# tkob-vh/umi-collapse-rs

Hardware: AMD Instinct MI355X
Metric: UMI-pair Hamming comparisons/s, effective (W pairs of the positions / hot-path time; 12-bp UMIs, all-pairs adjacency + directional collapse; the n-gram partition compares walked_fraction of W, the all-pairs kernels' result bit for bit) (higher is better)
Workload: dtype u32; 1 GPU; BASELINE config 2 per GPU: 1000000 reads, 12-bp UMIs, one alignment position (uniform UMIs), --data naive --algo dir -k 1 -p 0.5; standard=True, reads_per_rank=1000000, positions_per_rank=1, unique_umis_rank0=970714, pairs_W_total=471142349541, parallelism=one GPU

## Files before the change

### include/umihip.h

```cpp
#ifndef UMIHIP_H
#define UMIHIP_H

#include <stdint.h>

#ifdef __cplusplus
extern "C" {
#endif

#define UMI_OK 0
#define UMI_ERR_ARG (-1)
#define UMI_ERR_HIP (-2)
#define UMI_ERR_ORDER (-3)
#define UMI_ERR_NOMEM (-4)
#define UMI_ERR_NODEV (-5)
#define UMI_ERR_CHAR (-6)

#define UMI_ALGO_DIRECTIONAL 0
#define UMI_ALGO_ADJACENCY 1
#define UMI_ALGO_CLUSTER 2

#define UMI_MAX_UMI_LEN 21
#define UMI_MAX_WIDE_UMI_LEN 85
#define UMI_MAX_SEQ_LEN 256

typedef struct umi_ctx umi_ctx;
typedef struct umi_data umi_data;

typedef struct umi_stats {
    uint64_t n_umis;
    uint64_t n_buckets;
    uint64_t max_bucket;
    uint64_t n_kept;
    uint64_t n_pairs;
    uint64_t n_pairs_evaluated;
    uint64_t n_candidates;
    uint64_t n_edges;
    uint32_t n_rounds;
    uint32_t n_pair_launches;
    float ms_total;
    float ms_prep;
    float ms_pairs;
    float ms_collapse;
    float ms_finalize;
    float ms_kernel;
    uint32_t kernel_id;
} umi_stats;
#define UMI_KERNEL_NONE 0
#define UMI_KERNEL_FUSED 1
#define UMI_KERNEL_SEG_PAIRS 2
#define UMI_KERNEL_SEQ_PAIRS 3
#define UMI_KERNEL_EDIT_PAIRS 4

int umi_ctx_create(int device_id, umi_ctx **out);
int umi_ctx_create_multi(const int *device_ids, int n_devices, umi_ctx **out);
int umi_ctx_device_count(const umi_ctx *ctx);
void umi_ctx_destroy(umi_ctx *ctx);
int umi_partition_buckets(const uint64_t *bucket_off, uint64_t n_buckets, uint32_t n_ranks,
                          uint32_t *owner);
const char *umi_last_error(void);
int umi_ctx_set_option(umi_ctx *ctx, const char *name, int64_t value);
#define UMI_ABI_VERSION 2
int umi_abi_version(void);

int umi_encode_umis(const uint8_t *ascii, uint64_t n, int umi_len, uint64_t *keys,
                    uint64_t *nmask);

int umi_encode_umis_wide(const uint8_t *ascii, uint64_t n, int umi_len, int n_words, uint64_t *keys,
                         uint64_t *nmask);
int umi_dedup_batch_wide(umi_ctx *ctx, const uint64_t *keys, const uint64_t *nmask, int n_words,
                         const int32_t *freq, const uint64_t *bucket_off, uint64_t n_buckets,
                         int umi_len, int k, float percentage, int algo, int32_t adj_max_freq,
                         uint8_t *kept, uint32_t *root, umi_stats *stats);
int umi_dedup_batch_wide_device(umi_ctx *ctx, const uint64_t *d_keys, const uint64_t *d_nmask,
                                int n_words, const int32_t *d_freq, const uint64_t *bucket_off,
                                uint64_t n_buckets, int umi_len, int k, float percentage, int algo,
                                int32_t adj_max_freq, uint8_t *d_kept, uint32_t *d_root,
                                void *hip_stream, umi_stats *stats);

int umi_encode_seqs(const uint8_t *ascii, const uint64_t *seq_off, uint64_t n, int n_words, uint64_t *keys,
                    uint64_t *nmask);
int umi_dedup_seqs(umi_ctx *ctx, const uint64_t *keys, const uint64_t *nmask, int n_words, const int32_t *freq,
                   const uint64_t *bucket_off, const int32_t *bucket_len, uint64_t n_buckets, int k,
                   float percentage, int algo, int32_t adj_max_freq, uint8_t *kept, uint32_t *root,
                   umi_stats *stats);
int umi_dedup_seqs_device(umi_ctx *ctx, const uint64_t *d_keys, const uint64_t *d_nmask, int n_words,
                          const int32_t *d_freq, const uint64_t *bucket_off, const int32_t *bucket_len,
                          uint64_t n_buckets, int k, float percentage, int algo, int32_t adj_max_freq,
                          uint8_t *d_kept, uint32_t *d_root, void *hip_stream, umi_stats *stats);

int umi_stage_reads_device(umi_ctx *ctx, const uint64_t *d_align_key, int align_key_bits,
                           const uint8_t *d_umi_ascii, const int32_t *d_score, uint64_t n_reads,
                           int umi_len, int merge, uint64_t *d_keys, uint64_t *d_nmask,
                           int32_t *d_freq, uint64_t *d_rep, uint64_t *d_bucket_off,
                           uint64_t *n_entries, uint64_t *n_buckets, void *hip_stream);
int umi_stage_reads(umi_ctx *ctx, const uint64_t *align_key, int align_key_bits,
                    const uint8_t *umi_ascii, const int32_t *score, uint64_t n_reads, int umi_len,
                    int merge, uint64_t *keys, uint64_t *nmask, int32_t *freq, uint64_t *rep,
                    uint64_t *bucket_off, uint64_t *n_entries, uint64_t *n_buckets);
int umi_stage_reads_wide_device(umi_ctx *ctx, const uint64_t *d_align_key, int align_key_bits,
                                const uint8_t *d_umi_ascii, const int32_t *d_score, uint64_t n_reads, int umi_len,
                                int n_words, int merge, uint64_t *d_keys, uint64_t *d_nmask, int32_t *d_freq,
                                uint64_t *d_rep, uint64_t *d_bucket_off, uint64_t *n_entries, uint64_t *n_buckets,
                                void *hip_stream);
int umi_stage_reads_wide(umi_ctx *ctx, const uint64_t *align_key, int align_key_bits, const uint8_t *umi_ascii,
                         const int32_t *score, uint64_t n_reads, int umi_len, int n_words, int merge, uint64_t *keys,
                         uint64_t *nmask, int32_t *freq, uint64_t *rep, uint64_t *bucket_off, uint64_t *n_entries,
                         uint64_t *n_buckets);
int umi_stage_reads_grouped_device(umi_ctx *ctx, const uint64_t *d_align_key, int align_key_bits,
                                   const uint64_t *d_group_key, int group_key_bits, const uint8_t *d_umi_ascii,
                                   const int32_t *d_score, uint64_t n_reads, int umi_len, int merge, uint64_t *d_keys,
                                   uint64_t *d_nmask, int32_t *d_freq, uint64_t *d_rep, uint64_t *d_bucket_off,
                                   uint64_t *n_entries, uint64_t *n_buckets, void *hip_stream);
int umi_stage_reads_grouped(umi_ctx *ctx, const uint64_t *align_key, int align_key_bits, const uint64_t *group_key,
                            int group_key_bits, const uint8_t *umi_ascii, const int32_t *score, uint64_t n_reads, int umi_len,
                            int merge, uint64_t *keys, uint64_t *nmask, int32_t *freq, uint64_t *rep, uint64_t *bucket_off,
                            uint64_t *n_entries, uint64_t *n_buckets);
int umi_stage_reads_grouped_wide_device(umi_ctx *ctx, const uint64_t *d_align_key, int align_key_bits,
                                        const uint64_t *d_group_key, int group_key_bits, const uint8_t *d_umi_ascii,
                                        const int32_t *d_score, uint64_t n_reads, int umi_len, int n_words, int merge,
                                        uint64_t *d_keys, uint64_t *d_nmask, int32_t *d_freq, uint64_t *d_rep,
                                        uint64_t *d_bucket_off, uint64_t *n_entries, uint64_t *n_buckets, void *hip_stream);
int umi_stage_reads_grouped_wide(umi_ctx *ctx, const uint64_t *align_key, int align_key_bits, const uint64_t *group_key,
                                 int group_key_bits, const uint8_t *umi_ascii, const int32_t *score, uint64_t n_reads,
                                 int umi_len, int n_words, int merge, uint64_t *keys, uint64_t *nmask, int32_t *freq,
                                 uint64_t *rep, uint64_t *bucket_off, uint64_t *n_entries, uint64_t *n_buckets);

int umi_stage_seqs_device(umi_ctx *ctx, const uint8_t *d_text, const uint64_t *d_seq_pos,
                          const uint64_t *d_qual_pos, const uint32_t *d_len, uint64_t n_reads, int n_words,
                          int merge, uint64_t *d_keys, uint64_t *d_nmask, int32_t *d_freq, uint64_t *d_rep,
                          uint32_t *d_entry_of_read, uint64_t *bucket_off, int32_t *bucket_len,
                          uint64_t *n_entries, uint64_t *n_buckets, int *any_n, void *hip_stream);
int umi_stage_seqs(umi_ctx *ctx, const uint8_t *text, const uint64_t *seq_pos, const uint64_t *qual_pos,
                   const uint32_t *len, uint64_t n_reads, int n_words, int merge, uint64_t *keys,
                   uint64_t *nmask, int32_t *freq, uint64_t *rep, uint32_t *entry_of_read,
                   uint64_t *bucket_off, int32_t *bucket_len, uint64_t *n_entries, uint64_t *n_buckets,
                   int *any_n);

int umi_consensus_seqs_device(umi_ctx *ctx, const uint8_t *d_text, const uint64_t *d_seq_pos,
                              const uint64_t *d_qual_pos, const uint32_t *d_len, uint64_t n_reads,
                              const uint32_t *d_entry_of_read, const int32_t *d_freq, const uint8_t *d_kept,
                              const uint32_t *d_root, uint64_t n_entries, const uint64_t *bucket_off,
                              const int32_t *bucket_len, uint64_t n_buckets, uint8_t *d_cons_seq,
                              uint8_t *d_cons_qual, uint64_t *d_cons_off, uint32_t *d_cluster_reads,
// ... 243 lines not shown
```

### umi_collapse_rs_amd/_lib.py

```python
import ctypes as C
import os

_HERE = os.path.dirname(os.path.abspath(__file__))
LIB_PATH = os.environ.get("UMIHIP_LIB") or os.path.join(_HERE, "libumihip.so")

UMI_OK = 0
UMI_ERR_ARG, UMI_ERR_HIP, UMI_ERR_ORDER, UMI_ERR_NOMEM, UMI_ERR_NODEV, UMI_ERR_CHAR = (
    -1, -2, -3, -4, -5, -6)
UMI_ALGO_DIRECTIONAL, UMI_ALGO_ADJACENCY, UMI_ALGO_CLUSTER = 0, 1, 2
UMI_CELLS_CR22, UMI_CELLS_TOP, UMI_CELLS_MIN = 0, 1, 2
UMI_GENE_ASSIGNED, UMI_GENE_NONE, UMI_GENE_SEVERAL = 0, 1, 2
UMI_STRAND_FORWARD, UMI_STRAND_REVERSE, UMI_STRAND_UNSTRANDED = 0, 1, 2
UMI_INTRONS_OFF, UMI_INTRONS_EXON_FIRST, UMI_INTRONS_ALL = 0, 1, 2
UMI_GENE_TIER_EXON, UMI_GENE_TIER_INTRON = 0, 1
(UMI_READ_CLASS_NONE, UMI_READ_CLASS_EXONIC, UMI_READ_CLASS_JUNCTION, UMI_READ_CLASS_SPANNING,
 UMI_READ_CLASS_INTRONIC) = 0, 1, 2, 3, 4
UMI_READ_UNSTAGED = 0xFFFFFFFF
SATURATION_COLUMNS = ("reads", "molecules", "pairs", "cells", "molecules_in_cells", "pairs_in_cells", "median_molecules",
                      "median_genes")
UMI_MAX_UMI_LEN = 21
UMI_KERNEL_EDIT_PAIRS = 4
UMI_MAX_CONS_LEN = 1024
UMI_NO_CLUSTER = 0xFFFFFFFF


class UmiHipError(RuntimeError):
    def __init__(self, code, msg):
        super().__init__("umihip error %d: %s" % (code, msg))
        self.code = code


class Stats(C.Structure):
    _fields_ = [("n_umis", C.c_uint64), ("n_buckets", C.c_uint64), ("max_bucket", C.c_uint64),
                ("n_kept", C.c_uint64), ("n_pairs", C.c_uint64),
                ("n_pairs_evaluated", C.c_uint64), ("n_candidates", C.c_uint64),
                ("n_edges", C.c_uint64), ("n_rounds", C.c_uint32),
                ("n_pair_launches", C.c_uint32), ("ms_total", C.c_float),
                ("ms_prep", C.c_float), ("ms_pairs", C.c_float), ("ms_collapse", C.c_float),
                ("ms_finalize", C.c_float), ("ms_kernel", C.c_float), ("kernel_id", C.c_uint32)]

    def as_dict(self):
        return {k: getattr(self, k) for k, _ in self._fields_}


_u8p, _u32p, _u64p, _i32p = (C.POINTER(C.c_uint8), C.POINTER(C.c_uint32),
                             C.POINTER(C.c_uint64), C.POINTER(C.c_int32))

SIGNATURES = {
    "umi_ctx_create": (C.c_int, [C.c_int, C.POINTER(C.c_void_p)]),
    "umi_ctx_create_multi": (C.c_int, [C.POINTER(C.c_int), C.c_int, C.POINTER(C.c_void_p)]),
    "umi_ctx_device_count": (C.c_int, [C.c_void_p]),
    "umi_partition_buckets": (C.c_int, [_u64p, C.c_uint64, C.c_uint32, _u32p]),
    "umi_ctx_destroy": (None, [C.c_void_p]),
    "umi_last_error": (C.c_char_p, []),
    "umi_ctx_set_option": (C.c_int, [C.c_void_p, C.c_char_p, C.c_int64]),
    "umi_abi_version": (C.c_int, []),
    "umi_encode_umis": (C.c_int, [_u8p, C.c_uint64, C.c_int, _u64p, _u64p]),
    "umi_encode_umis_wide": (C.c_int, [_u8p, C.c_uint64, C.c_int, C.c_int, _u64p, _u64p]),
    "umi_dedup_batch_wide": (C.c_int, [C.c_void_p, _u64p, _u64p, C.c_int, _i32p, _u64p, C.c_uint64, C.c_int,
                                       C.c_int, C.c_float, C.c_int, C.c_int32, _u8p, _u32p, C.POINTER(Stats)]),
    "umi_dedup_batch_wide_device": (C.c_int, [C.c_void_p, C.c_void_p, C.c_void_p, C.c_int, C.c_void_p, _u64p,
                                              C.c_uint64, C.c_int, C.c_int, C.c_float, C.c_int, C.c_int32,
                                              C.c_void_p, C.c_void_p, C.c_void_p, C.POINTER(Stats)]),
    "umi_stage_reads_device": (C.c_int, [C.c_void_p, C.c_void_p, C.c_int, C.c_void_p, C.c_void_p, C.c_uint64,
                                         C.c_int, C.c_int, C.c_void_p, C.c_void_p, C.c_void_p, C.c_void_p,
                                         C.c_void_p, _u64p, _u64p, C.c_void_p]),
    "umi_stage_reads": (C.c_int, [C.c_void_p, _u64p, C.c_int, _u8p, _i32p, C.c_uint64, C.c_int, C.c_int,
                                  _u64p, _u64p, _i32p, _u64p, _u64p, _u64p, _u64p]),
    "umi_stage_reads_wide_device": (C.c_int, [C.c_void_p, C.c_void_p, C.c_int, C.c_void_p, C.c_void_p, C.c_uint64,
                                              C.c_int, C.c_int, C.c_int, C.c_void_p, C.c_void_p, C.c_void_p, C.c_void_p,
                                              C.c_void_p, _u64p, _u64p, C.c_void_p]),
    "umi_stage_reads_wide": (C.c_int, [C.c_void_p, _u64p, C.c_int, _u8p, _i32p, C.c_uint64, C.c_int, C.c_int, C.c_int,
                                       _u64p, _u64p, _i32p, _u64p, _u64p, _u64p, _u64p]),
    "umi_stage_reads_grouped_device": (C.c_int, [C.c_void_p, C.c_void_p, C.c_int, C.c_void_p, C.c_int, C.c_void_p,
                                                 C.c_void_p, C.c_uint64, C.c_int, C.c_int, C.c_void_p, C.c_void_p,
                                                 C.c_void_p, C.c_void_p, C.c_void_p, _u64p, _u64p, C.c_void_p]),
    "umi_stage_reads_grouped_wide_device": (C.c_int, [C.c_void_p, C.c_void_p, C.c_int, C.c_void_p, C.c_int,
                                                      C.c_void_p, C.c_void_p, C.c_uint64, C.c_int, C.c_int, C.c_int,
                                                      C.c_void_p, C.c_void_p, C.c_void_p, C.c_void_p, C.c_void_p,
                                                      _u64p, _u64p, C.c_void_p]),
    "umi_stage_reads_grouped": (C.c_int, [C.c_void_p, _u64p, C.c_int, _u64p, C.c_int, _u8p, _i32p, C.c_uint64, C.c_int,
                                          C.c_int, _u64p, _u64p, _i32p, _u64p, _u64p, _u64p, _u64p]),
    "umi_stage_reads_grouped_wide": (C.c_int, [C.c_void_p, _u64p, C.c_int, _u64p, C.c_int, _u8p, _i32p, C.c_uint64,
                                               C.c_int, C.c_int, C.c_int, _u64p, _u64p, _i32p, _u64p, _u64p, _u64p,
                                               _u64p]),
    "umi_stage_seqs_device": (C.c_int, [C.c_void_p, C.c_void_p, C.c_void_p, C.c_void_p, C.c_void_p, C.c_uint64, C.c_int,
                                        C.c_int, C.c_void_p, C.c_void_p, C.c_void_p, C.c_void_p, C.c_void_p, _u64p,
                                        _i32p, _u64p, _u64p, C.POINTER(C.c_int), C.c_void_p]),
    "umi_stage_seqs": (C.c_int, [C.c_void_p, _u8p, _u64p, _u64p, _u32p, C.c_uint64, C.c_int, C.c_int, _u64p, _u64p,
                                 _i32p, _u64p, _u32p, _u64p, _i32p, _u64p, _u64p, C.POINTER(C.c_int)]),
    "umi_encode_seqs": (C.c_int, [_u8p, _u64p, C.c_uint64, C.c_int, _u64p, _u64p]),
    "umi_dedup_seqs": (C.c_int, [C.c_void_p, _u64p, _u64p, C.c_int, _i32p, _u64p, _i32p, C.c_uint64, C.c_int,
                                 C.c_float, C.c_int, C.c_int32, _u8p, _u32p, C.POINTER(Stats)]),
    "umi_dedup_seqs_device": (C.c_int, [C.c_void_p, C.c_void_p, C.c_void_p, C.c_int, C.c_void_p, _u64p, _i32p,
                                        C.c_uint64, C.c_int, C.c_float, C.c_int, C.c_int32, C.c_void_p, C.c_void_p,
                                        C.c_void_p, C.POINTER(Stats)]),
    "umi_consensus_seqs_device": (C.c_int, [C.c_void_p, C.c_void_p, C.c_void_p, C.c_void_p, C.c_void_p, C.c_uint64,
                                            C.c_void_p, C.c_void_p, C.c_void_p, C.c_void_p, C.c_uint64, _u64p, _i32p,
                                            C.c_uint64, C.c_void_p, C.c_void_p, C.c_void_p, C.c_void_p, _u64p,
                                            C.c_void_p]),
    "umi_consensus_seqs": (C.c_int, [C.c_void_p, _u8p, _u64p, _u64p, _u32p, C.c_uint64, _u32p, _i32p, _u8p, _u32p,
                                     C.c_uint64, _u64p, _i32p, C.c_uint64, _u8p, _u8p, _u64p, _u32p, _u64p]),
    "umi_consensus_bam_device": (C.c_int, [C.c_void_p, C.c_void_p, C.c_void_p, C.c_void_p, C.c_void_p, C.c_void_p,
                                           C.c_uint64, C.c_void_p, C.c_uint64, C.c_void_p, C.c_void_p, C.c_void_p,
                                           C.c_void_p, C.c_void_p, C.c_void_p, _u64p, _u64p, C.c_void_p]),
    "umi_consensus_bam": (C.c_int, [C.c_void_p, _u8p, _u64p, _u64p, _u32p, _u32p, C.c_uint64, _u32p, C.c_uint64, _u8p,
                                    _u8p, _u64p, _u64p, _u32p, _u32p, _u64p, _u64p]),
    "umi_correct_umis_device": (C.c_int, [C.c_void_p, C.c_void_p, C.c_uint64, C.c_int, _u8p, C.c_uint32, C.c_int, C.c_int,
                                          C.c_void_p, C.c_void_p, C.c_void_p, C.c_void_p, _u64p, C.c_void_p]),
    "umi_correct_umis": (C.c_int, [C.c_void_p, _u8p, C.c_uint64, C.c_int, _u8p, C.c_uint32, C.c_int, C.c_int, _u8p,
                                   _i32p, _u8p, _u8p, _u64p]),
    "umi_correct_barcodes_device": (C.c_int, [C.c_void_p, C.c_void_p, C.c_uint64, C.c_int, _u8p, C.c_uint32, C.c_int,
                                              C.c_void_p, C.c_void_p, _u64p, C.c_void_p]),
    "umi_correct_barcodes": (C.c_int, [C.c_void_p, _u8p, C.c_uint64, C.c_int, _u8p, C.c_uint32, C.c_int, _i32p, _u8p,
                                       _u64p]),
    "umi_correct_barcodes_multi_device": (C.c_int, [C.c_void_p, C.c_void_p, C.c_void_p, C.c_uint64, C.c_int, _u8p,
                                                    C.c_uint32, C.c_int, C.c_int, C.c_void_p, C.c_void_p, C.c_void_p,
                                                    _u64p, C.c_void_p]),
    "umi_correct_barcodes_multi": (C.c_int, [C.c_void_p, _u8p, _u8p, C.c_uint64, C.c_int, _u8p, C.c_uint32, C.c_int,
                                             C.c_int, _i32p, _u8p, _u32p, _u64p]),
    "umi_assign_genes_device": (C.c_int, [C.c_void_p, _i32p, _i32p, _i32p, _u8p, _i32p, C.c_uint64, C.c_uint32, C.c_int,
                                          C.c_void_p, C.c_void_p, C.c_void_p, C.c_void_p, C.c_void_p, C.c_uint64,
                                          C.c_void_p, C.c_void_p, _u64p, C.c_void_p]),
    "umi_assign_genes": (C.c_int, [C.c_void_p, _i32p, _i32p, _i32p, _u8p, _i32p, C.c_uint64, C.c_uint32, C.c_int, _i32p,
                                   _i32p, _u8p, _u32p, _u64p, C.c_uint64, _i32p, _u8p, _u64p]),
    "umi_assign_genes_introns_device": (C.c_int, [C.c_void_p, _i32p, _i32p, _i32p, _u8p, _i32p, C.c_uint64, C.c_uint32, C.c_int,
                                                  C.c_int, C.c_void_p, C.c_void_p, C.c_void_p, C.c_void_p, C.c_void_p,
                                                  C.c_uint64, C.c_void_p, C.c_void_p, C.c_void_p, _u64p, C.c_void_p]),
    "umi_assign_genes_introns": (C.c_int, [C.c_void_p, _i32p, _i32p, _i32p, _u8p, _i32p, C.c_uint64, C.c_uint32, C.c_int,
                                           C.c_int, _i32p, _i32p, _u8p, _u32p, _u64p, C.c_uint64, _i32p, _u8p, _u8p, _u64p]),
    "umi_assign_genes_classes_device": (C.c_int, [C.c_void_p, _i32p, _i32p, _i32p, _u8p, _i32p, C.c_uint64, C.c_uint32, C.c_int,
                                                  C.c_int, C.c_void_p, C.c_void_p, C.c_void_p, C.c_void_p, C.c_void_p,
                                                  C.c_uint64, C.c_void_p, C.c_void_p, C.c_void_p, C.c_void_p, _u64p, _u64p,
                                                  C.c_void_p]),
    "umi_assign_genes_classes": (C.c_int, [C.c_void_p, _i32p, _i32p, _i32p, _u8p, _i32p, C.c_uint64, C.c_uint32, C.c_int,
                                           C.c_int, _i32p, _i32p, _u8p, _u32p, _u64p, C.c_uint64, _i32p, _u8p, _u8p, _u8p, _u64p,
                                           _u64p]),
    "umi_assign_genes_transcripts_device": (C.c_int, [C.c_void_p, _i32p, _i32p, _i32p, _u8p, _i32p, _i32p, C.c_uint64, C.c_uint32,
# ... 119 lines not shown
```

### umi_collapse_rs_amd/api.py

```python
import ctypes as C

import numpy as np

from . import _lib
from ._lib import (UMI_ALGO_ADJACENCY, UMI_ALGO_CLUSTER, UMI_ALGO_DIRECTIONAL, UMI_CELLS_CR22, Stats, UmiHipError, check, load, ptr)


def to_bitset(umis, umi_len=None):
    if isinstance(umis, np.ndarray):
        raw = np.ascontiguousarray(umis, dtype=np.uint8)
        assert umi_len, "umi_len is required for a raw byte array"
        n = raw.size // umi_len
    else:
        bs = [u.encode() if isinstance(u, str) else bytes(u) for u in umis]
        n = len(bs)
        umi_len = umi_len or (len(bs[0]) if bs else 1)
        if any(len(b) != umi_len for b in bs):
            raise ValueError("all UMIs of a run have the same length (umi_length)")
        raw = np.frombuffer(b"".join(bs), dtype=np.uint8)
    keys = np.zeros(n, dtype=np.uint64)
    nmask = np.zeros(n, dtype=np.uint64)
    check(load().umi_encode_umis(ptr(raw, C.c_uint8), n, umi_len, ptr(keys, C.c_uint64),
                                 ptr(nmask, C.c_uint64)))
    return keys, nmask


def to_bitset_wide(umis, umi_len):
    w = (3 * umi_len + 63) // 64
    buf = np.frombuffer("".join(umis).encode(), dtype=np.uint8)
    keys = np.zeros((len(umis), w), dtype=np.uint64)
    nm = np.zeros((len(umis), w), dtype=np.uint64)
    check(load().umi_encode_umis_wide(ptr(buf, C.c_uint8), len(umis), umi_len, w, ptr(keys, C.c_uint64),
                                      ptr(nm, C.c_uint64)))
    return keys, nm


def to_bitset_seq(seqs, n_words=None):
    bs = [s.encode() if isinstance(s, str) else bytes(s) for s in seqs]
    off = np.zeros(len(bs) + 1, dtype=np.uint64)
    off[1:] = np.cumsum([len(b) for b in bs], dtype=np.uint64)
    if n_words is None:
        n_words = max(1, (3 * max([len(b) for b in bs] or [0]) + 63) // 64)
    buf = np.frombuffer(b"".join(bs) or b"\0", dtype=np.uint8)
    keys = np.zeros((len(bs), n_words), dtype=np.uint64)
    nm = np.zeros((len(bs), n_words), dtype=np.uint64)
    check(load().umi_encode_seqs(ptr(buf, C.c_uint8), ptr(off, C.c_uint64), len(bs), n_words,
                                 ptr(keys, C.c_uint64), ptr(nm, C.c_uint64)))
    return keys, nm


def partition_buckets(bucket_off, n_ranks):
    bucket_off = np.ascontiguousarray(bucket_off, dtype=np.uint64)
    nb = max(0, len(bucket_off) - 1)
    owner = np.zeros(nb, dtype=np.uint32)
    check(load().umi_partition_buckets(ptr(bucket_off, C.c_uint64), nb, n_ranks, ptr(owner, C.c_uint32)))
    return owner


class Context:

    def __init__(self, device_id=0, profile=False):
        self._h = C.c_void_p()
        if isinstance(device_id, (list, tuple)):
            ids = (C.c_int * len(device_id))(*[int(d) for d in device_id])
            check(load().umi_ctx_create_multi(ids, len(device_id), C.byref(self._h)))
        else:
            check(load().umi_ctx_create(device_id, C.byref(self._h)))
        self.device_id = device_id
        if profile:
            self.set_option("profile", 1)

    def set_option(self, name, value):
        check(load().umi_ctx_set_option(self._h, name.encode(), int(value)))

    def close(self):
        if getattr(self, "_h", None):
            load().umi_ctx_destroy(self._h)
            self._h = None

    def __del__(self):
        try:
            self.close()
        except Exception:
            pass

    def dedup_batch(self, keys, nmask, freq, bucket_off, umi_len, k=1, percentage=0.5,
                    algo=UMI_ALGO_DIRECTIONAL, adj_max_freq=0, want_root=True):
        keys = np.ascontiguousarray(keys, dtype=np.uint64)
        freq = np.ascontiguousarray(freq, dtype=np.int32)
        bucket_off = np.ascontiguousarray(bucket_off, dtype=np.uint64)
        nm = None if nmask is None else np.ascontiguousarray(nmask, dtype=np.uint64)
        n = len(keys)
        if len(freq) != n or (nm is not None and len(nm) != n):
            raise ValueError("keys/nmask/freq lengths differ")
        if len(bucket_off) < 1 or (len(bucket_off) > 1 and int(bucket_off[-1]) != n):
            raise ValueError("bucket_off[-1] must equal len(keys)")
        kept = np.zeros(n, dtype=np.uint8)
        root = np.zeros(n, dtype=np.uint32) if want_root else None
        st = Stats()
        check(load().umi_dedup_batch(self._h, ptr(keys, C.c_uint64), ptr(nm, C.c_uint64),
                                     ptr(freq, C.c_int32), ptr(bucket_off, C.c_uint64),
                                     len(bucket_off) - 1, umi_len, k, percentage, algo,
                                     adj_max_freq, ptr(kept, C.c_uint8), ptr(root, C.c_uint32),
                                     C.byref(st)))
        return kept, root, st.as_dict()

    def dedup_batch_edit(self, keys, nmask, freq, bucket_off, umi_len, k=1, percentage=0.5,
                         algo=UMI_ALGO_DIRECTIONAL, adj_max_freq=0, want_root=True):
        keys = np.ascontiguousarray(keys, dtype=np.uint64)
        freq = np.ascontiguousarray(freq, dtype=np.int32)
        bucket_off = np.ascontiguousarray(bucket_off, dtype=np.uint64)
        nm = None if nmask is None else np.ascontiguousarray(nmask, dtype=np.uint64)
        n = len(keys)
        if len(freq) != n or (nm is not None and len(nm) != n):
            raise ValueError("keys/nmask/freq lengths differ")
        if len(bucket_off) < 1 or (len(bucket_off) > 1 and int(bucket_off[-1]) != n):
            raise ValueError("bucket_off[-1] must equal len(keys)")
        kept = np.zeros(n, dtype=np.uint8)
        root = np.zeros(n, dtype=np.uint32) if want_root else None
        st = Stats()
        check(load().umi_dedup_batch_edit(self._h, ptr(keys, C.c_uint64), ptr(nm, C.c_uint64),
                                          ptr(freq, C.c_int32), ptr(bucket_off, C.c_uint64),
                                          len(bucket_off) - 1, umi_len, k, percentage, algo,
                                          adj_max_freq, ptr(kept, C.c_uint8), ptr(root, C.c_uint32),
                                          C.byref(st)))
        return kept, root, st.as_dict()

    def dedup_batch_wide(self, keys, nmask, freq, bucket_off, umi_len, k=1, percentage=0.5,
                         algo=UMI_ALGO_DIRECTIONAL, adj_max_freq=0, want_root=True):
        keys = np.ascontiguousarray(keys, dtype=np.uint64)
        n, w = keys.shape
        nm = None if nmask is None else np.ascontiguousarray(nmask, dtype=np.uint64)
        freq = np.ascontiguousarray(freq, dtype=np.int32)
        bucket_off = np.ascontiguousarray(bucket_off, dtype=np.uint64)
        kept = np.zeros(max(1, n), dtype=np.uint8)
        root = np.zeros(max(1, n), dtype=np.uint32) if want_root else None
        st = Stats()
        check(load().umi_dedup_batch_wide(self._h, ptr(keys, C.c_uint64), ptr(nm, C.c_uint64), w,
                                          ptr(freq, C.c_int32), ptr(bucket_off, C.c_uint64), len(bucket_off) - 1,
                                          umi_len, k, percentage, algo, adj_max_freq, ptr(kept, C.c_uint8),
                                          ptr(root, C.c_uint32), C.byref(st)))
        return kept[:n], (root[:n] if want_root else None), st.as_dict()

    def dedup_seqs(self, keys, nmask, freq, bucket_off, bucket_len, k=1, percentage=0.5,
                   algo=UMI_ALGO_DIRECTIONAL, adj_max_freq=0, want_root=True):
        keys = np.ascontiguousarray(keys, dtype=np.uint64)
        if keys.ndim != 2:
            raise ValueError("keys must be [N, n_words]")
        n, w = keys.shape
        nm = None if nmask is None else np.ascontiguousarray(nmask, dtype=np.uint64)
        if nm is not None and nm.shape != keys.shape:
            raise ValueError("nmask must have the shape of keys")
        freq = np.ascontiguousarray(freq, dtype=np.int32)
        bucket_off = np.ascontiguousarray(bucket_off, dtype=np.uint64)
        bucket_len = np.ascontiguousarray(bucket_len, dtype=np.int32)
        if len(freq) != n or len(bucket_len) != len(bucket_off) - 1:
# ... 970 lines not shown
```

### umi_collapse_rs_amd/csrc/umihip_api.cpp

```cpp
#include "umihip_host.hpp"

#include <algorithm>
#include <cstdarg>
#include <cstdio>
#include <new>

using namespace umihip;

namespace umihip {

namespace {
thread_local std::string g_err;
}

int fail(int code, const char *fmt, ...)
{
    char buf[512];
    va_list ap;
    va_start(ap, fmt);
    vsnprintf(buf, sizeof(buf), fmt, ap);
    va_end(ap);
    g_err = buf;
    return code;
}

const std::string &last_error() { return g_err; }

int check_common(umi_ctx *ctx, const uint64_t *bucket_off, uint64_t n_buckets, int umi_len, int k,
                 int algo, uint64_t *n_out, int max_len)
{
    if (!ctx) return fail(UMI_ERR_ARG, "ctx is NULL");
    if (!bucket_off) return fail(UMI_ERR_ARG, "bucket_off is NULL");
    if (umi_len < 1 || umi_len > max_len)
        return fail(UMI_ERR_ARG, "umi_len %d outside 1..%d", umi_len, max_len);
    if (k < 0) return fail(UMI_ERR_ARG, "k must be >= 0 (got %d)", k);
    if (!known_algo(algo))
        return fail(UMI_ERR_ARG, "unknown algo %d", algo);
    const uint64_t n = n_buckets ? bucket_off[n_buckets] : 0;
    if (n_buckets && bucket_off[0] != 0) return fail(UMI_ERR_ARG, "bucket_off[0] must be 0");
    if (n >= 0x7FFFFFF0ull)
        return fail(UMI_ERR_ARG, "%llu entries exceed the 31-bit index space of one call",
                    (unsigned long long)n);
    *n_out = n;
    return UMI_OK;
}

}

extern "C" {

const char *umi_last_error(void) { return last_error().c_str(); }

int umi_abi_version(void) { return UMI_ABI_VERSION; }

int umi_ctx_create(int device_id, umi_ctx **out)
{
    if (!out) return fail(UMI_ERR_ARG, "out is NULL");
    *out = nullptr;
    int n_dev = 0;
    hipError_t e = hipGetDeviceCount(&n_dev);
    if (e != hipSuccess || n_dev == 0)
        return fail(UMI_ERR_NODEV, "no HIP device visible (%s)",
                    e == hipSuccess ? "device count 0" : hipGetErrorString(e));
    if (device_id < 0 || device_id >= n_dev)
        return fail(UMI_ERR_ARG, "device_id %d outside 0..%d", device_id, n_dev - 1);
    hipDeviceProp_t prop;
    HIP_TRY(hipGetDeviceProperties(&prop, device_id));
    if (strncmp(prop.gcnArchName, "gfx950", 6) != 0)
        return fail(UMI_ERR_NODEV, "device %d is %s; this library carries gfx950 code only",
                    device_id, prop.gcnArchName);
    HIP_TRY(hipSetDevice(device_id));
    umi_ctx *ctx = new (std::nothrow) umi_ctx();
    if (!ctx) return fail(UMI_ERR_NOMEM, "out of host memory");
    ctx->device = device_id;
    ctx->device_cus = prop.multiProcessorCount > 0 ? prop.multiProcessorCount : 256;
    ctx->n_cus = ctx->device_cus;
    hipError_t err = hipStreamCreateWithFlags(&ctx->own_stream, hipStreamNonBlocking);
    if (err == hipSuccess)
        err = hipHostMalloc((void **)&ctx->h_counters, CTRL_BYTES + 64);
    if (err == hipSuccess) *ctx->h_seq() = 0;
    for (int i = 0; i < umi_ctx::N_EVENTS && err == hipSuccess; i++) err = hipEventCreate(&ctx->ev[i]);

    if (err != hipSuccess) {
        umi_ctx_destroy(ctx);
        return fail(UMI_ERR_HIP, "context setup failed: %s", hipGetErrorString(err));
    }
    *out = ctx;
    return UMI_OK;
}

void umi_ctx_destroy(umi_ctx *ctx)
{
    if (!ctx) return;
    if (!ctx->subs.empty()) {
        for (ncclComm_t c : ctx->comms)
            if (c && ctx->rccl.CommDestroy) (void)ctx->rccl.CommDestroy(c);
        for (umi_ctx *sub : ctx->subs) umi_ctx_destroy(sub);
        delete ctx;
        return;
    }
    settle(ctx);
    (void)hipSetDevice(ctx->device);
    if (ctx->h_counters) (void)hipHostFree(ctx->h_counters);
    for (int i = 0; i < umi_ctx::N_EVENTS; i++)
        if (ctx->ev[i]) (void)hipEventDestroy(ctx->ev[i]);
    if (ctx->own_stream) (void)hipStreamDestroy(ctx->own_stream);
    delete ctx;
}

int umi_ctx_set_option(umi_ctx *ctx, const char *name, int64_t value)
{
    if (!ctx || !name) return fail(UMI_ERR_ARG, "ctx/name is NULL");
    if (!strcmp(name, "split_min")) {
        if (value < 2) return fail(UMI_ERR_ARG, "split_min must be >= 2");
        ctx->split_min = (uint64_t)value;
        return UMI_OK;
    }
    if (!ctx->subs.empty()) {
        for (umi_ctx *sub : ctx->subs) {
            const int rc = umi_ctx_set_option(sub, name, value);
            if (rc) return rc;
        }
        return UMI_OK;
    }
    if (!strcmp(name, "profile")) {
        ctx->profile = value != 0;
    } else if (!strcmp(name, "edge_capacity")) {
        if (value < 1) return fail(UMI_ERR_ARG, "edge_capacity must be >= 1");
        ctx->edge_capacity = (uint64_t)value;
#ifdef UMIHIP_DEV
    } else if (!strcmp(name, "prune")) {
        ctx->prune = value != 0;
    } else if (!strcmp(name, "bs_unit")) {
        if (value < 1 || value > 3) return fail(UMI_ERR_ARG, "bs_unit must be 1, 2 or 3");
        ctx->bs_unit = (int)value;
    } else if (!strcmp(name, "bs_sorted")) {
        ctx->bs_sorted = value != 0;
    } else if (!strcmp(name, "bs_tables")) {
        ctx->bs_tables = value != 0;
    } else if (!strcmp(name, "two_phase")) {
        if (value < 0 || value > 2) return fail(UMI_ERR_ARG, "two_phase must be 0, 1 or 2");
        ctx->two_phase = (int)value;
    } else if (!strcmp(name, "bs_col_chunk")) {
        if (value < BS_COL_TILE || value > (1 << 24) || value % BS_COL_TILE)
            return fail(UMI_ERR_ARG, "bs_col_chunk must be a multiple of %d in %d..%d", BS_COL_TILE,
                        BS_COL_TILE, 1 << 24);
        ctx->bs_col_chunk = (uint32_t)value;
    } else if (!strcmp(name, "bs_tab_min_run")) {
        if (value < 0 || value > (1 << 30)) return fail(UMI_ERR_ARG, "bs_tab_min_run must be in 0..2^30");
        ctx->bs_tab_min_run = (uint32_t)value;
    } else if (!strcmp(name, "bs_transposed")) {
        ctx->bs_transposed = value != 0;
    } else if (!strcmp(name, "bs_tab_waves")) {
        if (value < 0 || value > (1 << 20)) return fail(UMI_ERR_ARG, "bs_tab_waves must be in 0..%d", 1 << 20);
        ctx->bs_tab_waves = (uint32_t)value;
    } else if (!strcmp(name, "bitslice")) {
        ctx->use_bitslice = value != 0;
    } else if (!strcmp(name, "ovf_capacity")) {
        if (value < 1) return fail(UMI_ERR_ARG, "ovf_capacity must be >= 1");
        ctx->ovf_capacity = (uint64_t)value;
#endif
    } else if (!strcmp(name, "seg_index")) {
        ctx->seg_index = value != 0;
    } else if (!strcmp(name, "table_pieces")) {
        if (value < 1 || value > 64) return fail(UMI_ERR_ARG, "table_pieces must be in 1..64");
        ctx->table_pieces = (uint32_t)value;
    } else if (!strcmp(name, "seg_ckey")) {
        ctx->seg_ckey = value != 0;
    } else if (!strcmp(name, "spin_wait")) {
        ctx->spin_wait = value != 0;
    } else if (!strcmp(name, "seg_sliced")) {
        ctx->seg_sliced = value != 0;
    } else if (!strcmp(name, "seg_unite")) {
        ctx->seg_unite = value != 0;
    } else if (!strcmp(name, "seg_lds")) {
        ctx->seg_lds = value != 0;
    } else if (!strcmp(name, "seg_local")) {
        ctx->seg_local = value != 0;
    } else if (!strcmp(name, "seg_probe")) {
        if (value != 0 && value != 1) return fail(UMI_ERR_ARG, "seg_probe must be 0 or 1");
        ctx->seg_probe = value != 0;
    } else if (!strcmp(name, "seg_probe_min")) {
        if (value < 2 || value > SEG_LOCAL_MAX_CAP) return fail(UMI_ERR_ARG, "seg_probe_min must be in 2..%u", SEG_LOCAL_MAX_CAP);
        ctx->seg_probe_min = (uint32_t)value;
    } else if (!strcmp(name, "seg_super")) {
        if (value != 0 && value != 1) return fail(UMI_ERR_ARG, "seg_super must be 0 or 1");
        ctx->seg_super = value != 0;
    } else if (!strcmp(name, "seg_super_coarse")) {
        if (value != 0 && value != 1) return fail(UMI_ERR_ARG, "seg_super_coarse must be 0 or 1");
        ctx->seg_super_coarse = value != 0;
    } else if (!strcmp(name, "seg_super_bases")) {
        if (value < 0 || value > SEG_SUPER_MAX_BASES) return fail(UMI_ERR_ARG, "seg_super_bases must be in 0..%d", SEG_SUPER_MAX_BASES);
        ctx->seg_super_bases = (int)value;
    } else if (!strcmp(name, "seg_super_cap")) {
        if (value < 2 || value > SEG_SUPER_MAX_CAP) return fail(UMI_ERR_ARG, "seg_super_cap must be in 2..%u", SEG_SUPER_MAX_CAP);
        ctx->seg_super_cap = (uint32_t)value;
    } else if (!strcmp(name, "seg_super_min")) {
        if (value < 2 || value > SEG_SUPER_MAX_CAP) return fail(UMI_ERR_ARG, "seg_super_min must be in 2..%u", SEG_SUPER_MAX_CAP);
        ctx->seg_super_min = (uint32_t)value;
    } else if (!strcmp(name, "collapse_kept_only")) {
        ctx->collapse_kept_only = value != 0;
    } else if (!strcmp(name, "seg_local_cap")) {
        if (value < 2 || value > SEG_LOCAL_MAX_CAP) return fail(UMI_ERR_ARG, "seg_local_cap must be in 2..%u", SEG_LOCAL_MAX_CAP);
        ctx->seg_local_cap = (uint32_t)value;
    } else if (!strcmp(name, "seg_blocks")) {
        if (value < 0 || value > (1 << 22)) return fail(UMI_ERR_ARG, "seg_blocks must be in 0..2^22");
        ctx->seg_blocks = (uint32_t)value;
    } else if (!strcmp(name, "grid_cus")) {
        if (value < 0 || value > ctx->device_cus)
            return fail(UMI_ERR_ARG, "grid_cus must be in 0..%d (the device's CUs)", ctx->device_cus);
        ctx->n_cus = value ? (int)value : ctx->device_cus;
    } else if (!strcmp(name, "seg_min")) {
        if (value < 2 || value > (1ll << 31)) return fail(UMI_ERR_ARG, "seg_min must be in 2..2^31");
        ctx->seg_min = (uint32_t)value;
    } else if (!strcmp(name, "cons_split")) {
        if (value < 2 || value > (1ll << 30)) return fail(UMI_ERR_ARG, "cons_split must be in 2..2^30");
        ctx->cons_split = (uint32_t)value;
    } else if (!strcmp(name, "stats_split")) {
        if (value < 64 || value > (1ll << 30)) return fail(UMI_ERR_ARG, "stats_split must be in 64..2^30");
        ctx->stats_split = (uint32_t)value;
    } else if (!strcmp(name, "gene_top")) {
        if (value != 0 && value != 1) return fail(UMI_ERR_ARG, "gene_top must be 0 or 1");
        ctx->gene_top = value != 0;
    } else if (!strcmp(name, "gene_body_top")) {
        if (value != 0 && value != 1) return fail(UMI_ERR_ARG, "gene_body_top must be 0 or 1");
        ctx->gene_body_top = value != 0;
    } else if (!strcmp(name, "velocity_skip")) {
        if (value != 0 && value != 1) return fail(UMI_ERR_ARG, "velocity_skip must be 0 or 1");
        ctx->velocity_skip = value != 0;
    } else if (!strcmp(name, "saturation_skip")) {
        if (value != 0 && value != 1) return fail(UMI_ERR_ARG, "saturation_skip must be 0 or 1");
        ctx->saturation_skip = value != 0;
    } else if (!strcmp(name, "fused_sliced")) {
        ctx->fused_sliced = value != 0;
    } else if (!strcmp(name, "fused_blocks")) {
        if (value < 1 || value > 64) return fail(UMI_ERR_ARG, "fused_blocks must be in 1..64");
        ctx->fused_blocks = (uint32_t)value;
    } else if (!strcmp(name, "fused_max")) {
        if (value < 0) return fail(UMI_ERR_ARG, "fused_max must be >= 0");
        ctx->fused_max = (uint32_t)std::min<int64_t>(value, FUSED_MAX);
    } else if (!strcmp(name, "small_max")) {
        if (value < 0) return fail(UMI_ERR_ARG, "small_max must be >= 0");
        ctx->small_max = (uint32_t)std::min<int64_t>(value, 1 << 30);
    } else {
        return fail(UMI_ERR_ARG, "unknown option '%s'", name);
    }
    return UMI_OK;
}

int umi_ctx_create_multi(const int *device_ids, int n_devices, umi_ctx **out)
{
    if (!out) return fail(UMI_ERR_ARG, "out is NULL");
    *out = nullptr;
    if (!device_ids || n_devices < 1 || n_devices > 64)
        return fail(UMI_ERR_ARG, "device_ids is NULL or n_devices outside 1..64");
    umi_ctx *ctx = new (std::nothrow) umi_ctx();
    if (!ctx) return fail(UMI_ERR_NOMEM, "out of host memory");
    for (int i = 0; i < n_devices; i++) {
        umi_ctx *sub = nullptr;
        const int rc = umi_ctx_create(device_ids[i], &sub);
        if (rc) {
            const std::string msg = umi_last_error();
            umi_ctx_destroy(ctx);
            return fail(rc, "%s", msg.c_str());
        }
        ctx->subs.push_back(sub);
    }
    ctx->device = device_ids[0];
    *out = ctx;
    return UMI_OK;
}

int umi_ctx_device_count(const umi_ctx *ctx) { return !ctx ? 0 : (ctx->subs.empty() ? 1 : (int)ctx->subs.size()); }
// ... 3 lines not shown
```

### umi_collapse_rs_amd/csrc/umihip_host.hpp

```cpp
#pragma once
#include "../../include/umihip.h"

#include <cstring>
#include <dlfcn.h>
#include <string>
#include <type_traits>
#include <vector>

#include "umihip_internal.h"
#include "umihip_io_layout.hpp"
#include "umihip_plan.hpp"

#include <rccl/rccl.h>

namespace umihip {

int fail(int code, const char *fmt, ...);
const std::string &last_error();

#define HIP_TRY(expr)                                                                        \
    do {                                                                                     \
        hipError_t e__ = (expr);                                                             \
        if (e__ != hipSuccess)                                                               \
            return fail(UMI_ERR_HIP, "%s failed: %s (%s:%d)", #expr, hipGetErrorString(e__), \
// ... 93 lines not shown
        for (const char *name : {"librccl.so.1", "librccl.so", "/opt/rocm/lib/librccl.so.1"}) {
            handle = dlopen(name, RTLD_NOW | RTLD_GLOBAL);
            if (handle) break;
        }
        if (!handle) {
            error = std::string("cannot open librccl.so: ") + dlerror();
            return false;
        }
        auto sym = [&](const char *name) {
            void *p = dlsym(handle, name);
            if (!p && error.empty()) error = std::string("librccl.so lacks ") + name;
            return p;
        };
        CommInitAll = (decltype(CommInitAll))sym("ncclCommInitAll");
        CommDestroy = (decltype(CommDestroy))sym("ncclCommDestroy");
        GroupStart = (decltype(GroupStart))sym("ncclGroupStart");
        GroupEnd = (decltype(GroupEnd))sym("ncclGroupEnd");
        AllGather = (decltype(AllGather))sym("ncclAllGather");
        GetErrorString = (decltype(GetErrorString))sym("ncclGetErrorString");
        if (!error.empty()) {
            handle = nullptr;
            return false;
        }
        return true;
    }
};

constexpr int BATCH_MAX_K = 32 * 4;

inline bool known_algo(int algo) { return algo == UMI_ALGO_DIRECTIONAL || algo == UMI_ALGO_ADJACENCY || algo == UMI_ALGO_CLUSTER; }
inline int mode_of(int algo)
{
    return algo == UMI_ALGO_DIRECTIONAL ? MODE_DIRECTIONAL : algo == UMI_ALGO_CLUSTER ? MODE_CLUSTER : MODE_ADJACENCY;
}

inline int wide_words(int umi_len) { return (3 * umi_len + 63) / 64; }

}

struct umi_ctx {
    umihip::RcclApi rccl;
    std::vector<ncclComm_t> comms;
    std::vector<umi_ctx *> subs;
    umihip::PinnedBuf sh_in, sh_out;
    std::vector<uint64_t> sh_boff;
    int device = 0;
    hipStream_t own_stream = nullptr;
    bool profile = false;
    uint64_t edge_capacity = 1u << 20;
    uint64_t ovf_capacity = 1u << 18;
    uint32_t small_max = 1024;
#ifdef UMIHIP_DEV
    static constexpr bool LEGACY_DEFAULT = true;
#else
    static constexpr bool LEGACY_DEFAULT = false;
#endif
    bool use_bitslice = LEGACY_DEFAULT;
    uint32_t bs_col_chunk = umihip::BS_COL_CHUNK;
    uint32_t bs_tab_min_run = 4;
    bool bs_transposed = true;
    uint32_t bs_tab_waves = 0;
    uint32_t fused_max = umihip::FUSED_MAX;
    uint32_t fused_blocks = 20;
    bool fused_sliced = true;
    int bs_unit = 2;
    bool bs_sorted = LEGACY_DEFAULT;
    bool bs_tables = LEGACY_DEFAULT;
    int two_phase = 2;
    bool seg_index = true;
    uint32_t seg_min = 512;
    uint64_t split_min = 200000;
    uint32_t table_pieces = 1;
    bool seg_ckey = true;
    bool seg_sliced = true;
    bool seg_unite = true;
    bool seg_lds = true;
    int seg_occ[2][2][2] = {{{0, 0}, {0, 0}}, {{0, 0}, {0, 0}}};
    bool seg_local = true;
    uint32_t seg_local_cap = umihip::SEG_LOCAL_CAP;
    bool seg_probe = true;
    uint32_t seg_probe_min = umihip::SEG_PROBE_MIN;
    bool seg_super = true;
    bool seg_super_coarse = true;
    int seg_super_bases = 0;
    uint32_t seg_super_cap = umihip::SEG_SUPER_CAP;
    uint32_t seg_super_min = umihip::SEG_SUPER_MIN;
    int seg_local_occ[2] = {0, 0};
    uint32_t seg_local_occ_cap = 0;
    bool collapse_kept_only = true;
    uint32_t seg_blocks = 0;
    umihip::DevBuf fkey, thr, label, lab, edges, edge_dist, ovf, counters, boff, status, blocked;
    umihip::DevBuf plan_tables;
    umihip::DevBuf bs_tasks, plane_tasks, planes, tab_rows, tab_items;
    umihip::DevBuf seg_bin_cnt, seg_bin_start, seg_tasks, seg_sub_rec, seg_priv_edges, seg_priv_dist, seg_priv_cnt, seg_priv_stat;
    umihip::PinnedBuf h_plan_alt[2];
    int plan_flip = 0;
    size_t plan_uploaded = 0;
    const void *plan_uploaded_to = nullptr;
    int n_cus = 256;
    int device_cus = 256;
    umihip::DevBuf fkey_sorted, perm, iota, sort_tmp, sample_pos, sample_out;
    bool prune = false;
    umihip::Plan plan;
    umihip::TablePass table_pass;
    umihip::DevBuf io;
    umihip::DevBuf call_ws;
    umihip::DevBuf seq_groups, seq_ka, seq_kb, seq_va, seq_vb, seq_flag, seq_runid, seq_rs, seq_tend, seq_tmp;
    umihip::PinnedBuf cm_h, ds_h;
    uint32_t stats_split = umihip::STATS_SPLIT;
    bool gene_top = true;
    bool velocity_skip = false;
    bool saturation_skip = false;
    bool gene_body_top = true;
    uint32_t cons_split = 512;
    umihip::PinnedBuf h_boff;
    umihip::PinnedBuf h_tasks;
    unsigned long long *h_counters = nullptr;
    unsigned long long ctrl_seq = 0;
    int dag_rounds_ahead = umihip::DAG_ROUNDS;
    struct PendingCall {
        bool deferred = false, have_result = false;
        unsigned long long seq = 0;
        hipStream_t stream = nullptr;
        int rc = UMI_OK;
        std::string err;
        umi_stats st;
    } pending;
    bool spin_wait = true;
    unsigned long long *h_seq() const { return h_counters + umihip::CTRL_BYTES / sizeof(unsigned long long); }
    uint32_t *h_changed() const { return (uint32_t *)(h_counters + umihip::CNT_COUNT); }
    uint32_t *d_changed() const { return (uint32_t *)(counters.as<unsigned long long>() + umihip::CNT_COUNT); }
    static constexpr int N_EVENTS = 10;
    hipEvent_t ev[N_EVENTS] = {};
};

namespace umihip {

int check_common(umi_ctx *ctx, const uint64_t *bucket_off, uint64_t n_buckets, int umi_len, int k,
                 int algo, uint64_t *n_out, int max_len = UMI_MAX_UMI_LEN);

int run_pipeline(umi_ctx *ctx, const uint64_t *d_keys, const uint64_t *d_nmask,
                 const int32_t *d_freq, const uint64_t *bucket_off, uint64_t n_buckets, uint32_t n,
                 int umi_len, int k, float percentage, int mode, int32_t adj_max_freq,
                 uint8_t *d_kept, uint32_t *d_root, hipStream_t s, umi_stats *stats,
                 const uint64_t *d_bucket_off = nullptr, int n_words = 1, bool may_defer = false, bool edit = false);
int run_pipeline_part(umi_ctx *ctx, const uint64_t *d_keys, const uint64_t *d_nmask, const int32_t *d_freq,
                      const uint64_t *bucket_off, uint64_t n_buckets, uint32_t n, int umi_len, int k,
                      float percentage, int mode, int32_t adj_max_freq, hipStream_t s, uint32_t part,
                      uint32_t n_parts, umi_stats *stats, uint64_t *n_edges);
int collapse_edges(umi_ctx *ctx, uint32_t n, const uint2 *d_edges, uint32_t n_edges, int mode, uint8_t *d_kept,
                   uint32_t *d_root, hipStream_t s, umi_stats *stats);
int finish_pending(umi_ctx *ctx, umi_stats *stats);
void settle(umi_ctx *ctx);

template <typename T> struct IoPtr {
    const DevBuf *block = nullptr;
    size_t off = IO_ABSENT;
    operator T *() const { return (T *)io_at(block->p, off); }
};

class HostIo {
    struct Upload {
        const void *host;
        size_t off, bytes;
    };
    umi_ctx *ctx;
    IoLayout layout;
    std::vector<Upload> uploads;
    bool busy = false;

public:
    explicit HostIo(umi_ctx *c) : ctx(c) {}
    HostIo(const HostIo &) = delete;
    HostIo &operator=(const HostIo &) = delete;
    ~HostIo()
    {
        if (busy) (void)hipStreamSynchronize(ctx->own_stream);
// ... 39 lines not shown
```

### umi_collapse_rs_amd/csrc/umihip_internal.h

```cpp
#pragma once

#include <hip/hip_runtime_api.h>
#include <stdint.h>

namespace umihip {

struct PairTask {
    uint32_t row0;
    uint32_t row_end;
    uint32_t col0;
    uint32_t col1;
};

enum PairMode : int {
    MODE_DIRECTIONAL = 0,
    MODE_ADJACENCY = 1,
    MODE_NEIGHBOURS = 2,
    MODE_CLUSTER = 3,
};

enum Counter : int {
    CNT_EDGES = 0,
    CNT_CANDIDATES = 1,
    CNT_ERROR = 2,
    CNT_KEPT = 3,
    CNT_UNKNOWN = 4,
    CNT_RISES = 5,
    CNT_START_RISES = 6,
    CNT_OVF = 7,
    CNT_ITEMS = 8,
    CNT_DIAG_ITEMS = 9,
    CNT_GRAB = 10,
    CNT_DIAG_GRAB = 11,
    CNT_SEG_TASKS = 12,
    CNT_SEG_PAIRS = 13,
    CNT_KEPT_FUSED = 14,
    CNT_UF_DIRECT = 15,
    CNT_EDGES_MOVED = 16,
    CNT_COUNT = 17,
};
constexpr int MAX_ROUNDS_PER_SYNC = 16;
constexpr size_t CTRL_FLAGS_OFF = CNT_COUNT * sizeof(unsigned long long);
constexpr size_t CTRL_BYTES = (CTRL_FLAGS_OFF + (MAX_ROUNDS_PER_SYNC + 1) * sizeof(uint32_t) + 255) & ~(size_t)255;

struct BsTask {
    uint32_t bucket_start;
    uint32_t bucket_end;
    uint32_t group0;
    uint32_t ngroups;
    uint64_t plane_off;
    uint32_t col0, col1;
    uint32_t diag;
    uint32_t pad;
};

struct RangeTask {
    uint32_t start, end;
    uint32_t seg;
};
constexpr uint32_t SEG_NONE = 0xFFFFFFFFu;

constexpr int SEG_MAX_PARTS = 8;
struct SegDesc {
    uint32_t start, end;
    uint32_t bin_off[SEG_MAX_PARTS];
    uint8_t b0[SEG_MAX_PARTS];
    uint8_t nb[SEG_MAX_PARTS];
    uint64_t mask[SEG_MAX_PARTS];
    uint8_t sup_g;
    uint8_t sup_pad[7];
};
struct SegSuper {
    uint32_t bin0;
    uint8_t g, nb, rest, pad;
};
struct SegRec32 {
    uint32_t key;
    uint32_t idx;
    int32_t freq;
    uint32_t ckey;
};
struct SegRec64 {
    uint64_t key;
    uint32_t idx;
    int32_t freq;
};
struct SegScanChunk {
    uint32_t bin0, nbins;
    uint32_t seg, part;
};
constexpr uint32_t SEG_SCAN_CHUNK = 256;
struct SegTask {
    uint32_t row0, end;
    uint32_t col0;
    uint32_t where;
};
#if defined(__HIPCC__)
#define UMIHIP_HD __host__ __device__
#else
#define UMIHIP_HD
#endif
UMIHIP_HD inline uint32_t seg_chunks_of(uint32_t c) { return c >= 2 ? (c - 1 + 63) / 64 : 0u; }
UMIHIP_HD inline uint32_t seg_span_log2(uint32_t nt)
{
    uint32_t e = 0;
    while (((nt + 15) / 16) > (1u << e)) e++;
    return e;
}
UMIHIP_HD inline uint32_t seg_tasks_of_bin(uint32_t c)
{
    const uint32_t nt = seg_chunks_of(c);
    if (nt == 0) return 0;
    const uint32_t span = 1u << seg_span_log2(nt), q = nt / span, r = nt % span;
    return span * (q * (q + 1) / 2) + r * (q + 1);
}
inline uint64_t seg_task_bound(uint64_t n, uint64_t bins) { return n / 7 + (bins < n / 2 ? bins : n / 2) + 64; }
struct SegBlock {
    uint32_t start, end;
    uint32_t seg, pad;
};
constexpr uint32_t SEG_BLOCK_THREADS = 1024;
constexpr uint32_t SEG_BLOCK_ENTRIES = 8 * SEG_BLOCK_THREADS;
constexpr uint32_t SEG_LDS_BINS = 16384;
constexpr uint32_t RANGE_CHUNK = 2048;

constexpr int BS_TAB_G = 1;
constexpr int BS_TAB_TILE = 256;
constexpr int FUSED_MAX = 128;

struct PlaneTask {
    uint32_t row0;
    uint32_t bucket_end;
    uint64_t plane_off;
    uint32_t ngroups;
    uint32_t group;
};

struct PairArgs {
    const uint64_t *keys;
    const uint64_t *nmask;
    const int32_t *freq;
    const int32_t *thr;
    const void *fkey;
    const PairTask *tasks;
    const BsTask *bs_tasks;
    const uint32_t *planes;
    const uint32_t *perm;
    uint2 *edges;
    uint8_t *edge_dist;
    unsigned long long *counters;
    uint2 *ovf;
    uint32_t ovf_cap;
    uint32_t edge_cap;
    uint32_t n_entries;
    int k;
    int mode;
    int32_t adj_max_freq;
};

constexpr int SMALL_THREADS = 64;
constexpr int SMALL_RPT = 1;
constexpr int BIG_THREADS = 256;
constexpr int BIG_RPT = 8;
constexpr int SMALL_ROWS = SMALL_THREADS * SMALL_RPT;
constexpr int BIG_ROWS = BIG_THREADS * BIG_RPT;
constexpr int COL_TILE = 1024;

hipError_t launch_prep(const uint64_t *keys, const uint64_t *nmask, const int32_t *freq,
                       const uint64_t *bucket_off, uint64_t n_buckets, const RangeTask *ranges,
                       uint32_t n_ranges, uint32_t n, uint32_t fused_max, int umi_len, float percentage,
                       bool key32, void *fkey, int32_t *thr, uint32_t *label, uint32_t *lab,
                       unsigned long long *counters, const SegDesc *segs, int n_seg_parts,
                       uint32_t *bin_cnt, hipStream_t s, bool skip_seg = false, bool entries_too = true,
                       uint32_t seg_from = 0xFFFFFFFFu, int key_words = 1, int full_umi_len = 0);

struct SegArgs {
    const SegDesc *segs;
    const SegScanChunk *chunks;
    uint32_t n_chunks;
    int n_parts;
    uint32_t *bin_cnt;
    uint32_t *bin_start;
    unsigned long long *scan_state;
    SegTask *tasks;
    uint32_t task_cap;
    void *sub_rec;
    const RangeTask *ranges;
    uint32_t n_ranges;
    const SegBlock *blocks;
    uint32_t n_blocks;
    uint32_t lds_bins;
    uint32_t parts_per_pass;
    uint2 *priv_edges;
    uint8_t *priv_dist;
    uint32_t *priv_cnt;
    uint2 *priv_stat;
    uint32_t *uf_parent;
    const uint64_t *prep_keys, *prep_nmask;
    const int32_t *prep_freq;
    int32_t *prep_thr;
    uint32_t *prep_label;
    uint32_t *prep_lab;
    float prep_percentage;
    unsigned long long *prep_counters;
    int umi_len;
    int key_words;
    int full_umi_len;
    uint32_t use_ckey;
    uint32_t col_sliced;
    uint32_t local_cap;
    uint32_t probe_rest, probe_min;
    uint32_t super_cap;
    const SegSuper *supers;
    uint32_t n_supers;
    uint32_t super_coarse;
    uint32_t super_count_pairs;
#ifdef UMIHIP_DEV
    unsigned long long *super_stamps;
#endif
};
constexpr int SEG_SUPER_PHASES = 9;
UMIHIP_HD inline uint32_t seg_scan_flag_word(uint32_t n_chunks, uint32_t seg) { return 1u + n_chunks + seg; }
hipError_t launch_seg_build(const SegArgs &g, void *fkey, const int32_t *freq, bool key32,
                            unsigned long long *counters, hipStream_t s);
constexpr uint32_t SEG_PRIV_CAP = 512;
int seg_pair_blocks_per_cu(bool key32, bool has_n, bool ckey);
hipError_t launch_seg_pairs(const PairArgs &a, const SegArgs &g, bool key32, float percentage,
                            uint32_t part, uint32_t n_parts, uint32_t n_blocks, hipStream_t s);
hipError_t launch_seg_edge_append(const PairArgs &a, const SegArgs &g, uint32_t n_blocks, hipStream_t s);
constexpr uint32_t SEG_LOCAL_MAX_CAP = 2048;
constexpr uint32_t SEG_LOCAL_CAP = 512;
constexpr int SEG_PROBE_MAX_REST = 6;
constexpr uint32_t SEG_PROBE_WORDS = (1u << (2 * SEG_PROBE_MAX_REST)) / 32;
constexpr uint32_t SEG_PROBE_MIN = 129;
constexpr int SEG_SUPER_MAX_REST = 8;
constexpr uint32_t SEG_SUPER_WORDS = (1u << (2 * SEG_SUPER_MAX_REST)) / 32;
constexpr int SEG_SUPER_MAX_BASES = 4;
constexpr uint32_t SEG_SUPER_MAX_CAP = 8192;
constexpr uint32_t SEG_SUPER_CAP = 5632;
constexpr uint32_t SEG_SUPER_MIN = 1024;
constexpr uint32_t SEG_SUPER_SMALL = 2048;
inline uint32_t seg_super_threads(uint32_t cap) { return cap <= SEG_SUPER_SMALL ? 256u : 1024u; }
size_t seg_super_lds_bytes(uint32_t cap);
uint32_t seg_super_blocks(uint32_t n_supers, uint32_t n_cus);
hipError_t launch_seg_super(const PairArgs &a, const SegArgs &g, float percentage, uint32_t n_blocks, hipStream_t s);
size_t seg_local_lds_bytes(uint32_t cap);
int seg_local_blocks_per_cu(bool has_n, uint32_t cap);
hipError_t launch_seg_local(const PairArgs &a, const SegArgs &g, float percentage, uint32_t n_blocks, hipStream_t s);

hipError_t launch_wide_pairs(const PairArgs &a, uint32_t n_tasks, int n_words, hipStream_t s);

hipError_t launch_edit_prep(const uint64_t *keys, const uint64_t *nmask, const int32_t *freq, const uint64_t *bucket_off,
                            uint64_t n_buckets, uint32_t n, int umi_len, float percentage, uint64_t *planes,
                            uint32_t *counts, int32_t *thr, uint32_t *label, unsigned long long *counters, hipStream_t s);
hipError_t launch_edit_pairs(const PairArgs &a, const uint32_t *counts, uint32_t n_tasks, int umi_len, hipStream_t s);

constexpr int SEQ_MAX_WORDS = 12;
constexpr uint32_t SEQ_TILE = 64;
constexpr uint32_t SEQ_ALL_PAIRS = 0xFFFFFFFFu;
struct SeqGroup {
    uint32_t rec_off, bstart, n;
    uint32_t len, nw;
    uint32_t part, n_parts;
    uint32_t pad;
};
struct SeqPairArgs {
    const SeqGroup *groups;
    const uint64_t *rkey;
    const uint32_t *rval;
    uint32_t n_rec;
    const uint64_t *run_id;
    const uint32_t *run_start;
    const uint64_t *task_end;
    const uint64_t *keys, *nmask;
    int stride;
    const int32_t *freq, *thr;
    uint2 *edges;
    unsigned long long *counters;
    uint32_t edge_cap;
    int k, mode;
    int32_t adj_max_freq;
};
hipError_t launch_seq_records(const SeqGroup *groups, uint32_t n_groups, uint32_t n_rec, const uint64_t *keys,
                              const uint64_t *nmask, int stride, const int32_t *freq, float percentage, int32_t *thr,
                              uint64_t *rkey, uint32_t *rval, unsigned long long *counters, hipStream_t s);
hipError_t launch_seq_runs(const uint64_t *rkey, uint32_t n_rec, uint64_t *flag, uint64_t *run_id,
                           uint32_t *run_start, uint64_t *task_end, void *scan_temp, size_t scan_temp_size,
                           unsigned long long *counters, hipStream_t s);
hipError_t launch_seq_pairs(const SeqPairArgs &a, uint32_t n_blocks, hipStream_t s);

size_t stage_workspace_bytes(uint32_t n_reads, int n_words, bool grouped = false);
int stage_reads_on_device(void *workspace, const uint64_t *d_align, int align_bits, const uint64_t *d_group,
                          int group_bits, const uint8_t *d_umi,
                          const int32_t *d_score, uint32_t n, int umi_len, int n_words, int merge, uint64_t *d_keys,
                          uint64_t *d_nmask, int32_t *d_freq, uint64_t *d_rep, uint64_t *d_bucket_off,
                          uint64_t *n_entries_out, uint64_t *n_buckets_out, unsigned long long *h_pinned4,
                          hipStream_t s);

struct SeqFault {
    uint64_t read = 0, value = 0;
};
size_t stage_seqs_workspace_bytes(uint32_t n_reads, int n_words);
int stage_seqs_on_device(void *workspace, const uint8_t *d_text, const uint64_t *d_seq_pos, const uint64_t *d_qual_pos,
                         const uint32_t *d_len, uint32_t n, int n_words, int merge, uint64_t *d_keys, uint64_t *d_nmask,
                         int32_t *d_freq, uint64_t *d_rep, uint32_t *d_eor, uint64_t *h_bucket_off, int32_t *h_bucket_len,
                         uint64_t *n_entries_out, uint64_t *n_buckets_out, int *any_n, SeqFault *fault,
                         unsigned long long *h_pinned4, hipStream_t s);

struct ConsFault {
    unsigned long long bad_root = 0, bad_read = 0, bad_len = 0, empty = 0, freq_sum = 0;
};
uint32_t consensus_effective_split(uint32_t n_reads, uint32_t split);
size_t consensus_workspace_bytes(uint32_t n_reads, uint32_t n_entries, uint32_t n_buckets, uint32_t split);
int consensus_on_device(void *workspace, const uint8_t *d_text, const uint64_t *d_seq_pos, const uint64_t *d_qual_pos,
                        const uint32_t *d_len, uint32_t n_reads, const uint32_t *d_eor, const int32_t *d_freq,
                        const uint8_t *d_kept, const uint32_t *d_root, uint32_t n_entries, const uint64_t *h_bucket_off,
                        const int32_t *h_bucket_len, uint32_t n_buckets, uint32_t split, uint32_t n_cus, uint8_t *d_cons_seq,
                        uint8_t *d_cons_qual, uint64_t *d_cons_off, uint32_t *d_cluster_reads, uint64_t *cons_bytes,
                        ConsFault *fault, unsigned long long *h_pinned, hipStream_t s);

struct ConsBamFault {
    unsigned long long bad_cluster_len = 0, bad_id = 0, bad_len = 0;
};
size_t consensus_bam_workspace_bytes(uint32_t n_reads, uint32_t n_clusters, uint32_t split);
int consensus_bam_on_device(void *workspace, const uint8_t *d_data, const uint64_t *d_seq_pos, const uint64_t *d_qual_pos,
                            const uint32_t *d_len, const uint32_t *d_cluster, uint32_t n_reads, const uint32_t *d_cluster_len,
                            uint32_t n_clusters, uint32_t split, uint32_t n_cus, uint8_t *d_cons_seq, uint8_t *d_cons_qual,
                            uint64_t *d_seq_off, uint64_t *d_qual_off, uint32_t *d_depth, uint32_t *d_disagree,
// ... 262 lines not shown
```

### umi_collapse_rs_amd/csrc/umihip_pipeline.cpp

```cpp
#include "umihip_host.hpp"

#include <algorithm>
#include <chrono>

using namespace umihip;

namespace {

template <class LaunchRound>
int run_rounds(umi_ctx *ctx, hipStream_t s, LaunchRound launch_round, int &rounds, int batch = 4)
{
    uint32_t *d_changed = ctx->d_changed();
    for (;;) {
        HIP_TRY(hipMemsetAsync(d_changed, 0, sizeof(uint32_t) * MAX_ROUNDS_PER_SYNC, s));
        for (int r = 0; r < batch; r++) HIP_TRY(launch_round(d_changed, r));
        HIP_TRY(hipMemcpyAsync(ctx->h_changed(), d_changed, sizeof(uint32_t) * batch, hipMemcpyDeviceToHost, s));
        HIP_TRY(hipStreamSynchronize(s));
        bool done = false;
        for (int r = 0; r < batch && !done; r++) {
            rounds++;
            done = ctx->h_changed()[r] == 0;
        }
        if (done) return UMI_OK;
        if (rounds > MAX_ROUNDS) return fail(UMI_ERR_HIP, "label propagation diverged");
// ... 65 lines not shown
    const unsigned long long bad =
        ctx->h_counters[CNT_ERROR] + (ctx->h_counters[CNT_RISES] - ctx->h_counters[CNT_START_RISES]);
    if (bad)
        return fail(UMI_ERR_ORDER,
                    "%llu entries break the input contract (freq < 1, not in freq-descending rank "
                    "order inside a bucket, or an N base without nmask)",
                    bad);
    return UMI_OK;
}

class Pipeline {
  public:
    Pipeline(umi_ctx *ctx, const uint64_t *d_keys, const uint64_t *d_nmask, const int32_t *d_freq,
             const uint64_t *bucket_off, uint64_t n_buckets, uint32_t n, int umi_len, int k,
             float percentage, int mode, int32_t adj_max_freq, uint8_t *d_kept, uint32_t *d_root,
             hipStream_t s, uint32_t part = 0, uint32_t n_parts = 1)
        : ctx(ctx), d_keys(d_keys), d_nmask(d_nmask), d_freq(d_freq), bucket_off(bucket_off),
          n_buckets(n_buckets), n(n), umi_len(umi_len), k(std::min(k, BATCH_MAX_K)), percentage(percentage), mode(mode),
          adj_max_freq(adj_max_freq), d_kept(d_kept), d_root(d_root), s(s), pl(ctx->plan),
          key32(umi_len <= 16),
          need_pairs(!(mode == MODE_ADJACENCY && adj_max_freq < 1)),
          fused_max((mode == MODE_NEIGHBOURS || !need_pairs || n_parts > 1)
                        ? 0u
                        : std::min<uint32_t>(ctx->fused_max, FUSED_MAX)),
          prof(ctx->profile), part(part), n_parts(n_parts)
    {
        memset(&st, 0, sizeof(st));
        st.n_umis = n;
        st.n_buckets = n_buckets;
    }

    int run(umi_stats *stats)
    {
        HIP_TRY(hipSetDevice(ctx->device));
        int rc = run_stages();
        if (!drained) (void)hipStreamSynchronize(s);
        if (rc == UMI_OK && stats) *stats = st;
        return rc;
    }

    uint64_t edge_count() const { return n_edges; }
    void use_device_table(const uint64_t *d_table) { d_boff_caller = d_table; }
    void use_wide_keys(int words) { n_words = words; }
    void allow_deferred_end() { may_defer = true; }
    void use_edit_distance()
    {
        edit = true;
        k = std::min(k, umi_len);
        fused_max = 0;
    }

  private:
    umi_ctx *ctx;
    const uint64_t *d_keys, *d_nmask;
    const int32_t *d_freq;
    const uint64_t *bucket_off;
    const uint64_t *d_boff_caller = nullptr;
    int n_words = 1;
    bool edit = false;
    bool wide() const { return n_words > 1; }
    int plan_umi_len() const { return wide() ? 21 : umi_len; }
    const uint64_t *d_boff() const { return d_boff_caller ? d_boff_caller : ctx->boff.as<uint64_t>(); }
    uint64_t n_buckets;
    uint32_t n;
    int umi_len, k;
    float percentage;
    int mode;
    int32_t adj_max_freq;
    uint8_t *d_kept;
    uint32_t *d_root;
    hipStream_t s;
    Plan &pl;
    const bool key32, need_pairs;
    uint32_t fused_max;
    const bool prof;
    const uint32_t part, n_parts;
    uint64_t task_counter = 0;
    bool prune = false, drained = false, fused_ran = false, seg_timed = false, edit_timed = false;
    bool may_defer = false;
    size_t zero_behind_control = 0;
    uint32_t priv_blocks_for_collapse = 0;
    uint64_t seg_local_bins = 0;
    bool super_pairs_counted = false;
    umi_stats st;
    unsigned long long *d_cnt = nullptr;
    size_t n_tasks = 0;
    uint64_t n_edges = 0;
    uint64_t n_direct = 0;
    uint64_t seg_tasks_made = 0;
    uint32_t cap_used = 0;
    const void *bs_fkey = nullptr;
    [[maybe_unused]] const uint32_t *bs_perm = nullptr;
    const RangeTask *d_ranges = nullptr;
    const SegDesc *d_segs = nullptr;
    const SegScanChunk *d_chunks = nullptr;
    const PairTask *d_small = nullptr, *d_big = nullptr;
    const SegBlock *d_seg_blocks = nullptr;
    const SegSuper *d_supers = nullptr;
    SegArgs seg;

    bool one_sync() const
    {
        return (mode == MODE_DIRECTIONAL || mode == MODE_CLUSTER || !need_pairs) && n_parts == 1 && ctx->two_phase == 2 &&
               !legacy_tiles();
    }
    bool unions_collapse() const { return mode == MODE_DIRECTIONAL || mode == MODE_CLUSTER; }
    bool mask_only_collapse() const { return d_root == nullptr && ctx->collapse_kept_only; }
    uint32_t *prep_lab() const
    {
        return mode == MODE_DIRECTIONAL && n_parts == 1 && ctx->two_phase == 2 && mask_only_collapse() ? ctx->lab.as<uint32_t>() : nullptr;
    }

    int run_stages()
    {
        int rc;
        if (wide() && (mode != MODE_DIRECTIONAL || k > 3)) fused_max = 0;
        const bool plan_first = n_buckets <= 4096;
        if (plan_first) {
            for (uint64_t b = 0; b < n_buckets; b++)
                if (bucket_off[b + 1] < bucket_off[b])
                    return fail(UMI_ERR_ARG, "bucket_off not monotone at bucket %llu", (unsigned long long)b);
            plan_host();
            if (pl.seg_parts && need_pairs) zero_behind_control = seg_zero_bytes();
        }
        if ((rc = reserve_core())) return rc;
        if ((rc = upload_table(!plan_first))) return rc;
        if (plan_first && pl.n_fused && (rc = fused_stage(0, n_buckets))) return rc;
        if (!plan_first) plan_host();
        if (ctx->table_pass.bad_at != ~0ull)
            return fail(UMI_ERR_ARG, "bucket_off not monotone at bucket %llu", (unsigned long long)ctx->table_pass.bad_at);
        if ((rc = upload_plan())) return rc;
        if ((rc = configure_seg())) return rc;
        if ((rc = prep_stage())) return rc;
        if ((rc = cut_legacy_tiles())) return rc;
        if (need_pairs && pl.seg_parts)
            HIP_TRY(launch_seg_build(seg, ctx->fkey.p, d_freq, key32, d_cnt, s));
        if ((rc = upload_legacy_tiles())) return rc;
        if ((rc = count_tasks())) return rc;
        if (one_sync()) return run_one_sync();
        if (mode == MODE_CLUSTER && n_parts == 1)
            return fail(UMI_ERR_ARG, "algo cluster does not run with the development option two_phase below 2");
        if ((rc = pair_stage())) return rc;
        if (mode == MODE_NEIGHBOURS || n_parts > 1) return finish_neighbours();
        if (mode == MODE_DIRECTIONAL || !need_pairs)
            rc = collapse_directional();
        else
            rc = collapse_adjacency();
        if (rc) return rc;
        return finish();
    }

    int key_bits() const { return key32 ? 2 * umi_len : std::min(64, 3 * umi_len); }

    template <class T> void keep_my_share(std::vector<T> &v)
    {
        if (n_parts <= 1) return;
        size_t w = 0;
        for (size_t i = 0; i < v.size(); i++)
            if ((task_counter++ % n_parts) == part) v[w++] = v[i];
        v.resize(w);
    }

    int defer_control()
    {
        ctx->pending.seq = ++ctx->ctrl_seq;
        ctx->pending.stream = s;
        HIP_TRY(launch_control_to_host(d_cnt, ctx->h_counters, CTRL_BYTES, s, ctx->h_seq(), ctx->pending.seq));
        ctx->pending.st = st;
        ctx->pending.deferred = true;
        drained = true;
        return UMI_OK;
    }
    int read_control()
    {
        if (ctx->spin_wait && !prof) {
            const unsigned long long seq = ++ctx->ctrl_seq;
            HIP_TRY(launch_control_to_host(d_cnt, ctx->h_counters, CTRL_BYTES, s, ctx->h_seq(), seq));
            HIP_TRY(await_control(ctx, seq, s));
        } else {
            HIP_TRY(launch_control_to_host(d_cnt, ctx->h_counters, CTRL_BYTES, s));
            HIP_TRY(hipStreamSynchronize(s));
        }
        return contract_verdict(ctx);
    }

    int reserve_core()
    {
        int rc;
        if ((rc = ctx->fkey.reserve((size_t)n * 8)) || (rc = ctx->thr.reserve((size_t)n * 4)) ||
            (rc = ctx->label.reserve((size_t)n * 4)) || (rc = ctx->lab.reserve((size_t)n * 4)) ||
            (rc = ctx->counters.reserve(CTRL_BYTES + zero_behind_control)) || (rc = ctx->boff.reserve((n_buckets + 1) * 8)))
            return rc;
        if (mode == MODE_ADJACENCY && need_pairs)
            if ((rc = ctx->status.reserve(n)) || (rc = ctx->blocked.reserve(n))) return rc;
        if (edit && (rc = ctx->planes.reserve((size_t)n * 4))) return rc;
        d_cnt = ctx->counters.as<unsigned long long>();
        bs_fkey = ctx->fkey.p;
        return UMI_OK;
    }

    void plan_host()
    {
        scan_table_range(bucket_off, 0, n_buckets, fused_max, nullptr, ctx->table_pass);
        const bool dev_tiles = mode != MODE_CLUSTER;
        const bool seg_on = ctx->seg_index && need_pairs && !(ctx->prune && dev_tiles) && !edit;
        SegSuperOpt sup;
        sup.on = ctx->seg_super && ctx->seg_unite && ctx->seg_ckey && unions_collapse() && n_parts == 1 && ctx->two_phase == 2 &&
                 key32 && !wide() && !edit && !d_nmask;
        sup.bases = ctx->seg_super_bases;
        sup.cap = ctx->seg_super_cap;
        sup.min = ctx->seg_super_min;
        build_plan(bucket_off, n_buckets, wide() || edit ? 0x7FFFFFFFu : ctx->small_max,
                   ctx->use_bitslice && k <= BS_MAX_K && !wide() && !edit && dev_tiles,
                   plan_umi_len(), fused_max, ctx->prune && dev_tiles, ctx->bs_sorted && ctx->bs_unit == 2 && need_pairs && dev_tiles,
                   ctx->bs_tables && key32 && dev_tiles, ctx->bs_tab_min_run, seg_on ? std::max(ctx->seg_min, 1u) : 0u, k, key32, pl,
                   &ctx->table_pass, sup);
        prune = ctx->prune && dev_tiles && need_pairs && !pl.bs_buckets.empty() && !wide() && !edit;
        keep_my_share(pl.small_tasks);
        keep_my_share(pl.big_tasks);
        st.max_bucket = pl.max_bucket;
        st.n_pairs = pl.n_pairs;
    }

    size_t seg_bins_bytes() const { return (pl.seg_bins * 4 + 15) & ~(size_t)15; }
    size_t seg_zero_bytes() const
    {
        return (seg_bins_bytes() + (1 + pl.seg_chunks.size() + pl.segs.size()) * sizeof(unsigned long long) + 15) & ~(size_t)15;
    }

    int upload_plan()
    {
        int rc;
        size_t off = 0;
        auto place = [&](size_t bytes) {
            const size_t at = off;
            off = (off + bytes + 63) & ~(size_t)63;
            return at;
        };
        const size_t o_ranges = place(pl.ranges.size() * sizeof(RangeTask));
        const size_t o_segs = place(pl.segs.size() * sizeof(SegDesc));
        const size_t o_chunks = place(pl.seg_chunks.size() * sizeof(SegScanChunk));
        const size_t o_blocks = place(pl.seg_blocks.size() * sizeof(SegBlock));
        const size_t o_supers = place(pl.seg_supers.size() * sizeof(SegSuper));
        const size_t o_small = place(pl.small_tasks.size() * sizeof(PairTask));
        const size_t o_big = place(pl.big_tasks.size() * sizeof(PairTask));
        const size_t total = std::max<size_t>(off, 64);
        PinnedBuf &hp = ctx->h_plan_alt[ctx->plan_flip];
        if ((rc = hp.reserve(total)) || (rc = ctx->plan_tables.reserve(total))) return rc;
        if (off) memset(hp.p, 0, off);
        if ((rc = hp.put(o_ranges, pl.ranges.data(), pl.ranges.size() * sizeof(RangeTask))) ||
            (rc = hp.put(o_segs, pl.segs.data(), pl.segs.size() * sizeof(SegDesc))) ||
            (rc = hp.put(o_chunks, pl.seg_chunks.data(), pl.seg_chunks.size() * sizeof(SegScanChunk))) ||
            (rc = hp.put(o_blocks, pl.seg_blocks.data(), pl.seg_blocks.size() * sizeof(SegBlock))) ||
            (rc = hp.put(o_supers, pl.seg_supers.data(), pl.seg_supers.size() * sizeof(SegSuper))) ||
            (rc = hp.put(o_small, pl.small_tasks.data(), pl.small_tasks.size() * sizeof(PairTask))) ||
            (rc = hp.put(o_big, pl.big_tasks.data(), pl.big_tasks.size() * sizeof(PairTask))))
            return rc;
        const PinnedBuf &prev = ctx->h_plan_alt[ctx->plan_flip ^ 1];
        const bool same = off && ctx->plan_uploaded == off && ctx->plan_uploaded_to == ctx->plan_tables.p &&
                          prev.p && prev.cap >= off && memcmp(prev.p, hp.p, off) == 0;
        if (off && !same) {
            HIP_TRY(hipMemcpyAsync(ctx->plan_tables.p, hp.p, off, hipMemcpyHostToDevice, s));
            ctx->plan_uploaded = off;
            ctx->plan_uploaded_to = ctx->plan_tables.p;
            ctx->plan_flip ^= 1;
        }
        const char *d = (const char *)ctx->plan_tables.p;
        d_ranges = (const RangeTask *)(d + o_ranges);
        d_segs = (const SegDesc *)(d + o_segs);
        d_chunks = (const SegScanChunk *)(d + o_chunks);
        d_seg_blocks = (const SegBlock *)(d + o_blocks);
        d_supers = (const SegSuper *)(d + o_supers);
        d_small = (const PairTask *)(d + o_small);
        d_big = (const PairTask *)(d + o_big);

        if ((rc = ctx->plane_tasks.reserve(std::max<size_t>(1, pl.plane_tasks.size()) * sizeof(PlaneTask))) ||
            (rc = ctx->planes.reserve(std::max<uint64_t>(1, pl.plane_words) * sizeof(uint32_t))))
            return rc;
        return UMI_OK;
    }

    int configure_seg()
    {
        int rc;
        memset(&seg, 0, sizeof(seg));
        if (pl.seg_parts && need_pairs) {
            if (pl.seg_task_cap > 0x7FFFFFF0ull / sizeof(SegTask) || pl.seg_bins > 0x7FFFFFF0ull ||
                pl.seg_entries * (uint64_t)pl.seg_parts > 0x7FFFFFF0ull)
                return fail(UMI_ERR_NOMEM, "segment index of this call too large (set seg_index=0)");
            const size_t m = (size_t)pl.seg_entries * (size_t)pl.seg_parts;
            if (pl.segs.size() >= (1u << 24)) return fail(UMI_ERR_NOMEM, "too many segments in one call (set seg_index=0)");
            const size_t bins_bytes = seg_bins_bytes(), zero_bytes = seg_zero_bytes();
            if ((!zero_behind_control && (rc = ctx->seg_bin_cnt.reserve(zero_bytes))) ||
                (rc = ctx->seg_bin_start.reserve(pl.seg_bins * 4)) ||
                (rc = ctx->seg_tasks.reserve(pl.seg_task_cap * sizeof(SegTask))) ||
                (rc = ctx->seg_sub_rec.reserve(m * sizeof(SegRec32))))
                return rc;
            static_assert(sizeof(SegRec32) == 16 && sizeof(SegRec64) == 16, "one 16-byte store per record");
            seg.segs = d_segs;
            seg.chunks = d_chunks;
            seg.n_chunks = (uint32_t)pl.seg_chunks.size();
            seg.n_parts = pl.seg_parts;
            seg.bin_cnt = zero_behind_control ? (uint32_t *)((char *)ctx->counters.p + CTRL_BYTES) : ctx->seg_bin_cnt.as<uint32_t>();
            seg.bin_start = ctx->seg_bin_start.as<uint32_t>();
            seg.scan_state = (unsigned long long *)((char *)seg.bin_cnt + bins_bytes);
            seg.tasks = ctx->seg_tasks.as<SegTask>();
            seg.task_cap = (uint32_t)pl.seg_task_cap;
            seg.sub_rec = ctx->seg_sub_rec.p;
            seg.ranges = d_ranges;
            seg.n_ranges = (uint32_t)pl.ranges.size();
            seg.umi_len = plan_umi_len();
            seg.key_words = n_words;
            seg.full_umi_len = umi_len;
            seg.use_ckey = key32 && ctx->seg_ckey && pl.seg_max_rest <= 10 ? 1u : 0u;
            seg.col_sliced = ctx->seg_sliced ? 1u : 0u;
            const bool super_on = !pl.seg_supers.empty() && ctx->seg_unite && unions_collapse() && one_sync() && seg.use_ckey &&
                                  k == 1 && !d_nmask;
            if (super_on) {
                seg.super_cap = ctx->seg_super_cap;
                seg.supers = d_supers;
                seg.n_supers = (uint32_t)pl.seg_supers.size();
            }
            if (ctx->seg_local && ctx->seg_unite && unions_collapse() && one_sync() && seg.use_ckey) {
                seg.local_cap = ctx->seg_local_cap;
                seg_local_bins = 0;
                for (const SegDesc &sd : pl.segs) seg_local_bins += 1ull << (2 * sd.nb[0]);
                if (super_on && pl.seg_plain == 0) seg_local_bins = 0;
                if (ctx->seg_probe && k == 1 && !d_nmask) {
                    seg.probe_rest = SEG_PROBE_MAX_REST;
                    seg.probe_min = ctx->seg_probe_min;
                }
            }
            if (ctx->seg_lds && pl.seg_max_bins <= SEG_LDS_BINS && !pl.seg_blocks.empty()) {
                seg.blocks = d_seg_blocks;
                seg.n_blocks = (uint32_t)pl.seg_blocks.size();
                seg.lds_bins = pl.seg_max_bins;
                seg.parts_per_pass = std::max(1u, std::min({4u, (uint32_t)pl.seg_parts, SEG_LDS_BINS / std::max(1u, pl.seg_max_bins)}));
                seg.super_coarse = super_on && ctx->seg_super_coarse ? 1u : 0u;
            }
            if (!zero_behind_control) HIP_TRY(hipMemsetAsync(seg.bin_cnt, 0, zero_bytes, s));
        }
        return UMI_OK;
    }

    int upload_table(bool fuse)
    {
        if (prof) HIP_TRY(hipEventRecord(ctx->ev[0], s));
        HIP_TRY(hipMemsetAsync(d_cnt, 0, CTRL_BYTES + zero_behind_control, s));
        int rc;
        if ((rc = ctx->h_boff.reserve((n_buckets + 1) * 8))) return rc;
        uint64_t *h_boff = ctx->h_boff.as<uint64_t>();
        if (mode == MODE_ADJACENCY && need_pairs) {
            HIP_TRY(hipMemsetAsync(ctx->status.p, 0, n, s));
            HIP_TRY(hipMemsetAsync(ctx->blocked.p, 0, n, s));
        }
        TablePass &tp = ctx->table_pass;
        scan_table_reset(tp);
        const uint64_t pieces = fuse && fused_max >= 1 ? ctx->table_pieces : 1;
        h_boff[0] = bucket_off[0];
        for (uint64_t c = 0; c < pieces; c++) {
            const uint64_t b0 = n_buckets * c / pieces, b1 = n_buckets * (c + 1) / pieces;
            uint64_t prev = bucket_off[b0], back = 0;
            if (d_boff_caller) {
            } else {
                for (uint64_t b = b0; b < b1; b++) {
                    const uint64_t v = bucket_off[b + 1];
                    back |= v < prev;
                    h_boff[b + 1] = prev = v;
                }
            }
            if (back) {
                for (uint64_t b = b0; b < b1; b++)
                    if (bucket_off[b + 1] < bucket_off[b])
                        return fail(UMI_ERR_ARG, "bucket_off not monotone at bucket %llu", (unsigned long long)b);
            }
            if (!d_boff_caller)
                HIP_TRY(hipMemcpyAsync(ctx->boff.as<uint64_t>() + b0, h_boff + b0, (b1 - b0 + 1) * 8,
                                       hipMemcpyHostToDevice, s));
            if (fuse && b1 > b0 && (rc = fused_stage(b0, b1))) return rc;
        }
        return UMI_OK;
    }

    int fused_stage(uint64_t b0, uint64_t b1)
    {
        if (fused_max < 1 || b1 <= b0) return UMI_OK;
        if (prof && !fused_ran) HIP_TRY(hipEventRecord(ctx->ev[5], s));
        const bool need_label = collapse_walks_all_labels() || !((unions_collapse() || !need_pairs) && n_parts == 1);
        if (wide())
            HIP_TRY(launch_small_buckets_wide(d_keys, d_nmask, n_words, d_freq, percentage, d_boff() + b0, (uint32_t)(b1 - b0),
                                              fused_max, n, d_kept, d_root, k, umi_len, d_cnt,
                                              (uint32_t)ctx->n_cus * ctx->fused_blocks, s));
        else
        HIP_TRY(launch_small_buckets(d_keys, d_nmask, d_freq, percentage, d_boff() + b0,
                                     (uint32_t)(b1 - b0), fused_max, n, need_label ? ctx->label.as<uint32_t>() : nullptr, d_kept,
                                     d_root, k, umi_len, ctx->fused_sliced, mode, adj_max_freq, d_cnt,
                                     (uint32_t)ctx->n_cus * ctx->fused_blocks, s));
        if (prof) HIP_TRY(hipEventRecord(ctx->ev[6], s));
        if (!fused_ran) st.n_pair_launches += 1;
        fused_ran = true;
        return UMI_OK;
    }

    int prep_stage()
    {
        if (edit) {
            HIP_TRY(launch_edit_prep(d_keys, d_nmask, d_freq, d_boff(), n_buckets, n, umi_len, percentage,
                                     ctx->fkey.as<uint64_t>(), ctx->planes.as<uint32_t>(), ctx->thr.as<int32_t>(),
                                     ctx->label.as<uint32_t>(), d_cnt, s));
            if (prep_lab()) HIP_TRY(launch_iota(prep_lab(), n, s));
            return UMI_OK;
        }
        const bool fold = seg.blocks != nullptr;
        if (fold) {
            seg.prep_keys = d_keys;
            seg.prep_nmask = d_nmask;
            seg.prep_freq = d_freq;
            seg.prep_thr = ctx->thr.as<int32_t>();
            seg.prep_label = ctx->label.as<uint32_t>();
            seg.prep_lab = prep_lab();
            seg.prep_percentage = percentage;
            seg.prep_counters = d_cnt;
        }
// ... 164 lines not shown
    static constexpr bool collapse_walks_all_labels() { return false; }
    static int cut_legacy_tiles() { return UMI_OK; }
    static int upload_legacy_tiles() { return UMI_OK; }
    static int enqueue_legacy_tiles(const PairArgs &) { return UMI_OK; }
    static int verify_overflow(uint64_t, uint64_t) { return UMI_OK; }
#endif

    int count_tasks()
    {
        n_tasks = pl.small_tasks.size() + pl.big_tasks.size() + pl.n_bs() + pl.tab_rows.size() +
                  (pl.seg_parts ? 1 : 0);
        if (need_pairs) st.n_pairs_evaluated = edit ? pl.n_pairs : pl.n_pairs_eval;
        if (prof) HIP_TRY(hipEventRecord(ctx->ev[1], s));
        return UMI_OK;
    }

    int reserve_lists(uint64_t cap, uint64_t &ovf_cap)
    {
        int rc;
        if (cap > 0x7FFFFFF0ull) return fail(UMI_ERR_NOMEM, "edge list too large");
        if ((rc = ctx->edges.reserve(cap * sizeof(uint2)))) return rc;
        if (mode == MODE_NEIGHBOURS && (rc = ctx->edge_dist.reserve(cap))) return rc;
        cap_used = (uint32_t)cap;
        ovf_cap = std::min<uint64_t>(std::max<uint64_t>(ctx->ovf_capacity, 1024), 0x7FFFFFF0ull);
        if (legacy_tiles() && (rc = ctx->ovf.reserve(ovf_cap * sizeof(uint2)))) return rc;
        return UMI_OK;
    }

    uint32_t seg_occupancy()
    {
        const bool has_n = d_nmask != nullptr, ck = seg.use_ckey != 0;
        int &slot = ctx->seg_occ[key32 ? 1 : 0][has_n ? 1 : 0][ck ? 1 : 0];
        if (!slot) slot = seg_pair_blocks_per_cu(key32, has_n, ck);
        return (uint32_t)slot;
    }
    uint32_t seg_local_occupancy()
    {
        if (ctx->seg_local_occ_cap != seg.local_cap) {
            ctx->seg_local_occ[0] = ctx->seg_local_occ[1] = 0;
            ctx->seg_local_occ_cap = seg.local_cap;
        }
        int &slot = ctx->seg_local_occ[d_nmask != nullptr ? 1 : 0];
        if (!slot) slot = seg_local_blocks_per_cu(d_nmask != nullptr, seg.local_cap);
        return (uint32_t)slot;
    }

    PairArgs pair_args(uint64_t ovf_cap) const
    {
        PairArgs a;
        a.keys = d_keys;
        a.nmask = d_nmask;
        a.freq = d_freq;
        a.thr = ctx->thr.as<int32_t>();
        a.fkey = ctx->fkey.p;
        a.tasks = d_small;
        a.bs_tasks = ctx->bs_tasks.as<BsTask>();
        a.planes = ctx->planes.as<uint32_t>();
        a.perm = nullptr;
        a.edges = ctx->edges.as<uint2>();
        a.edge_dist = ctx->edge_dist.as<uint8_t>();
        a.counters = d_cnt;
        a.ovf = ctx->ovf.as<uint2>();
        a.ovf_cap = (uint32_t)ovf_cap;
        a.edge_cap = cap_used;
        a.k = k;
        a.mode = mode;
        a.adj_max_freq = adj_max_freq;
        a.n_entries = n;
        return a;
    }

    int enqueue_pairs(uint64_t ovf_cap)
    {
        int rc;
        const PairArgs a = pair_args(ovf_cap);
        if (pl.seg_parts) {
            const uint32_t blocks = std::max(1u, (uint32_t)std::min<uint64_t>(
                pl.seg_task_cap, ctx->seg_blocks ? ctx->seg_blocks : (uint64_t)ctx->n_cus * std::min(16u, seg_occupancy())));
            const uint32_t local_blocks = seg.local_cap && seg_local_bins ? (uint32_t)std::max<uint64_t>(1, std::min<uint64_t>(
                                                              seg_local_bins, (uint64_t)ctx->n_cus * seg_local_occupancy()))
                                                        : 0u;
            const uint32_t super_blocks = seg.super_cap ? seg_super_blocks(seg.n_supers, (uint32_t)ctx->n_cus) : 0u;
            const uint32_t super_slots = super_blocks * (seg_super_threads(seg.super_cap) / 64u);
            const size_t slots = (size_t)local_blocks + super_slots + blocks;
            if ((rc = ctx->seg_priv_edges.reserve(slots * SEG_PRIV_CAP * sizeof(uint2))) ||
                (rc = ctx->seg_priv_cnt.reserve(slots * 4)) || (rc = ctx->seg_priv_stat.reserve(slots * sizeof(uint2))) ||
                (mode == MODE_NEIGHBOURS && (rc = ctx->seg_priv_dist.reserve((size_t)blocks * SEG_PRIV_CAP))))
                return rc;
            seg.priv_edges = ctx->seg_priv_edges.as<uint2>();
            seg.priv_dist = ctx->seg_priv_dist.as<uint8_t>();
            seg.priv_cnt = ctx->seg_priv_cnt.as<uint32_t>();
            seg.uf_parent = one_sync() && ctx->seg_unite ? ctx->label.as<uint32_t>() : nullptr;
            const bool slots_to_collapse = seg.uf_parent && unions_collapse();
            seg.priv_stat = slots_to_collapse ? ctx->seg_priv_stat.as<uint2>() : nullptr;
            if ((seg.local_cap || seg.super_cap) && !seg.uf_parent)
                return fail(UMI_ERR_HIP, "internal: part-0 sub-buckets planned for the local kernel without unions");
            SegArgs super_seg = seg;
            super_seg.super_count_pairs = seg.super_coarse && !super_pairs_counted ? 1u : 0u;
            super_pairs_counted = super_pairs_counted || super_blocks != 0;
            super_seg.priv_edges += (size_t)local_blocks * SEG_PRIV_CAP;
            super_seg.priv_cnt += local_blocks;
            if (super_seg.priv_stat) super_seg.priv_stat += local_blocks;
            SegArgs pair_seg = super_seg;
            pair_seg.priv_edges += (size_t)super_slots * SEG_PRIV_CAP;
            pair_seg.priv_cnt += super_slots;
            if (pair_seg.priv_stat) pair_seg.priv_stat += super_slots;

            if (prof) HIP_TRY(hipEventRecord(ctx->ev[7], s));
            if (local_blocks) HIP_TRY(launch_seg_local(a, seg, percentage, local_blocks, s));
#ifdef UMIHIP_DEV
            const char *phase_file = super_blocks ? getenv("UMIHIP_SUPER_PHASES") : nullptr;
            if (phase_file && *phase_file) {
                const size_t n_stamps = (size_t)super_blocks * SEG_SUPER_PHASES;
                HIP_TRY(hipMalloc((void **)&super_seg.super_stamps, n_stamps * sizeof(unsigned long long)));
                HIP_TRY(hipMemsetAsync(super_seg.super_stamps, 0, n_stamps * sizeof(unsigned long long), s));
            }
#endif
            if (super_blocks) HIP_TRY(launch_seg_super(a, super_seg, percentage, super_blocks, s));
#ifdef UMIHIP_DEV
            if (super_seg.super_stamps) {
                std::vector<unsigned long long> ticks((size_t)super_blocks * SEG_SUPER_PHASES);
                const hipError_t e = hipMemcpyAsync(ticks.data(), super_seg.super_stamps, ticks.size() * sizeof(unsigned long long),
                                                    hipMemcpyDeviceToHost, s);
                const hipError_t e2 = e == hipSuccess ? hipStreamSynchronize(s) : e;
                (void)hipFree(super_seg.super_stamps);
                HIP_TRY(e2);
                if (FILE *f = fopen(phase_file, "a")) {
                    static const char *const names[SEG_SUPER_PHASES] = {"records in", "map built", "ranks and placement",
                        "bit tests, pushes (w0)", "drains", "pointer jumping", "atomicMin", "label stores",
                        "fine-bin pairs counted"};
                    fprintf(f, "seg_super_kernel: %u blocks, us per block (100 MHz clock): phase, mean, max\n", super_blocks);
                    double sum_mean = 0;
                    for (int i = 0; i < SEG_SUPER_PHASES; i++) {
                        unsigned long long tot = 0, mx = 0;
                        for (uint32_t b = 0; b < super_blocks; b++) {
                            const unsigned long long t = ticks[(size_t)b * SEG_SUPER_PHASES + i];
                            tot += t;
                            mx = std::max(mx, t);
                        }
                        sum_mean += (double)tot / super_blocks / 100.0;
                        fprintf(f, "  %-22s %8.2f %8.2f\n", names[i], (double)tot / super_blocks / 100.0, (double)mx / 100.0);
                    }
                    fprintf(f, "  %-22s %8.2f\n", "all phases", sum_mean);
                    fclose(f);
                }
            }
#endif
            HIP_TRY(launch_seg_pairs(a, pair_seg, key32, percentage, part, n_parts, blocks, s));
            if (prof) HIP_TRY(hipEventRecord(ctx->ev[8], s));
            seg_timed = true;
            priv_blocks_for_collapse = slots_to_collapse ? (uint32_t)slots : 0u;
            if (!priv_blocks_for_collapse) HIP_TRY(launch_seg_edge_append(a, seg, blocks, s));
            st.n_pair_launches += 1;
        }
        if ((rc = enqueue_legacy_tiles(a))) return rc;
        if (edit) {
            if (prof) HIP_TRY(hipEventRecord(ctx->ev[7], s));
            HIP_TRY(launch_edit_pairs(a, ctx->planes.as<uint32_t>(), (uint32_t)pl.small_tasks.size(), umi_len, s));
            if (prof) HIP_TRY(hipEventRecord(ctx->ev[8], s));
            edit_timed = true;
            st.n_pair_launches += pl.small_tasks.empty() ? 0 : 1;
            return UMI_OK;
        }
        if (wide()) {
            HIP_TRY(launch_wide_pairs(a, (uint32_t)pl.small_tasks.size(), n_words, s));
            st.n_pair_launches += pl.small_tasks.empty() ? 0 : 1;
            return UMI_OK;
        }
        PairArgs big = a;
        big.tasks = d_big;
        HIP_TRY(launch_pairs(big, (uint32_t)pl.big_tasks.size(), true, key32, s));
        HIP_TRY(launch_pairs(a, (uint32_t)pl.small_tasks.size(), false, key32, s));
        for (auto &v : pl.bs_tasks) st.n_pair_launches += v.empty() ? 0 : 1;
        st.n_pair_launches += pl.tab_rows.empty() ? 0 : 2;
        st.n_pair_launches += (pl.small_tasks.empty() ? 0 : 1) + (pl.big_tasks.empty() ? 0 : 1);
        return UMI_OK;
    }

    int note_pair_counters()
    {
        n_edges = ctx->h_counters[CNT_EDGES] + ctx->h_counters[CNT_EDGES_MOVED];
        n_direct = ctx->h_counters[CNT_UF_DIRECT];
        seg_tasks_made = ctx->h_counters[CNT_SEG_TASKS];
        st.n_candidates = ctx->h_counters[CNT_CANDIDATES];
        st.n_pairs_evaluated = edit ? pl.n_pairs : pl.n_pairs_eval + ctx->h_counters[CNT_SEG_PAIRS];
        if (!pl.tab_rows.empty())
            st.n_pairs_evaluated = st.n_pairs_evaluated - pl.n_pairs_eval_tab +
                                   (ctx->h_counters[CNT_ITEMS] + ctx->h_counters[CNT_DIAG_ITEMS]) *
                                       (64ull * BS_TAB_G * 32) * BS_TAB_TILE;
        if (pl.seg_parts && seg_tasks_made > seg.task_cap)
            return fail(UMI_ERR_HIP, "internal: %llu segment tasks for a list of %u", (unsigned long long)seg_tasks_made, seg.task_cap);
        return UMI_OK;
    }

    int grow_edge_list(uint64_t &cap, int attempt)
    {
        if (attempt >= 3) return fail(UMI_ERR_HIP, "edge list overflow persists");
        if (n_edges > cap) {
            cap = n_edges + n_edges / 16 + 1024;
            ctx->edge_capacity = cap;
        }
        HIP_TRY(hipMemsetAsync(&d_cnt[CNT_EDGES], 0, 2 * sizeof(unsigned long long), s));
        return UMI_OK;
    }

    int pair_stage()
    {
        if (!(need_pairs && n_tasks)) {
            if (prof) HIP_TRY(hipEventRecord(ctx->ev[2], s));
            return UMI_OK;
        }
        int rc;
        uint64_t cap = std::max<uint64_t>(ctx->edge_capacity, 1024);
        for (int attempt = 0;; attempt++) {
            uint64_t ovf_cap = 0;
            if ((rc = reserve_lists(cap, ovf_cap))) return rc;
            if ((rc = enqueue_pairs(ovf_cap))) return rc;
            if ((rc = read_control())) return rc;
            const uint64_t n_ovf = ctx->h_counters[CNT_OVF];
            const bool redo = n_ovf > ovf_cap;
            if (redo)
                ctx->ovf_capacity = n_ovf + n_ovf / 8 + 1024;
            else if (n_ovf && (rc = verify_overflow(n_ovf, ovf_cap)))
                return rc;
            if (prof && !redo) HIP_TRY(hipEventRecord(ctx->ev[2], s));
            if ((rc = note_pair_counters())) return rc;
            if (!redo && n_edges <= cap) break;
            if ((rc = grow_edge_list(cap, attempt))) return rc;
            HIP_TRY(hipMemsetAsync(&d_cnt[CNT_OVF], 0, 5 * sizeof(unsigned long long), s));
        }
        st.n_edges = n_edges;
        return UMI_OK;
    }

    CollapseDesc collapse_desc() const
    {
        CollapseDesc d;
        d.parent = ctx->label.as<uint32_t>();
        d.lab = ctx->lab.as<uint32_t>();
        d.edges = ctx->edges.as<uint2>();
        d.edge_cap = cap_used;
        d.ranges = d_ranges;
        d.n_ranges = (uint32_t)pl.ranges.size();
        d.n = n;
        d.kept = d_kept;
        d.root = d_root;
        d.kept_only = mask_only_collapse();
        d.counters = d_cnt;
        d.changed = ctx->d_changed();
        if (priv_blocks_for_collapse) {
            d.priv_edges = seg.priv_edges;
            d.priv_cnt = seg.priv_cnt;
            d.priv_stat = seg.priv_stat;
            d.priv_blocks = priv_blocks_for_collapse;
        }
        return d;
    }

    int run_one_sync()
    {
        int rc;
        const bool cluster = mode == MODE_CLUSTER;
        uint32_t *d_label = ctx->label.as<uint32_t>();
        const bool have_pairs = need_pairs && n_tasks;
        uint64_t cap = std::max<uint64_t>(ctx->edge_capacity, 1024);
        const int ahead = std::min(std::max(ctx->dag_rounds_ahead, DAG_ROUNDS), MAX_ROUNDS_PER_SYNC);
        for (int attempt = 0;; attempt++) {
            if (have_pairs) {
                uint64_t ovf_cap = 0;
                if ((rc = reserve_lists(cap, ovf_cap))) return rc;
                if ((rc = enqueue_pairs(ovf_cap))) return rc;
            }
            if (prof) HIP_TRY(hipEventRecord(ctx->ev[2], s));
            if (have_pairs && (!seg.uf_parent || legacy_tiles() || !pl.small_tasks.empty() || !pl.big_tasks.empty()))
                HIP_TRY(launch_uf_union_list(ctx->edges.as<uint2>(), d_cnt, cap_used, d_label, cap_used, s));
            if (prof && cluster) HIP_TRY(hipEventRecord(ctx->ev[3], s));
            if (!have_pairs)
                HIP_TRY(launch_finalize(d_label, d_ranges, (uint32_t)pl.ranges.size(), n, d_kept, d_root, d_cnt, s));
            else if (cluster)
                HIP_TRY(launch_cluster_write(collapse_desc(), s));
            else if ((rc = enqueue_directional_collapse(ahead)))
                return rc;
            if (prof && !cluster) HIP_TRY(hipEventRecord(ctx->ev[3], s));
            if (prof) HIP_TRY(hipEventRecord(ctx->ev[4], s));
            if (may_defer && !have_pairs && !prof && ctx->spin_wait) {
                st.n_pairs_evaluated = pl.n_pairs_eval;
                return defer_control();
            }
            if ((rc = read_control())) return rc;
            if ((rc = note_pair_counters())) return rc;
            if (n_edges <= cap || !have_pairs) break;
            if ((rc = grow_edge_list(cap, attempt))) return rc;
            HIP_TRY(hipMemsetAsync(&d_cnt[CNT_KEPT], 0, sizeof(unsigned long long), s));
            HIP_TRY(hipMemsetAsync(&d_cnt[CNT_UF_DIRECT], 0, 2 * sizeof(unsigned long long), s));
            if (!cluster) HIP_TRY(hipMemsetAsync(ctx->d_changed(), 0, CTRL_BYTES - CTRL_FLAGS_OFF, s));
            HIP_TRY(launch_iota(d_label, n, s));
            if (prep_lab()) HIP_TRY(launch_iota(prep_lab(), n, s));
        }
        st.n_edges = n_edges + n_direct;
        if (cluster)
            st.n_rounds = have_pairs && st.n_edges ? 1u : 0u;
        else if ((rc = directional_rounds_end(have_pairs, ahead)))
            return rc;
        return finish_stats();
    }

    int enqueue_directional_collapse(int ahead)
    {
        const CollapseDesc cd = collapse_desc();
        HIP_TRY(launch_collapse_flatten(cd, s));
        static_assert(DAG_ROUNDS >= 2, "the check beside finalize needs a resolving round ahead of it");
        for (int r = cd.kept_only ? 1 : 0; r < ahead - 1; r++) HIP_TRY(launch_collapse_round(cd, r, s));
        HIP_TRY(launch_collapse_finalize(cd, s, ahead - 1));
        return UMI_OK;
    }

    int directional_rounds_end(bool have_pairs, int ahead)
    {
        int rc;
        int rounds = have_pairs && st.n_edges ? 1 : 0;
        for (int r = 0; have_pairs && r < ahead; r++) rounds += (r == 0 || ctx->h_changed()[r - 1]) ? 1 : 0;
        const int rounds_first = rounds;
        if (have_pairs && ctx->h_changed()[ahead - 1]) {
            const CollapseDesc cd = collapse_desc();
            if ((rc = run_rounds(ctx, s, [&](uint32_t *, int r) { return launch_collapse_round(cd, r, s); }, rounds, 4)))
                return rc;
            HIP_TRY(hipMemsetAsync(&d_cnt[CNT_KEPT], 0, sizeof(unsigned long long), s));
            HIP_TRY(launch_collapse_finalize(cd, s));
            if ((rc = read_control())) return rc;
        }
        if (have_pairs) ctx->dag_rounds_ahead = std::max(DAG_ROUNDS, (rounds > rounds_first ? rounds : rounds_first) - 1);
        st.n_rounds = (uint32_t)rounds;
        return UMI_OK;
    }

    int finish_neighbours()
    {
        if (!(need_pairs && n_tasks)) {
            int rc = read_control();
            if (rc) return rc;
        }
        drained = true;
        if (prof) {
            HIP_TRY(hipEventSynchronize(ctx->ev[2]));
            HIP_TRY(hipEventElapsedTime(&st.ms_prep, ctx->ev[0], ctx->ev[1]));
            HIP_TRY(hipEventElapsedTime(&st.ms_pairs, ctx->ev[1], ctx->ev[2]));
            st.ms_total = st.ms_prep + st.ms_pairs;
        }
        return UMI_OK;
    }

    int collapse_directional()
    {
        if (n_edges) {
            int rounds = 0;
            const int rc = directional_labels(ctx, ctx->edges.as<uint2>(), d_cnt, cap_used, n_edges, n, s, rounds);
            if (rc) return rc;
            st.n_rounds = (uint32_t)rounds;
        }
        if (prof) HIP_TRY(hipEventRecord(ctx->ev[3], s));
        HIP_TRY(launch_finalize(ctx->label.as<uint32_t>(), d_ranges, (uint32_t)pl.ranges.size(), n,
                                d_kept, d_root, d_cnt, s));
        return UMI_OK;
    }

    int collapse_adjacency()
    {
        int iters = 0;
        const int rc = adjacency_status(ctx, ctx->edges.as<uint2>(), d_cnt, cap_used, n_edges, n, s, iters);
        if (rc) return rc;
        st.n_rounds = (uint32_t)iters;
        if (prof) HIP_TRY(hipEventRecord(ctx->ev[3], s));
        HIP_TRY(launch_adj_finalize(ctx->status.as<uint8_t>(), ctx->label.as<uint32_t>(), d_ranges,
                                    (uint32_t)pl.ranges.size(), n, d_kept, d_root, d_cnt, s));
        return UMI_OK;
    }

    int finish()
    {
        if (prof) HIP_TRY(hipEventRecord(ctx->ev[4], s));
        int rc = read_control();
        if (rc) return rc;
        return finish_stats();
    }

    int finish_stats()
    {
// ... 180 lines not shown
```

### umi_collapse_rs_amd/csrc/umihip_plan.hpp

```cpp
#pragma once

#include <algorithm>
#include <cstdint>
#include <numeric>
#include <vector>

#include "umihip_internal.h"

namespace umihip {

constexpr uint32_t BIG_COL_CHUNK = 16 * COL_TILE;

struct Plan {
    std::vector<PairTask> small_tasks, big_tasks;
    std::vector<BsTask> bs_tasks[4];
    std::vector<TabRowTile> tab_rows;
    uint64_t tab_items_max = 0;
    uint64_t n_pairs_eval_tab = 0;
    std::vector<PlaneTask> plane_tasks;
    std::vector<RangeTask> ranges;
    struct BsBucket {
        uint64_t s, e, plane_off;
        uint32_t ngroups;
        bool wide;
        int pu;
        int live;
    };
    std::vector<BsBucket> bs_buckets;
    std::vector<SegDesc> segs;
    std::vector<SegScanChunk> seg_chunks;
    std::vector<SegBlock> seg_blocks;
    std::vector<SegSuper> seg_supers;
    uint64_t seg_plain = 0;
    uint32_t seg_max_bins = 0;
    int seg_max_rest = 0;
    int seg_parts = 0;
    uint64_t seg_entries = 0;
    uint64_t seg_bins = 0;
    uint64_t seg_task_cap = 0;
    uint64_t n_fused = 0;
    uint64_t plane_words = 0;
    uint64_t n_pairs = 0, n_pairs_eval = 0, max_bucket = 0, n_tasks_pruned = 0;
    size_t n_bs() const
    {
        size_t t = 0;
        for (auto &v : bs_tasks) t += v.size();
        return t;
    }
    bool any_sorted() const
    {
        for (auto &bb : bs_buckets)
            if (bb.pu || bb.live) return true;
        return false;
    }
};

inline int shared_top_bases(uint64_t lo, uint64_t hi, int umi_len, int bpb)
{
    const uint64_t x = lo ^ hi;
    if (!x) return umi_len;
    const int hb = 63 - __builtin_clzll(x);
    return std::max(0, umi_len - 1 - hb / bpb);
}
inline int range_distance_bound(uint64_t a_lo, uint64_t a_hi, uint64_t b_lo, uint64_t b_hi, int umi_len,
                         int bpb)
{
    const int t = std::min(shared_top_bases(a_lo, a_hi, umi_len, bpb),
                           shared_top_bases(b_lo, b_hi, umi_len, bpb));
    int mism = 0;
    const uint64_t mask = (1ull << bpb) - 1;
    for (int i = umi_len - t; i < umi_len; i++)
        mism += ((a_lo >> (bpb * i)) & mask) != ((b_lo >> (bpb * i)) & mask);
    return mism;
}

inline void gen_bs_tasks(Plan &pl, int umi_len, uint32_t col_chunk, int k,
                  const std::vector<std::vector<uint64_t>> *samples, bool key32)
{
    const uint32_t gpl = (uint32_t)bs_groups_per_lane(umi_len);
    const int bpb = key32 ? 2 : 3;
    for (size_t bi = 0; bi < pl.bs_buckets.size(); bi++) {
        const Plan::BsBucket &bb = pl.bs_buckets[bi];
        const uint64_t s = bb.s, e = bb.e;
        if (bb.live) {
            const uint32_t tile_groups = 64u * (uint32_t)BS_TAB_G;
            for (uint32_t g0 = 0; g0 < bb.ngroups; g0 += tile_groups) {
                const uint64_t r_lo = s + (uint64_t)g0 * 32;
                pl.tab_rows.push_back(TabRowTile{(uint32_t)s, (uint32_t)e, g0, bb.ngroups, bb.plane_off});
                pl.tab_items_max += (e - r_lo + BS_TAB_TILE - 1) / BS_TAB_TILE;
                pl.n_pairs_eval += (uint64_t)tile_groups * 32 * (e - r_lo);
                pl.n_pairs_eval_tab += (uint64_t)tile_groups * 32 * (e - r_lo);
            }
            continue;
        }
        const uint32_t tile_groups = (bb.wide ? 256u : 64u) * gpl;
        const std::vector<uint64_t> *smp = samples ? &(*samples)[bi] : nullptr;
        std::vector<BsTask> &list = pl.bs_tasks[!bb.wide ? 0 : (bb.pu == 3 ? 2 : (bb.pu == 4 ? 3 : 1))];
        auto key_lo = [&](uint64_t pos) { return (*smp)[(pos - s) / BS_COL_TILE]; };
        auto key_hi = [&](uint64_t end) {
            if (end >= e) return smp->back();
            const uint64_t idx = (end - s + BS_COL_TILE - 1) / BS_COL_TILE;
            return idx < smp->size() ? (*smp)[idx] : smp->back();
        };
        for (int pass = 0; pass < 2; pass++)
            for (uint32_t g0 = 0; g0 < bb.ngroups; g0 += tile_groups) {
                const uint64_t r_lo = s + (uint64_t)g0 * 32;
                const uint64_t r_hi = std::min<uint64_t>(e, r_lo + (uint64_t)tile_groups * 32);
                const uint64_t c_begin = pass == 0 ? r_lo : r_lo + (r_hi - r_lo + col_chunk - 1) / col_chunk * col_chunk;
                const uint64_t c_end = pass == 0 ? std::min<uint64_t>(e, c_begin + (r_hi - r_lo + col_chunk - 1) / col_chunk * col_chunk) : e;
                for (uint64_t c0 = c_begin; c0 < c_end; c0 += col_chunk) {
                    const uint64_t c1 = std::min<uint64_t>(e, c0 + col_chunk);
                    const bool diag = c0 < r_hi;
                    if (smp && !diag &&
                        range_distance_bound(key_lo(r_lo), key_hi(r_hi), key_lo(c0), key_hi(c1), umi_len,
                                             bpb) > k) {
                        pl.n_tasks_pruned++;
                        continue;
                    }
                    list.push_back(BsTask{(uint32_t)s, (uint32_t)e, g0, bb.ngroups, bb.plane_off,
                                          (uint32_t)c0, (uint32_t)c1, diag ? 1u : 0u, 0u});
                    pl.n_pairs_eval += (uint64_t)tile_groups * 32 * (c1 - c0);
                }
            }
    }
}

inline int choose_prefix_units(uint64_t n, int umi_len)
{
    const int lp = bs_padded_len(umi_len), units = lp / 2, pad = lp - umi_len;
    for (int pu = 4; pu >= 3; pu--) {
        if (pu >= units) continue;
        const int bases = std::max(0, 2 * pu - pad);
        if ((n >> (2 * bases)) >= 4) return pu;
    }
    return 0;
}

inline int choose_live_units(uint64_t n, int umi_len, uint32_t min_run)
{
    const int lp = bs_padded_len(umi_len), units = lp / 2, pad = lp - umi_len;
    if (units <= 2) return 0;
    const int bases = std::max(0, 2 * (units - 2) - pad);
    return (n >> (2 * bases)) >= min_run ? 2 : 0;
}

inline bool seg_index_applies(int umi_len, int k)
{
    return k >= 0 && k + 1 <= SEG_MAX_PARTS && umi_len / (k + 1) >= 3;
}

struct SegSuperOpt {
    bool on = false;
    int bases = 0;
    uint32_t cap = SEG_SUPER_CAP, min = SEG_SUPER_MIN;
};
inline int choose_super_bases(uint64_t n, int umi_len, int nb0, const SegSuperOpt &o)
{
    if (!o.on) return 0;
    for (int g = std::min(SEG_SUPER_MAX_BASES, nb0); g >= 1; g--) {
        if (o.bases && g != o.bases) continue;
        if (umi_len - nb0 + g > SEG_SUPER_MAX_REST) continue;
        const uint64_t expect = n >> (2 * (nb0 - g));
        if (expect > (uint64_t)o.cap / 4 * 3 || expect < o.min) continue;
        return g;
    }
    return 0;
}

inline void plan_segment(Plan &pl, uint64_t s, uint64_t e, int umi_len, int k, bool key32,
                         const SegSuperOpt &sup = SegSuperOpt())
{
    const int P = k + 1;
    const uint64_t n = e - s;
    int bits = 0;
    while ((n >> bits) > 1) bits++;
    const int nb_cap = std::max(2, std::min(12, (bits - 4) / 2));
    SegDesc sd;
    sd.start = (uint32_t)s;
    sd.end = (uint32_t)e;
    const uint32_t seg = (uint32_t)pl.segs.size();
    for (int j = 0; j < SEG_MAX_PARTS; j++) {
        sd.bin_off[j] = 0;
        sd.b0[j] = 0;
        sd.nb[j] = 0;
        sd.mask[j] = 0;
    }
    sd.sup_g = 0;
    for (uint8_t &b : sd.sup_pad) b = 0;
    for (int j = 0; j < P; j++) {
        const int b0 = j * umi_len / P, b1 = (j + 1) * umi_len / P;
        const int nb = std::min(b1 - b0, nb_cap);
        const uint64_t bins = 1ull << (2 * nb);
        sd.b0[j] = (uint8_t)b0;
        sd.nb[j] = (uint8_t)nb;
        sd.mask[j] = key32 ? (((1ull << (2 * nb)) - 1ull) << (2 * b0)) : (((1ull << (3 * nb)) - 1ull) << (3 * b0));
        sd.bin_off[j] = (uint32_t)pl.seg_bins;
        for (uint64_t b = 0; b < bins; b += SEG_SCAN_CHUNK)
            pl.seg_chunks.push_back({(uint32_t)(pl.seg_bins + b), (uint32_t)std::min<uint64_t>(SEG_SCAN_CHUNK, bins - b),
                                     seg, (uint32_t)j});
        pl.seg_bins += bins;
        pl.seg_max_bins = std::max<uint32_t>(pl.seg_max_bins, (uint32_t)std::min<uint64_t>(bins, 0xFFFFFFFFull));
        pl.seg_max_rest = std::max(pl.seg_max_rest, umi_len - nb);
        pl.seg_task_cap += seg_task_bound(n, bins);
    }
    if (k == 1 && key32) sd.sup_g = (uint8_t)choose_super_bases(n, umi_len, sd.nb[0], sup);
    if (sd.sup_g) {
        const uint32_t g = sd.sup_g, nb0 = sd.nb[0];
        for (uint32_t sb = 0; sb < (1u << (2 * (nb0 - g))); sb++)
            pl.seg_supers.push_back({sd.bin_off[0] + (sb << (2 * g)), (uint8_t)g, (uint8_t)nb0, (uint8_t)(umi_len - nb0 + g), 0});
    } else {
        pl.seg_plain++;
    }
    pl.seg_entries += n;
    for (uint64_t q = s; q < e; q += SEG_BLOCK_ENTRIES)
        pl.seg_blocks.push_back({(uint32_t)q, (uint32_t)std::min<uint64_t>(e, q + SEG_BLOCK_ENTRIES), seg, 0u});
    pl.segs.push_back(sd);
}

struct TablePass {
    uint64_t n_fused = 0, n_pairs = 0, n_pairs_eval = 0, max_bucket = 0;
    uint64_t bad_at = ~0ull;
    std::vector<uint64_t> large;
};
struct TableBlockSums {
    uint64_t fused, pairs, eval, mx, over;
};
#define UMIHIP_TABLE_BLOCK_BODY                                                                         \
    uint32_t fused = 0, pairs = 0, eval = 0, mx = 0, over = 0;                                          \
    for (uint64_t b = b0; b < b1; b++) {                                                                \
        const uint64_t e = bucket_off[b + 1];                                                           \
        const uint64_t n = e - bucket_off[b];                    \
        if (copy) copy[b + 1] = e;                                                                      \
        const uint32_t small = n <= fused_max ? ~0u : 0u;                                               \
        const uint32_t m = (uint32_t)n & small;                                                         \
        fused += m != 0;                                                                                \
        pairs += m * (m - 1u) / 2u;                          \
        eval += m >= 2 ? m * m : 0u;                                                                    \
        mx = m > mx ? m : mx;                                                                           \
        over |= ~small;                                                                                 \
    }                                                                                                   \
    return TableBlockSums{fused, pairs, eval, mx, over};
inline TableBlockSums table_block_generic(const uint64_t *__restrict bucket_off, uint64_t b0, uint64_t b1,
                                          uint32_t fused_max, uint64_t *__restrict copy)
{
    UMIHIP_TABLE_BLOCK_BODY
}
#if defined(__x86_64__)
__attribute__((target("avx2"))) inline TableBlockSums table_block_avx2(const uint64_t *__restrict bucket_off,
                                                                        uint64_t b0, uint64_t b1, uint32_t fused_max,
                                                                        uint64_t *__restrict copy)
{
    UMIHIP_TABLE_BLOCK_BODY
}
#endif
#undef UMIHIP_TABLE_BLOCK_BODY

inline void scan_table_reset(TablePass &tp)
{
    tp.n_fused = tp.n_pairs = tp.n_pairs_eval = tp.max_bucket = 0;
    tp.bad_at = ~0ull;
    tp.large.clear();
}
inline void scan_table_range(const uint64_t *__restrict bucket_off, uint64_t b_begin, uint64_t b_end,
                             uint32_t fused_max, uint64_t *__restrict copy, TablePass &tp)
{
#if defined(__x86_64__)
    const bool avx2 = __builtin_cpu_supports("avx2");
#endif
    constexpr uint64_t BLOCK = 2048;
    for (uint64_t b0 = b_begin; b0 < b_end; b0 += BLOCK) {
        const uint64_t b1 = std::min(b_end, b0 + BLOCK);
        TableBlockSums t;
        if (fused_max > 1024) {
            t = TableBlockSums{0, 0, 0, 0, 0};
            for (uint64_t b = b0; b < b1; b++) {
                const uint64_t e = bucket_off[b + 1], n = e - bucket_off[b];
                if (copy) copy[b + 1] = e;
                if (n <= fused_max) {
                    t.fused += n != 0;
                    t.pairs += n ? n * (n - 1) / 2 : 0;
                    t.eval += n >= 2 ? n * n : 0;
                    t.mx = std::max(t.mx, n);
                } else {
                    t.over = 1;
                }
            }
        } else {
#if defined(__x86_64__)
            t = avx2 ? table_block_avx2(bucket_off, b0, b1, fused_max, copy)
                     : table_block_generic(bucket_off, b0, b1, fused_max, copy);
#else
            t = table_block_generic(bucket_off, b0, b1, fused_max, copy);
#endif
        }
        tp.n_fused += t.fused;
        tp.n_pairs += t.pairs;
        tp.n_pairs_eval += t.eval;
        tp.max_bucket = std::max(tp.max_bucket, t.mx);
        if (t.over)
            for (uint64_t b = b0; b < b1; b++) {
                if (bucket_off[b + 1] < bucket_off[b]) {
                    if (tp.bad_at == ~0ull) tp.bad_at = b;
                } else if (bucket_off[b + 1] - bucket_off[b] > fused_max) {
                    tp.large.push_back(b);
                }
            }
    }
}

inline void scan_table(const uint64_t *__restrict bucket_off, uint64_t n_buckets, uint32_t fused_max,
                       uint64_t *__restrict copy, TablePass &tp)
{
    scan_table_reset(tp);
    if (copy) copy[0] = bucket_off[0];
    scan_table_range(bucket_off, 0, n_buckets, fused_max, copy, tp);
}

inline void build_plan(const uint64_t *bucket_off, uint64_t n_buckets, uint32_t small_max, bool use_bs,
                int umi_len, uint32_t fused_max, bool narrow_only, bool cache_prefix, bool tables,
                uint32_t tab_min_run, uint32_t seg_min, int k, bool key32, Plan &pl,
                const TablePass *pass = nullptr, const SegSuperOpt &sup = SegSuperOpt())
{
    pl.segs.clear();
    pl.seg_chunks.clear();
    pl.seg_blocks.clear();
    pl.seg_supers.clear();
    pl.seg_plain = 0;
    pl.seg_max_bins = 0;
    pl.seg_max_rest = 0;
    pl.seg_parts = 0;
    pl.seg_entries = pl.seg_bins = pl.seg_task_cap = 0;
    const bool seg_ok = seg_min > 0 && seg_index_applies(umi_len, k);
    pl.n_fused = 0;
    pl.ranges.clear();
    uint64_t run_s = 0, run_e = 0;
    uint32_t run_seg = SEG_NONE;
    auto close_run = [&]() {
        for (uint64_t q = run_s; q < run_e; q += RANGE_CHUNK)
            pl.ranges.push_back({(uint32_t)q, (uint32_t)std::min<uint64_t>(run_e, q + RANGE_CHUNK), run_seg});
        run_s = run_e = 0;
        run_seg = SEG_NONE;
    };
    pl.small_tasks.clear();
    pl.big_tasks.clear();
    for (auto &v : pl.bs_tasks) v.clear();
    pl.tab_rows.clear();
    pl.tab_items_max = 0;
    pl.n_pairs_eval_tab = 0;
    pl.plane_tasks.clear();
    pl.bs_buckets.clear();
    pl.plane_words = 0;
    pl.n_pairs = pl.n_pairs_eval = pl.max_bucket = pl.n_tasks_pruned = 0;
    const uint32_t np = 2 * (uint32_t)bs_padded_len(umi_len);
    if (pass) {
        pl.n_fused = pass->n_fused;
        pl.n_pairs = pass->n_pairs;
        pl.n_pairs_eval = pass->n_pairs_eval;
        pl.max_bucket = pass->max_bucket;
    }
    const uint64_t n_visit = pass ? pass->large.size() : n_buckets;
    for (uint64_t vi = 0; vi < n_visit; vi++) {
        const uint64_t b = pass ? pass->large[vi] : vi;
        const uint64_t s = bucket_off[b], e = bucket_off[b + 1];
        const uint64_t n = e - s;
        pl.max_bucket = std::max(pl.max_bucket, n);
        const bool is_seg = seg_ok && n > fused_max && n >= seg_min;
        if (n > fused_max) {
            if (run_e != s || is_seg || run_seg != SEG_NONE) {
                close_run();
                run_s = s;
            }
            run_e = e;
            if (is_seg) run_seg = (uint32_t)pl.segs.size();
        }
        if (n >= 1 && n <= fused_max) pl.n_fused++;
        if (n < 2) continue;
        pl.n_pairs += n * (n - 1) / 2;
        if (n <= fused_max) {
            pl.n_pairs_eval += n * n;
        } else if (is_seg) {
            plan_segment(pl, s, e, umi_len, k, key32, sup);
            pl.seg_parts = k + 1;
        } else if (n <= small_max) {
            for (uint64_t r0 = s; r0 < e; r0 += SMALL_ROWS) {
                pl.small_tasks.push_back({(uint32_t)r0, (uint32_t)e, (uint32_t)r0, (uint32_t)e});
                pl.n_pairs_eval += (uint64_t)SMALL_ROWS * (((e - r0) + 31) / 32 * 32);
            }
        } else if (use_bs) {
            const uint32_t ngroups = (uint32_t)((n + 31) / 32);
            const bool wide = !narrow_only && n >= (uint64_t)BS_WIDE_MIN;
            for (uint32_t g = 0; g < ngroups; g += 2)
                pl.plane_tasks.push_back(
                    {(uint32_t)(s + (uint64_t)g * 32), (uint32_t)e, pl.plane_words, ngroups, g});
            int live = wide && cache_prefix && tables ? choose_live_units(n, umi_len, tab_min_run) : 0;
            if (live && (n / (64u * BS_TAB_G * 32u) + 1) * (n / BS_TAB_TILE + 1) / 2 > (1ull << 26)) live = 0;
            pl.bs_buckets.push_back({s, e, pl.plane_words, ngroups, wide,
                                     wide && cache_prefix && !live ? choose_prefix_units(n, umi_len) : 0, live});
            pl.plane_words += (uint64_t)np * ngroups;
        } else {
            for (uint64_t r0 = s; r0 < e; r0 += BIG_ROWS) {
                for (uint64_t c0 = r0; c0 < e; c0 += BIG_COL_CHUNK) {
                    const uint64_t c1 = std::min<uint64_t>(e, c0 + BIG_COL_CHUNK);
                    pl.big_tasks.push_back(
                        {(uint32_t)r0, (uint32_t)e, (uint32_t)c0, (uint32_t)c1});
                    pl.n_pairs_eval += (uint64_t)BIG_ROWS * (((c1 - c0) + 31) / 32 * 32);
                }
            }
        }
    }
    close_run();
// ... 29 lines not shown
```

### umi_collapse_rs_amd/csrc/umihip_seg.hip

```cpp
#include <hip/hip_runtime.h>

#include "umihip_internal.h"
#include "umihip_device.h"

namespace umihip {

namespace {

constexpr int SCAN_THREADS = 256;
constexpr int SCAN_PER_THREAD = SEG_SCAN_CHUNK / SCAN_THREADS;

__device__ __forceinline__ bool probe_part(const SegArgs &g, uint32_t nb)
{
    return g.probe_rest != 0u && g.umi_len - (int)nb <= (int)g.probe_rest;
}
__device__ __forceinline__ bool local_bin(const SegArgs &g, uint32_t part, uint32_t c) { return part == 0 && c <= g.local_cap; }
__device__ __forceinline__ bool super_taken(const SegArgs &g, uint32_t n) { return n >= 2u && n <= g.super_cap; }
__device__ __forceinline__ uint32_t super_bases(const SegArgs &g, uint32_t seg) { return g.super_cap ? g.segs[seg].sup_g : 0u; }
__device__ __forceinline__ uint32_t coarse_bases(const SegArgs &g, uint32_t seg) { return g.super_coarse ? super_bases(g, seg) : 0u; }

constexpr unsigned long long SCAN_HAVE = 1ull << 63, SCAN_PREFIX = 1ull << 31;
__device__ __forceinline__ unsigned long long scan_pack(uint32_t e, uint32_t t) { return ((unsigned long long)e << 32) | t; }
__global__ __launch_bounds__(SCAN_THREADS) void seg_scan_kernel(SegArgs g, unsigned long long *counters)
{
    __shared__ uint2 wsum[SCAN_THREADS / 64];
    __shared__ uint32_t my_chunk;
    __shared__ uint2 prefix;
    unsigned long long *ticket = g.scan_state, *status = g.scan_state + 1;
    if (threadIdx.x == 0) my_chunk = (uint32_t)atomicAdd(ticket, 1ull);
    __syncthreads();
    const uint32_t ci = my_chunk;
    const SegScanChunk ch = g.chunks[ci];
    uint32_t c[SCAN_PER_THREAD];
    uint2 mine = make_uint2(0u, 0u);
    const uint32_t b_first = threadIdx.x * SCAN_PER_THREAD;
#pragma unroll
    for (int q = 0; q < SCAN_PER_THREAD; q++) {
        const uint32_t b = b_first + q;
        c[q] = b < ch.nbins ? g.bin_cnt[ch.bin0 + b] : 0u;
        mine.x += c[q];
    }
    uint32_t no_tasks = 0;
    const uint32_t sg = ch.part == 0 ? super_bases(g, ch.seg) : 0u;
    if (sg) {
        static_assert(SCAN_PER_THREAD == 1 || SCAN_PER_THREAD == 4, "a super-bin is whole threads' bins");
        __shared__ uint32_t tcnt[SCAN_THREADS];
        tcnt[threadIdx.x] = mine.x;
        __syncthreads();
        const uint32_t nthr = (1u << (2 * sg)) / SCAN_PER_THREAD, t0 = threadIdx.x & ~(nthr - 1u);
        uint32_t n_super = 0;
        for (uint32_t i = 0; i < nthr; i++) n_super += tcnt[t0 + i];
        if (super_taken(g, n_super)) no_tasks = (1u << SCAN_PER_THREAD) - 1u;
        if (n_super > g.super_cap && threadIdx.x == t0) g.scan_state[seg_scan_flag_word(g.n_chunks, ch.seg)] = 1ull;
    } else {
#pragma unroll
        for (int q = 0; q < SCAN_PER_THREAD; q++)
            if (local_bin(g, ch.part, c[q])) no_tasks |= 1u << q;
    }
#pragma unroll
    for (int q = 0; q < SCAN_PER_THREAD; q++) mine.y += (no_tasks >> q) & 1u ? 0u : seg_tasks_of_bin(c[q]);
    uint2 incl = mine;
    for (int d = 1; d < 64; d <<= 1) {
        const uint32_t ux = __shfl_up(incl.x, d), uy = __shfl_up(incl.y, d);
        if ((int)(threadIdx.x & 63) >= d) {
            incl.x += ux;
            incl.y += uy;
        }
    }
    if ((threadIdx.x & 63) == 63) wsum[threadIdx.x >> 6] = incl;
    __syncthreads();
    if (threadIdx.x < 64) {
        uint2 tot = make_uint2(0u, 0u);
        for (int w = 0; w < SCAN_THREADS / 64; w++) {
            tot.x += wsum[w].x;
            tot.y += wsum[w].y;
        }
        const int lane = threadIdx.x;
        if (lane == 0)
            __hip_atomic_store(&status[ci], SCAN_HAVE | (ci == 0 ? SCAN_PREFIX : 0ull) | scan_pack(tot.x, tot.y),
                               __ATOMIC_RELEASE, __HIP_MEMORY_SCOPE_AGENT);
        uint2 before = make_uint2(0u, 0u);
        int64_t j0 = (int64_t)ci - 1;
        while (j0 >= 0) {
            const int64_t j = j0 - lane;
            unsigned long long st = SCAN_HAVE | SCAN_PREFIX;
            if (j >= 0)
                do st = __hip_atomic_load(&status[j], __ATOMIC_ACQUIRE, __HIP_MEMORY_SCOPE_AGENT);
                while (!(st & SCAN_HAVE));
            const unsigned long long stops = __ballot((st & SCAN_PREFIX) != 0);
            const int first = __ffsll(stops) - 1;
            const bool take = first < 0 || lane <= first;
            uint32_t e = take && j >= 0 ? (uint32_t)(st >> 32) & 0x7FFFFFFFu : 0u;
            uint32_t t = take && j >= 0 ? (uint32_t)st & 0x7FFFFFFFu : 0u;
            for (int off = 32; off > 0; off >>= 1) {
                e += __shfl_xor(e, off);
                t += __shfl_xor(t, off);
            }
            before.x += e;
            before.y += t;
            if (first >= 0) break;
            j0 -= 64;
        }
        if (lane == 0) {
            if (ci != 0)
                __hip_atomic_store(&status[ci], SCAN_HAVE | SCAN_PREFIX | scan_pack(before.x + tot.x, before.y + tot.y),
                                   __ATOMIC_RELEASE, __HIP_MEMORY_SCOPE_AGENT);
            prefix = before;
            if (ci + 1 == g.n_chunks) counters[CNT_SEG_TASKS] = before.y + tot.y;
        }
    }
    __syncthreads();
    const uint2 base = prefix;
    uint2 off = make_uint2(base.x + incl.x - mine.x, base.y + incl.y - mine.y);
    for (uint32_t w = 0; w < (threadIdx.x >> 6); w++) {
        off.x += wsum[w].x;
        off.y += wsum[w].y;
    }
    unsigned long long pairs = 0;
#pragma unroll
    for (int q = 0; q < SCAN_PER_THREAD; q++) {
        const uint32_t b = b_first + q;
        if (b < ch.nbins) {
            g.bin_start[ch.bin0 + b] = off.x;
            g.bin_cnt[ch.bin0 + b] = 0;
            const uint32_t nt = (no_tasks >> q) & 1u ? 0u : seg_chunks_of(c[q]), e = seg_span_log2(nt), span = 1u << e;
            const uint32_t where = ch.seg | (ch.part << 24) | (e << 28);
            uint32_t ti = off.y;
            for (uint32_t t = 0; t < nt; t++) {
                const uint32_t row0 = off.x + 64u * t;
                for (uint32_t sp = 0; sp < nt - t; sp += span, ti++)
                    if (ti < g.task_cap) g.tasks[ti] = SegTask{row0, off.x + c[q], row0 + 1u + 64u * sp, where};
            }
            const uint32_t n_bin_tasks = ti - off.y;
            if (!(sg && g.super_coarse)) pairs += (unsigned long long)c[q] * (c[q] ? c[q] - 1 : 0) / 2;
            off.x += c[q];
            off.y += n_bin_tasks;
        }
    }
    __shared__ unsigned long long psum[SCAN_THREADS / 64];
    for (int o = 32; o > 0; o >>= 1) pairs += __shfl_down(pairs, o);
    if ((threadIdx.x & 63) == 0) psum[threadIdx.x >> 6] = pairs;
// ... 91 lines not shown
{
    for (uint32_t b = threadIdx.x; b < ps.total; b += SEG_BLOCK_THREADS) hist[b] = 0;
    __syncthreads();
    constexpr int B = 8;
    for (uint32_t i0 = blk.start + threadIdx.x; i0 < blk.end; i0 += B * SEG_BLOCK_THREADS) {
        KeyT key[B];
#pragma unroll
        for (int q = 0; q < B; q++) {
            const uint32_t i = i0 + (uint32_t)q * SEG_BLOCK_THREADS;
            key[q] = i < blk.end ? fkey[i] : KeyT(0);
        }
#pragma unroll
        for (int q = 0; q < B; q++)
            if (i0 + (uint32_t)q * SEG_BLOCK_THREADS < blk.end) {
#pragma unroll
                for (int j = 0; j < SEG_PASS_PARTS; j++)
                    if (j < ps.np) atomicAdd(&hist[ps.lds_off[j] + (seg_part_bits(key[q], ps.b0[j], ps.nb[j]) >> ps.sh[j])], 1u);
            }
    }
    __syncthreads();
}

__device__ __forceinline__ void store_filter_key(uint32_t *fkey, uint32_t i, uint64_t k3, int umi_len)
{
    uint32_t fk = 0;
    for (int b = 0; b < umi_len; b++) fk |= (uint32_t)((k3 >> (3 * b)) & 3ull) << (2 * b);
    fkey[i] = fk;
}
__device__ __forceinline__ void store_filter_key(uint64_t *fkey, uint32_t i, uint64_t k3, int) { fkey[i] = k3; }

template <typename KeyT>
__global__ __launch_bounds__(SEG_BLOCK_THREADS) void seg_count_lds_kernel(SegArgs g, KeyT *fkey)
{
    extern __shared__ uint32_t hist[];
    const SegBlock blk = g.blocks[blockIdx.x];
    const SegDesc *__restrict__ sd = g.segs + blk.seg;
    const uint32_t cg = coarse_bases(g, blk.seg);
    if (g.prep_keys) {
        unsigned int bad = 0, rises = 0;
        for (uint32_t i = blk.start + threadIdx.x; i < blk.end; i += SEG_BLOCK_THREADS) {
            const uint64_t key = g.prep_keys[(size_t)i * g.key_words];
            const uint64_t nm = g.prep_nmask ? g.prep_nmask[(size_t)i * g.key_words] : 0ull;
            const int32_t f = g.prep_freq[i];
            g.prep_thr[i] = threshold_of(g.prep_percentage, f);
            g.prep_label[i] = i;
            if (g.prep_lab) g.prep_lab[i] = i;
            const uint64_t k3 = key & ~nm & (g.umi_len >= 21 ? 0x7FFFFFFFFFFFFFFFull : ((1ull << (3 * g.umi_len)) - 1ull));
            store_filter_key(fkey, i, k3, g.umi_len);
            bad += f < 1 ? 1u : 0u;
            const uint64_t b2 = k3 & 0x4924924924924924ull;
            bad += (b2 & ~((k3 << 1) | (k3 << 2))) != 0 ? 1u : 0u;
            if (g.key_words > 1 && !g.prep_nmask)
                bad += wide_n_codes(g.prep_keys + (size_t)i * g.key_words, g.key_words, g.full_umi_len);
            rises += (i > sd->start && f > g.prep_freq[i - 1]) ? 1u : 0u;
        }
        if (__any(bad != 0u)) {
            if (bad) atomicAdd(&g.prep_counters[CNT_ERROR], (unsigned long long)bad);
        }
        for (int off = 32; off > 0; off >>= 1) rises += __shfl_down(rises, off);
        if ((threadIdx.x & 63) == 0 && rises) atomicAdd(&g.prep_counters[CNT_RISES], (unsigned long long)rises);
        __syncthreads();
    }
    for (int j0 = 0; j0 < g.n_parts; j0 += (int)g.parts_per_pass) {
        const SegPass ps = seg_pass_of(sd, j0, g.n_parts, (int)g.parts_per_pass, cg);
        seg_block_histogram(blk, fkey, ps, hist);
        for (uint32_t c = threadIdx.x; c < ps.total; c += SEG_BLOCK_THREADS) {
            const uint32_t cnt = hist[c];
            if (cnt) atomicAdd(&g.bin_cnt[seg_pass_global_bin(ps, c)], cnt);
        }
        __syncthreads();
    }
}

template <typename KeyT>
__global__ __launch_bounds__(SEG_BLOCK_THREADS) void seg_scatter_lds_kernel(SegArgs g, const KeyT *__restrict__ fkey,
                                                                            const int32_t *__restrict__ freq)
{
    using Rec = typename SegRecOf<KeyT>::type;
    extern __shared__ uint32_t hist[];
    const SegBlock blk = g.blocks[blockIdx.x];
    const SegDesc *__restrict__ sd = g.segs + blk.seg;
    const uint32_t cg = coarse_bases(g, blk.seg);
    Rec *__restrict__ sub = (Rec *)g.sub_rec;
    for (int j0 = 0; j0 < g.n_parts; j0 += (int)g.parts_per_pass) {
        const SegPass ps = seg_pass_of(sd, j0, g.n_parts, (int)g.parts_per_pass, cg);
        seg_block_histogram(blk, fkey, ps, hist);
        for (uint32_t c = threadIdx.x; c < ps.total; c += SEG_BLOCK_THREADS) {
            const uint32_t cnt = hist[c];
            if (cnt) {
                const uint32_t gb = seg_pass_global_bin(ps, c);
                hist[c] = g.bin_start[gb] + atomicAdd(&g.bin_cnt[gb], cnt);
            }
        }
        __syncthreads();
        constexpr int B = 4;
        for (uint32_t i0 = blk.start + threadIdx.x; i0 < blk.end; i0 += B * SEG_BLOCK_THREADS) {
            KeyT key[B];
            int32_t f[B];
#pragma unroll
            for (int q = 0; q < B; q++) {
                const uint32_t i = i0 + (uint32_t)q * SEG_BLOCK_THREADS;
                key[q] = i < blk.end ? fkey[i] : KeyT(0);
                f[q] = i < blk.end ? freq[i] : 0;
            }
            uint64_t e3[B];
#pragma unroll
            for (int q = 0; q < B; q++) e3[q] = g.use_ckey ? expand3(key[q], g.umi_len) : 0ull;
#pragma unroll
            for (int j = 0; j < SEG_PASS_PARTS; j++) {
                if (j < ps.np) {
                    uint32_t pos[B];
#pragma unroll
                    for (int q = 0; q < B; q++)
                        pos[q] = i0 + (uint32_t)q * SEG_BLOCK_THREADS < blk.end
                                     ? atomicAdd(&hist[ps.lds_off[j] + (seg_part_bits(key[q], ps.b0[j], ps.nb[j]) >> ps.sh[j])], 1u)
                                     : 0u;
#pragma unroll
                    for (int q = 0; q < B; q++) {
                        const uint32_t i = i0 + (uint32_t)q * SEG_BLOCK_THREADS;
                        if (i < blk.end)
                            sub[pos[q]] = make_rec(key[q], i, f[q],
                                                   g.use_ckey ? compare_key(e3[q], ps.b0[j], ps.nb[j], g.umi_len) : 0u);
                    }
                }
            }
        }
        __syncthreads();
    }
}

__device__ __forceinline__ uint32_t readlane_key(uint32_t v, int lane)
{
    return (uint32_t)__builtin_amdgcn_readlane((int)v, lane);
}
__device__ __forceinline__ uint64_t readlane_key(uint64_t v, int lane)
{
    const uint32_t lo = (uint32_t)__builtin_amdgcn_readlane((int)(uint32_t)v, lane);
    const uint32_t hi = (uint32_t)__builtin_amdgcn_readlane((int)(uint32_t)(v >> 32), lane);
    return ((uint64_t)hi << 32) | lo;
}

__device__ __forceinline__ bool within_k(uint32_t z, int k)
{
    return __builtin_popcount((z | (z >> 1)) & 0x55555555u) <= k;
}
__device__ __forceinline__ bool within_k(uint64_t z, int k)
{
    return __builtin_popcountll(z) <= 2 * k;
}

template <bool CK> __device__ __forceinline__ uint32_t loop_key(const SegRec32 &r) { return CK ? r.ckey : r.key; }
template <bool CK> __device__ __forceinline__ uint64_t loop_key(const SegRec64 &r) { return r.key; }
template <bool CK> __device__ __forceinline__ bool loop_within_k(uint32_t z, int k)
{
    return CK ? __builtin_popcount(z) <= 2 * k : within_k(z, k);
}
template <bool CK> __device__ __forceinline__ bool loop_within_k(uint64_t z, int k) { return within_k(z, k); }

template <bool CK, int J> __device__ __forceinline__ uint32_t four_columns(uint32_t h, uint32_t x, uint32_t ky, int k, uint32_t lim2)
{
    if (CK) {
        uint32_t s0, s1, s2, s3, t0, t1, t2, t3;
        unsigned long long p0, p1, p2, p3;
        asm("v_readlane_b32 %1, %14, %16\n\t"
            "v_readlane_b32 %2, %14, %17\n\t"
            "v_readlane_b32 %3, %14, %18\n\t"
            "v_readlane_b32 %4, %14, %19\n\t"
            "v_xor_b32_e32 %5, %1, %13\n\t"
// ... 724 lines not shown
#else
    auto stamp = [](int) {};
#endif
    auto decide = [&](bool has, uint32_t pa, uint32_t pb) {
        const uint32_t ia = ix[pa], ib = ix[pb];
        const int32_t fa = (int32_t)fr[pa], fb = (int32_t)fr[pb];
        const bool sw = ib < ia;
        const uint32_t gi = sw ? ib : ia, gj = sw ? ia : ib;
        const int32_t fi = sw ? fb : fa, fj = sw ? fa : fb;
        if (has) n_cand++;
        const bool fwd = has && (CLUSTER || fj <= threshold_of(percentage, fi));
        const bool bwd = has && (CLUSTER || fi <= threshold_of(percentage, fj));
        if (fwd && bwd) {
            n_direct++;
            lds_union_halving(par, min(pa, pb), max(pa, pb));
        }
        emit(fwd != bwd, fwd ? gi : gj, fwd ? gj : gi);
    };
    auto rank_of = [&](uint32_t s) {
        return pre[s >> 5] + (uint32_t)__builtin_popcount(bm[s >> 5] & ((1u << (s & 31u)) - 1u));
    };
    uint32_t nq = 0;
    auto drain = [&](bool walk) {
        const uint32_t n = min(nq, 64u);
        nq -= n;
        __builtin_amdgcn_fence(__ATOMIC_ACQ_REL, "wavefront");
        __builtin_amdgcn_wave_barrier();
        const bool has = (uint32_t)lane < n;
        const uint32_t h = has ? hitq[nq + (uint32_t)lane] : 0u;
        const uint32_t x = h >> 13;
        decide(has, h & 0x1FFFu, walk ? x : rank_of(x));
        __builtin_amdgcn_wave_barrier();
    };
    auto push = [&](bool has, uint32_t h, bool walk) {
        const unsigned long long bal = __ballot(has);
        if (has) hitq[nq + (uint32_t)__builtin_popcountll(bal & ((1ull << lane) - 1ull))] = h;
        nq += (uint32_t)__builtin_popcountll(bal);
        if (nq >= SUPER_DRAIN_AT) {
            stamp(3);
            drain(walk);
            stamp(4);
        }
    };

    __shared__ uint32_t fine[SUPER_FINE];
    __shared__ unsigned long long fine_pairs;
    if (tid == 0) fine_pairs = 0ull;
    static_assert(SUPER_FINE == 256 && NT >= (int)SUPER_FINE, "at most 64 copies: inside a wave");
    auto fine_add = [&](uint32_t key, uint32_t lo_bits) {
        const uint32_t cb = 8u - lo_bits;
        atomicAdd(&fine[((key & ((1u << lo_bits) - 1u)) << cb) | ((uint32_t)lane & ((1u << cb) - 1u))], 1u);
    };
    auto fine_pairs_out = [&](uint32_t lo_bits) {
        if (tid >= SUPER_FINE) return;
        const uint32_t cb = 8u - lo_bits;
        uint32_t n = fine[tid];
#pragma unroll
        for (uint32_t s = 0; s < 6; s++) {
            const uint32_t other = __shfl_xor(n, 1 << s);
            if (s < cb) n += other;
        }
        unsigned long long pairs = (tid & ((1u << cb) - 1u)) == 0u ? (unsigned long long)n * (n ? n - 1u : 0u) / 2ull : 0ull;
        for (int off = 32; off > 0; off >>= 1) pairs += __shfl_down(pairs, off);
        if (lane == 0 && pairs) atomicAdd(&fine_pairs, pairs);
    };
    auto fine_pairs_ranked = [&](uint32_t lo_bits, uint32_t hi_bits, uint32_t c) {
        if (tid >= SUPER_FINE) return;
        unsigned long long pairs = 0ull;
        if (tid < (1u << lo_bits)) {
            const uint32_t first = rank_of(tid << hi_bits);
            const uint32_t next = tid + 1u < (1u << lo_bits) ? rank_of((tid + 1u) << hi_bits) : c;
            const uint32_t n = next - first;
            pairs = (unsigned long long)n * (n ? n - 1u : 0u) / 2ull;
        }
        for (int off = 32; off > 0; off >>= 1) pairs += __shfl_down(pairs, off);
        if (lane == 0 && pairs) atomicAdd(&fine_pairs, pairs);
    };

    for (uint32_t u = blockIdx.x; u < g.n_supers; u += gridDim.x) {
        const SegSuper su = g.supers[u];
        const uint32_t start = __builtin_amdgcn_readfirstlane(g.bin_start[su.bin0]);
        const uint32_t c = __builtin_amdgcn_readfirstlane(g.bin_start[su.bin0 + (1u << (2 * su.g))]) - start;
        const uint32_t lo_bits = 2u * su.g, hi_shift = 2u * su.nb, rest = su.rest;
        if (!super_taken(g, c)) {
            if (g.super_count_pairs && c >= 2u) {
                for (uint32_t w = tid; w < SUPER_FINE; w += NT) fine[w] = 0u;
                __syncthreads();
                for (uint32_t p = tid; p < c; p += NT) fine_add(sub[start + p].key, lo_bits);
                __syncthreads();
                fine_pairs_out(lo_bits);
                __syncthreads();
            }
            continue;
        }
        const uint32_t hi_bits = 2u * rest - lo_bits;
        const uint32_t lo_mask = (1u << lo_bits) - 1u, hi_mask = (1u << hi_bits) - 1u;
        for (uint32_t w = tid; w < SEG_SUPER_WORDS; w += NT) bm[w] = 0u;
        if (g.super_count_pairs)
            for (uint32_t w = tid; w < SUPER_FINE; w += NT) fine[w] = 0u;
        uint32_t rc[SUPER_RPT], ri[SUPER_RPT], rf[SUPER_RPT], rq[SUPER_RPT];
#pragma unroll
        for (int r = 0; r < SUPER_RPT; r++) {
            const uint32_t p = tid + (uint32_t)r * NT;
            rc[r] = ri[r] = rf[r] = rq[r] = 0u;
            if (p < c) {
                const SegRec32 rec = sub[start + p];
                rc[r] = ((rec.key >> hi_shift) & hi_mask) | ((rec.key & lo_mask) << hi_bits);
                ri[r] = rec.idx;
                rf[r] = (uint32_t)rec.freq;
            }
        }
        __syncthreads();
        stamp(0);
        bool twice = false;
#pragma unroll
        for (int r = 0; r < SUPER_RPT; r++)
            if (tid + (uint32_t)r * NT < c) {
                const uint32_t bit = 1u << (rc[r] & 31u);
                twice = twice || (atomicOr(&bm[rc[r] >> 5], bit) & bit) != 0u;
            }
        const bool dup = __syncthreads_or(twice ? 1 : 0) != 0;
        stamp(1);
        if (dup && g.super_count_pairs) {
#pragma unroll
            for (int r = 0; r < SUPER_RPT; r++)
                if (tid + (uint32_t)r * NT < c) fine_add(rc[r] >> hi_bits, lo_bits);
            __syncthreads();
            fine_pairs_out(lo_bits);
            stamp(8);
        }
        if (!dup) {
            {
                uint32_t n_w[WPT], mine = 0;
#pragma unroll
                for (int i = 0; i < WPT; i++) mine += n_w[i] = (uint32_t)__builtin_popcount(bm[tid * WPT + i]);
                uint32_t incl = mine;
                for (int d = 1; d < 64; d <<= 1) {
                    const uint32_t up = __shfl_up(incl, d);
                    if (lane >= d) incl += up;
                }
                if (lane == 63) wsum[wave] = incl;
                __syncthreads();
                uint32_t before = incl - mine;
                for (uint32_t w = 0; w < wave; w++) before += wsum[w];
#pragma unroll
                for (int i = 0; i < WPT; i++) {
                    pre[tid * WPT + i] = before;
                    before += n_w[i];
                }
            }
            __syncthreads();
            if (g.super_count_pairs) {
                stamp(2);
                fine_pairs_ranked(lo_bits, hi_bits, c);
                stamp(8);
            }
#pragma unroll
            for (int r = 0; r < SUPER_RPT; r++)
                if (tid + (uint32_t)r * NT < c) {
                    const uint32_t q = rank_of(rc[r]);
                    rq[r] = q;
                    sc[q] = rc[r];
                    ix[q] = ri[r];
                    fr[q] = rf[r];
                    par[q] = q;
                }
            __syncthreads();
            stamp(2);
#pragma unroll
            for (int r = 0; r < SUPER_RPT; r++) {
                if ((uint32_t)r * NT >= c) break;
                const uint32_t s = rc[r];
                uint32_t m = 0;
#pragma unroll
                for (int bb = 0; bb < SEG_SUPER_MAX_REST; bb++) {
#pragma unroll
                    for (int d = 1; d <= 3; d++) {
                        const uint32_t t = s ^ ((uint32_t)d << (2 * bb));
                        const uint32_t there = (bm[t >> 5] >> (t & 31u)) & 1u;
                        if ((uint32_t)bb < rest && t > s) m |= there << (3 * bb + d - 1);
                    }
                }
                if (tid + (uint32_t)r * NT >= c) m = 0u;
                while (__any(m != 0u)) {
                    const bool has = m != 0u;
                    uint32_t h = 0;
                    if (has) {
                        const int j = __builtin_ctz(m), bb = j / 3;
                        m &= m - 1u;
                        h = rq[r] | ((s ^ ((uint32_t)(j - 3 * bb + 1) << (2 * bb))) << 13);
                    }
                    push(has, h, false);
                }
            }
            stamp(3);
            if (nq) drain(false);
        } else {
#pragma unroll
            for (int r = 0; r < SUPER_RPT; r++) {
                const uint32_t p = tid + (uint32_t)r * NT;
                if (p < c) {
                    sc[p] = rc[r];
                    ix[p] = ri[r];
                    fr[p] = rf[r];
                    par[p] = p;
                }
            }
            __syncthreads();
            stamp(2);
#pragma unroll
            for (int r = 0; r < SUPER_RPT; r++) {
                if ((uint32_t)r * NT >= c) break;
                const uint32_t p = tid + (uint32_t)r * NT, p_first = p - (uint32_t)lane;
                const uint32_t s = rc[r];
                const uint32_t n_it = c > p_first + 1u ? c - 1u - p_first : 0u;
                for (uint32_t i = 1; i <= n_it; i++) {
                    const uint32_t q = p + i;
                    const uint32_t z = s ^ (q < c ? sc[q] : 0u);
                    const bool hit = p < c && q < c && __builtin_popcount((z | (z >> 1)) & 0x55555555u) <= 1;
                    if (__any(hit)) push(hit, p | (q << 13), true);
                }
            }
            stamp(3);
            if (nq) drain(true);
        }
        __syncthreads();
        stamp(4);
        for (;;) {
            bool moved = false;
            for (uint32_t p = tid; p < c; p += NT) {
                const uint32_t q = lds_ld(&par[p]), up = lds_ld(&par[q]);
                if (up != q) {
                    __hip_atomic_store(&par[p], up, __ATOMIC_RELAXED, __HIP_MEMORY_SCOPE_WORKGROUP);
                    moved = true;
                }
            }
            if (!__syncthreads_or(moved ? 1 : 0)) break;
        }
        stamp(5);
        for (uint32_t p = tid; p < c; p += NT) sc[p] = lds_ld(&par[p]);
        __syncthreads();
        for (uint32_t p = tid; p < c; p += NT) fr[p] = 0xFFFFFFFFu;
        __syncthreads();
        for (uint32_t p = tid; p < c; p += NT) atomicMin(&fr[sc[p]], ix[p]);
        __syncthreads();
        stamp(6);
        for (uint32_t p = tid; p < c; p += NT) g.uf_parent[ix[p]] = fr[sc[p]];
        __syncthreads();
        stamp(7);
    }
    if (lane == 0) g.priv_cnt[my_slot] = min(n_out, SEG_PRIV_CAP);
    for (int off = 32; off > 0; off >>= 1) n_cand += __shfl_down(n_cand, off);
    for (int off = 32; off > 0; off >>= 1) n_direct += __shfl_down(n_direct, off);
    if (lane == 0) g.priv_stat[my_slot] = make_uint2(n_cand, n_direct);
    if (g.super_count_pairs) {
        __syncthreads();
        if (tid == 0 && fine_pairs) atomicAdd(&a.counters[CNT_SEG_PAIRS], fine_pairs);
    }
}

__global__ __launch_bounds__(1024) void seg_edge_scan_kernel(uint32_t *priv_cnt, uint32_t n_blocks,
                                                             unsigned long long *counters)
{
    __shared__ uint32_t wsum[16];
    __shared__ uint32_t carry;
    if (threadIdx.x == 0) carry = 0;
    __syncthreads();
    const unsigned long long base = counters[CNT_EDGES];
    for (uint32_t b0 = 0; b0 < n_blocks; b0 += 1024) {
        const uint32_t i = b0 + threadIdx.x;
        const uint32_t v = i < n_blocks ? priv_cnt[i] : 0u;
        uint32_t incl = v;
        for (int d = 1; d < 64; d <<= 1) {
            const uint32_t up = __shfl_up(incl, d);
            if ((int)(threadIdx.x & 63) >= d) incl += up;
        }
        if ((threadIdx.x & 63) == 63) wsum[threadIdx.x >> 6] = incl;
        __syncthreads();
        uint32_t off = carry;
        for (uint32_t w = 0; w < (threadIdx.x >> 6); w++) off += wsum[w];
        if (i < n_blocks) priv_cnt[i] = (uint32_t)min(base + off + incl - v, 0xFFFFFFFFull);
        __syncthreads();
        if (threadIdx.x == 1023) carry = off + incl;
        __syncthreads();
    }
    if (threadIdx.x == 0) counters[CNT_EDGES] = base + carry;
}

__global__ __launch_bounds__(64) void seg_edge_move_kernel(SegArgs g, const uint32_t *__restrict__ priv_off,
                                                           uint32_t n_blocks, uint2 *__restrict__ edges,
                                                           uint8_t *__restrict__ edge_dist, uint32_t edge_cap,
                                                           const unsigned long long *counters)
{
    const uint32_t b = blockIdx.x;
    const unsigned long long first = priv_off[b];
    const unsigned long long next = b + 1 < n_blocks ? (unsigned long long)priv_off[b + 1] : counters[CNT_EDGES];
    const uint32_t cnt = (uint32_t)(next - first);
    for (uint32_t i = threadIdx.x; i < cnt; i += 64) {
        const unsigned long long pos = first + i;
        if (pos < edge_cap) {
            edges[pos] = g.priv_edges[(size_t)b * SEG_PRIV_CAP + i];
            if (edge_dist) edge_dist[pos] = g.priv_dist[(size_t)b * SEG_PRIV_CAP + i];
        }
    }
}

}

hipError_t launch_seg_build(const SegArgs &g, void *fkey, const int32_t *freq, bool key32,
                            unsigned long long *counters, hipStream_t s)
{
    if (g.n_chunks == 0 || g.n_ranges == 0) return hipSuccess;
    const size_t lds = (size_t)g.lds_bins * g.parts_per_pass * sizeof(uint32_t);
    if (g.blocks) {
        if (key32) seg_count_lds_kernel<uint32_t><<<g.n_blocks, SEG_BLOCK_THREADS, lds, s>>>(g, (uint32_t *)fkey);
        else seg_count_lds_kernel<uint64_t><<<g.n_blocks, SEG_BLOCK_THREADS, lds, s>>>(g, (uint64_t *)fkey);
    }
    seg_scan_kernel<<<g.n_chunks, SCAN_THREADS, 0, s>>>(g, counters);
    if (g.blocks) {
        if (key32) seg_scatter_lds_kernel<uint32_t><<<g.n_blocks, SEG_BLOCK_THREADS, lds, s>>>(g, (const uint32_t *)fkey, freq);
        else seg_scatter_lds_kernel<uint64_t><<<g.n_blocks, SEG_BLOCK_THREADS, lds, s>>>(g, (const uint64_t *)fkey, freq);
    } else {
        if (key32) seg_scatter_kernel<uint32_t><<<g.n_ranges, 256, 0, s>>>(g, (const uint32_t *)fkey, freq);
        else seg_scatter_kernel<uint64_t><<<g.n_ranges, 256, 0, s>>>(g, (const uint64_t *)fkey, freq);
    }
    return hipGetLastError();
}

int seg_pair_blocks_per_cu(bool key32, bool has_n, bool ckey)
{
    int nb = 0;
    hipError_t e;
    if (key32 && ckey)
        e = has_n ? hipOccupancyMaxActiveBlocksPerMultiprocessor(&nb, seg_pair_kernel<uint32_t, true, true>, 64, 0)
                  : hipOccupancyMaxActiveBlocksPerMultiprocessor(&nb, seg_pair_kernel<uint32_t, false, true>, 64, 0);
    else if (key32)
        e = has_n ? hipOccupancyMaxActiveBlocksPerMultiprocessor(&nb, seg_pair_kernel<uint32_t, true, false>, 64, 0)
                  : hipOccupancyMaxActiveBlocksPerMultiprocessor(&nb, seg_pair_kernel<uint32_t, false, false>, 64, 0);
    else
        e = has_n ? hipOccupancyMaxActiveBlocksPerMultiprocessor(&nb, seg_pair_kernel<uint64_t, true, false>, 64, 0)
                  : hipOccupancyMaxActiveBlocksPerMultiprocessor(&nb, seg_pair_kernel<uint64_t, false, false>, 64, 0);
// ... 14 lines not shown
    } else if (g.key_words <= 1) {
        if (has_n) seg_pair_kernel<uint64_t, true, false><<<n_blocks, 64, 0, s>>>(a, g, percentage, part, n_parts);
        else seg_pair_kernel<uint64_t, false, false><<<n_blocks, 64, 0, s>>>(a, g, percentage, part, n_parts);
    } else {
#define UMI_SEG_WIDE(WN)                                                                                           \
    do {                                                                                                           \
        if (has_n) seg_pair_kernel<uint64_t, true, false, WN><<<n_blocks, 64, 0, s>>>(a, g, percentage, part, n_parts);  \
        else seg_pair_kernel<uint64_t, false, false, WN><<<n_blocks, 64, 0, s>>>(a, g, percentage, part, n_parts);       \
    } while (0)
        switch (g.key_words) {
        case 2: UMI_SEG_WIDE(2); break;
        case 3: UMI_SEG_WIDE(3); break;
        case 4: UMI_SEG_WIDE(4); break;
        default: return hipErrorInvalidValue;
        }
#undef UMI_SEG_WIDE
    }
    return hipGetLastError();
}

size_t seg_local_lds_bytes(uint32_t cap) { return ((size_t)4 * cap + LOCAL_HITQ + 2 * SEG_PROBE_WORDS) * sizeof(uint32_t); }

int seg_local_blocks_per_cu(bool has_n, uint32_t cap)
{
    int nb = 0;
    const size_t lds = seg_local_lds_bytes(cap);
    const hipError_t e = has_n ? hipOccupancyMaxActiveBlocksPerMultiprocessor(&nb, seg_local_kernel<true>, 64, lds)
                               : hipOccupancyMaxActiveBlocksPerMultiprocessor(&nb, seg_local_kernel<false>, 64, lds);
    return e == hipSuccess && nb > 0 ? nb : 8;
}

hipError_t launch_seg_local(const PairArgs &a, const SegArgs &g, float percentage, uint32_t n_blocks, hipStream_t s)
{
    if (g.n_chunks == 0 || n_blocks == 0 || g.local_cap == 0) return hipSuccess;
    if (g.local_cap > SEG_LOCAL_MAX_CAP || !g.uf_parent || !g.priv_stat || !g.use_ckey ||
        (a.mode != MODE_DIRECTIONAL && a.mode != MODE_CLUSTER))
        return hipErrorInvalidValue;
    const size_t lds = seg_local_lds_bytes(g.local_cap);
    if (a.mode == MODE_CLUSTER) {
        if (a.nmask) seg_local_kernel<true, true><<<n_blocks, 64, lds, s>>>(a, g, percentage);
        else seg_local_kernel<false, true><<<n_blocks, 64, lds, s>>>(a, g, percentage);
    } else if (a.nmask) seg_local_kernel<true><<<n_blocks, 64, lds, s>>>(a, g, percentage);
    else seg_local_kernel<false><<<n_blocks, 64, lds, s>>>(a, g, percentage);
    return hipGetLastError();
}

size_t seg_super_lds_bytes(uint32_t cap)
{
    const uint32_t n_waves = seg_super_threads(cap) / 64u;
    return ((size_t)4 * cap + 2 * SEG_SUPER_WORDS + (size_t)n_waves * SUPER_HITQ) * sizeof(uint32_t);
}
static_assert(((size_t)4 * SEG_SUPER_MAX_CAP + 2 * SEG_SUPER_WORDS + 16 * SUPER_HITQ + SUPER_FINE) * sizeof(uint32_t) + 64 <= 160 * 1024,
              "the largest block, its wave sums and its fine-bin counters fit a CU's LDS");

uint32_t seg_super_blocks(uint32_t n_supers, uint32_t n_cus) { return n_supers < n_cus ? n_supers : n_cus; }

template <bool CLUSTER, int NT>
static hipError_t launch_seg_super_as(const PairArgs &a, const SegArgs &g, float percentage, uint32_t n_blocks, size_t lds,
                                      hipStream_t s)
{
    const hipError_t e = hipFuncSetAttribute((const void *)seg_super_kernel<CLUSTER, NT>,
                                             hipFuncAttributeMaxDynamicSharedMemorySize, (int)lds);
    if (e != hipSuccess) return e;
    seg_super_kernel<CLUSTER, NT><<<n_blocks, NT, lds, s>>>(a, g, percentage);
    return hipGetLastError();
}

hipError_t launch_seg_super(const PairArgs &a, const SegArgs &g, float percentage, uint32_t n_blocks, hipStream_t s)
{
    if (g.n_supers == 0 || n_blocks == 0 || g.super_cap == 0) return hipSuccess;
    if (g.super_cap > SEG_SUPER_MAX_CAP || !g.supers || !g.uf_parent || !g.priv_stat || a.nmask || a.k != 1 ||
        (a.mode != MODE_DIRECTIONAL && a.mode != MODE_CLUSTER))
        return hipErrorInvalidValue;
    const size_t lds = seg_super_lds_bytes(g.super_cap);
    static_assert(SEG_SUPER_SMALL <= 256 * SUPER_RPT && SEG_SUPER_MAX_CAP <= 1024 * SUPER_RPT, "a block holds the cap in registers");
    const bool small = seg_super_threads(g.super_cap) == 256u;
    if (a.mode == MODE_CLUSTER)
        return small ? launch_seg_super_as<true, 256>(a, g, percentage, n_blocks, lds, s)
                     : launch_seg_super_as<true, 1024>(a, g, percentage, n_blocks, lds, s);
    return small ? launch_seg_super_as<false, 256>(a, g, percentage, n_blocks, lds, s)
                 : launch_seg_super_as<false, 1024>(a, g, percentage, n_blocks, lds, s);
}

hipError_t launch_seg_edge_append(const PairArgs &a, const SegArgs &g, uint32_t n_blocks, hipStream_t s)
{
    if (g.n_chunks == 0 || n_blocks == 0) return hipSuccess;
    seg_edge_scan_kernel<<<1, 1024, 0, s>>>(g.priv_cnt, n_blocks, a.counters);
    seg_edge_move_kernel<<<n_blocks, 64, 0, s>>>(g, g.priv_cnt, n_blocks, a.edges,
                                                 a.mode == MODE_NEIGHBOURS ? a.edge_dist : nullptr, a.edge_cap,
                                                 a.counters);
    return hipGetLastError();
}

}
```

Baseline: 1993000 billion UMI-pair comparisons/s.

## Replace cross-super-bin pair scan with bitmap intersection kernel

Adds a seg_cross path. Each super-bin kernel writes its occupancy bitmap and prefix counts to a global cross map, and a new seg_cross_kernel then finds Hamming-1 neighbours across super-bins by ANDing the bitmaps of partner super-bins that differ in one shared base. This replaces the generic segment pair kernel for those segments and aims to avoid the sort/partition pair scanning. It adds global map memory (up to 64 MB per call), an extra launch and a fallback path that re-plans and reruns when the kernel abandons.

```diff
diff --git a/include/umihip.h b/include/umihip.h
--- a/include/umihip.h
+++ b/include/umihip.h
@@ -59,6 +59,7 @@
                           uint32_t *owner);
 const char *umi_last_error(void);
 int umi_ctx_set_option(umi_ctx *ctx, const char *name, int64_t value);
+int umi_ctx_get_counter(const umi_ctx *ctx, const char *name, uint64_t *out);
 #define UMI_ABI_VERSION 2
 int umi_abi_version(void);
 
diff --git a/umi_collapse_rs_amd/_lib.py b/umi_collapse_rs_amd/_lib.py
--- a/umi_collapse_rs_amd/_lib.py
+++ b/umi_collapse_rs_amd/_lib.py
@@ -54,6 +54,7 @@
     "umi_ctx_destroy": (None, [C.c_void_p]),
     "umi_last_error": (C.c_char_p, []),
     "umi_ctx_set_option": (C.c_int, [C.c_void_p, C.c_char_p, C.c_int64]),
+    "umi_ctx_get_counter": (C.c_int, [C.c_void_p, C.c_char_p, C.POINTER(C.c_uint64)]),
     "umi_abi_version": (C.c_int, []),
     "umi_encode_umis": (C.c_int, [_u8p, C.c_uint64, C.c_int, _u64p, _u64p]),
     "umi_encode_umis_wide": (C.c_int, [_u8p, C.c_uint64, C.c_int, C.c_int, _u64p, _u64p]),
diff --git a/umi_collapse_rs_amd/api.py b/umi_collapse_rs_amd/api.py
--- a/umi_collapse_rs_amd/api.py
+++ b/umi_collapse_rs_amd/api.py
@@ -72,6 +72,11 @@
 
     def set_option(self, name, value):
         check(load().umi_ctx_set_option(self._h, name.encode(), int(value)))
+
+    def counter(self, name):
+        v = C.c_uint64(0)
+        check(load().umi_ctx_get_counter(self._h, name.encode(), C.byref(v)))
+        return int(v.value)
 
     def close(self):
         if getattr(self, "_h", None):
diff --git a/umi_collapse_rs_amd/csrc/umihip_api.cpp b/umi_collapse_rs_amd/csrc/umihip_api.cpp
--- a/umi_collapse_rs_amd/csrc/umihip_api.cpp
+++ b/umi_collapse_rs_amd/csrc/umihip_api.cpp
@@ -106,6 +106,15 @@
         if (ctx->ev[i]) (void)hipEventDestroy(ctx->ev[i]);
     if (ctx->own_stream) (void)hipStreamDestroy(ctx->own_stream);
     delete ctx;
+}
+
+int umi_ctx_get_counter(const umi_ctx *ctx, const char *name, uint64_t *out)
+{
+    if (!ctx || !name || !out) return fail(UMI_ERR_ARG, "ctx/name/out is NULL");
+    if (!strcmp(name, "seg_cross_launches")) *out = ctx->seg_cross_launches;
+    else if (!strcmp(name, "seg_cross_abandoned")) *out = ctx->seg_cross_abandoned_calls;
+    else return fail(UMI_ERR_ARG, "unknown counter '%s'", name);
+    return UMI_OK;
 }
 
 int umi_ctx_set_option(umi_ctx *ctx, const char *name, int64_t value)
@@ -189,6 +198,13 @@
     } else if (!strcmp(name, "seg_super_coarse")) {
         if (value != 0 && value != 1) return fail(UMI_ERR_ARG, "seg_super_coarse must be 0 or 1");
         ctx->seg_super_coarse = value != 0;
+    } else if (!strcmp(name, "seg_cross")) {
+        if (value != 0 && value != 1) return fail(UMI_ERR_ARG, "seg_cross must be 0 or 1");
+        ctx->seg_cross = value != 0;
+        ctx->seg_cross_failed = false;
+    } else if (!strcmp(name, "seg_cross_map_mb")) {
+        if (value < 0 || value > 64) return fail(UMI_ERR_ARG, "seg_cross_map_mb must be in 0..64");
+        ctx->seg_cross_map_mb = (uint32_t)value;
     } else if (!strcmp(name, "seg_super_bases")) {
         if (value < 0 || value > SEG_SUPER_MAX_BASES) return fail(UMI_ERR_ARG, "seg_super_bases must be in 0..%d", SEG_SUPER_MAX_BASES);
         ctx->seg_super_bases = (int)value;
diff --git a/umi_collapse_rs_amd/csrc/umihip_host.hpp b/umi_collapse_rs_amd/csrc/umihip_host.hpp
--- a/umi_collapse_rs_amd/csrc/umihip_host.hpp
+++ b/umi_collapse_rs_amd/csrc/umihip_host.hpp
@@ -199,6 +199,11 @@
     uint32_t seg_probe_min = umihip::SEG_PROBE_MIN;
     bool seg_super = true;
     bool seg_super_coarse = true;
+    bool seg_cross = true;
+    bool seg_cross_failed = false;
+    uint64_t seg_cross_launches = 0;
+    uint64_t seg_cross_abandoned_calls = 0;
+    uint32_t seg_cross_map_mb = umihip::SEG_CROSS_MAP_MB;
     int seg_super_bases = 0;
     uint32_t seg_super_cap = umihip::SEG_SUPER_CAP;
     uint32_t seg_super_min = umihip::SEG_SUPER_MIN;
@@ -210,6 +215,7 @@
     umihip::DevBuf plan_tables;
     umihip::DevBuf bs_tasks, plane_tasks, planes, tab_rows, tab_items;
     umihip::DevBuf seg_bin_cnt, seg_bin_start, seg_tasks, seg_sub_rec, seg_priv_edges, seg_priv_dist, seg_priv_cnt, seg_priv_stat;
+    umihip::DevBuf seg_cross_maps;
     umihip::PinnedBuf h_plan_alt[2];
     int plan_flip = 0;
     size_t plan_uploaded = 0;
diff --git a/umi_collapse_rs_amd/csrc/umihip_internal.h b/umi_collapse_rs_amd/csrc/umihip_internal.h
--- a/umi_collapse_rs_amd/csrc/umihip_internal.h
+++ b/umi_collapse_rs_amd/csrc/umihip_internal.h
@@ -37,7 +37,8 @@
     CNT_KEPT_FUSED = 14,
     CNT_UF_DIRECT = 15,
     CNT_EDGES_MOVED = 16,
-    CNT_COUNT = 17,
+    CNT_SEG_CROSS_ABANDONED = 17,
+    CNT_COUNT = 18,
 };
 constexpr int MAX_ROUNDS_PER_SYNC = 16;
 constexpr size_t CTRL_FLAGS_OFF = CNT_COUNT * sizeof(unsigned long long);
@@ -61,6 +62,11 @@
 constexpr uint32_t SEG_NONE = 0xFFFFFFFFu;
 
 constexpr int SEG_MAX_PARTS = 8;
+#if defined(__HIPCC__)
+#define UMIHIP_HD __host__ __device__
+#else
+#define UMIHIP_HD
+#endif
 struct SegDesc {
     uint32_t start, end;
     uint32_t bin_off[SEG_MAX_PARTS];
@@ -68,12 +74,17 @@
     uint8_t nb[SEG_MAX_PARTS];
     uint64_t mask[SEG_MAX_PARTS];
     uint8_t sup_g;
-    uint8_t sup_pad[7];
+    uint8_t cross;
+    uint8_t sup_pad[6];
 };
 struct SegSuper {
     uint32_t bin0;
-    uint8_t g, nb, rest, pad;
-};
+    uint8_t g, nb, rest, cross;
+    uint32_t seg;
+    uint32_t map0;
+};
+static_assert(sizeof(SegSuper) == 16, "no padding: the plan's tables are compared byte by byte");
+UMIHIP_HD inline uint32_t seg_cross_words(uint32_t rest) { return rest >= 3u ? 1u << (2u * rest - 5u) : 1u; }
 struct SegRec32 {
     uint32_t key;
     uint32_t idx;
@@ -95,11 +106,6 @@
     uint32_t col0;
     uint32_t where;
 };
-#if defined(__HIPCC__)
-#define UMIHIP_HD __host__ __device__
-#else
-#define UMIHIP_HD
-#endif
 UMIHIP_HD inline uint32_t seg_chunks_of(uint32_t c) { return c >= 2 ? (c - 1 + 63) / 64 : 0u; }
 UMIHIP_HD inline uint32_t seg_span_log2(uint32_t nt)
 {
@@ -215,6 +221,8 @@
     uint32_t n_supers;
     uint32_t super_coarse;
     uint32_t super_count_pairs;
+    uint32_t *cross_map;
+    uint16_t *cross_pre;
 #ifdef UMIHIP_DEV
     unsigned long long *super_stamps;
 #endif
@@ -244,6 +252,11 @@
 size_t seg_super_lds_bytes(uint32_t cap);
 uint32_t seg_super_blocks(uint32_t n_supers, uint32_t n_cus);
 hipError_t launch_seg_super(const PairArgs &a, const SegArgs &g, float percentage, uint32_t n_blocks, hipStream_t s);
+constexpr uint32_t SEG_CROSS_CHUNKS = SEG_SUPER_WORDS / 64u;
+constexpr int SEG_CROSS_MAX_SHARED = 8;
+constexpr uint64_t SEG_CROSS_CALL_BYTES = 64ull << 20;
+constexpr uint32_t SEG_CROSS_MAP_MB = 8;
+hipError_t launch_seg_cross(const PairArgs &a, const SegArgs &g, float percentage, uint32_t n_blocks, hipStream_t s);
 size_t seg_local_lds_bytes(uint32_t cap);
 int seg_local_blocks_per_cu(bool has_n, uint32_t cap);
 hipError_t launch_seg_local(const PairArgs &a, const SegArgs &g, float percentage, uint32_t n_blocks, hipStream_t s);
diff --git a/umi_collapse_rs_amd/csrc/umihip_pipeline.cpp b/umi_collapse_rs_amd/csrc/umihip_pipeline.cpp
--- a/umi_collapse_rs_amd/csrc/umihip_pipeline.cpp
+++ b/umi_collapse_rs_amd/csrc/umihip_pipeline.cpp
@@ -171,6 +171,7 @@
     uint32_t priv_blocks_for_collapse = 0;
     uint64_t seg_local_bins = 0;
     bool super_pairs_counted = false;
+    uint32_t launches_before_attempt = 0;
     umi_stats st;
     unsigned long long *d_cnt = nullptr;
     size_t n_tasks = 0;
@@ -299,6 +300,8 @@
         sup.bases = ctx->seg_super_bases;
         sup.cap = ctx->seg_super_cap;
         sup.min = ctx->seg_super_min;
+        sup.cross = sup.on && ctx->seg_cross && !ctx->seg_cross_failed && ctx->seg_super_coarse && ctx->seg_lds && k == 1;
+        sup.cross_map_mb = ctx->seg_cross_map_mb;
         build_plan(bucket_off, n_buckets, wide() || edit ? 0x7FFFFFFFu : ctx->small_max,
                    ctx->use_bitslice && k <= BS_MAX_K && !wide() && !edit && dev_tiles,
                    plan_umi_len(), fused_max, ctx->prune && dev_tiles, ctx->bs_sorted && ctx->bs_unit == 2 && need_pairs && dev_tiles,
@@ -366,6 +369,30 @@
         if ((rc = ctx->plane_tasks.reserve(std::max<size_t>(1, pl.plane_tasks.size()) * sizeof(PlaneTask))) ||
             (rc = ctx->planes.reserve(std::max<uint64_t>(1, pl.plane_words) * sizeof(uint32_t))))
             return rc;
+        return UMI_OK;
+    }
+
+    void strip_cross()
+    {
+        for (SegDesc &sd : pl.segs) sd.cross = 0;
+        for (SegSuper &su : pl.seg_supers) {
+            su.cross = 0;
+            su.map0 = 0;
+        }
+        pl.seg_cross = pl.seg_cross_words = 0;
+    }
+    int upload_stripped_plan()
+    {
+        int rc;
+        strip_cross();
+        if ((rc = upload_plan())) return rc;
+        seg.segs = d_segs;
+        seg.chunks = d_chunks;
+        seg.ranges = d_ranges;
+        if (seg.blocks) seg.blocks = d_seg_blocks;
+        if (seg.supers) seg.supers = d_supers;
+        seg.cross_map = nullptr;
+        seg.cross_pre = nullptr;
         return UMI_OK;
     }
 
@@ -427,7 +454,18 @@
                 seg.parts_per_pass = std::max(1u, std::min({4u, (uint32_t)pl.seg_parts, SEG_LDS_BINS / std::max(1u, pl.seg_max_bins)}));
                 seg.super_coarse = super_on && ctx->seg_super_coarse ? 1u : 0u;
             }
+            if (pl.seg_cross) {
+                if (!(super_on && seg.super_coarse)) {
+                    if ((rc = upload_stripped_plan())) return rc;
+                } else {
+                    if ((rc = ctx->seg_cross_maps.reserve(pl.seg_cross_words * (sizeof(uint32_t) + sizeof(uint16_t))))) return rc;
+                    seg.cross_map = ctx->seg_cross_maps.as<uint32_t>();
+                    seg.cross_pre = (uint16_t *)(seg.cross_map + pl.seg_cross_words);
+                }
+            }
             if (!zero_behind_control) HIP_TRY(hipMemsetAsync(seg.bin_cnt, 0, zero_bytes, s));
+        } else if (pl.seg_cross) {
+            strip_cross();
         }
         return UMI_OK;
     }
@@ -758,7 +796,13 @@
                                                         : 0u;
             const uint32_t super_blocks = seg.super_cap ? seg_super_blocks(seg.n_supers, (uint32_t)ctx->n_cus) : 0u;
             const uint32_t super_slots = super_blocks * (seg_super_threads(seg.super_cap) / 64u);
-            const size_t slots = (size_t)local_blocks + super_slots + blocks;
+            const uint32_t pair_blocks = pl.seg_cross < pl.segs.size() ? blocks : 0u;
+            const uint32_t cross_blocks = pl.seg_cross && super_blocks
+                                              ? (uint32_t)std::max<uint64_t>(1, std::min<uint64_t>((uint64_t)seg.n_supers * SEG_CROSS_CHUNKS,
+                                                    ctx->seg_blocks ? ctx->seg_blocks : (uint64_t)ctx->n_cus * 16u))
+                                              : 0u;
+            if (pl.seg_cross && !cross_blocks) return fail(UMI_ERR_HIP, "internal: cross segments planned without super-bins");
+            const size_t slots = (size_t)local_blocks + super_slots + pair_blocks + cross_blocks;
             if ((rc = ctx->seg_priv_edges.reserve(slots * SEG_PRIV_CAP * sizeof(uint2))) ||
                 (rc = ctx->seg_priv_cnt.reserve(slots * 4)) || (rc = ctx->seg_priv_stat.reserve(slots * sizeof(uint2))) ||
                 (mode == MODE_NEIGHBOURS && (rc = ctx->seg_priv_dist.reserve((size_t)blocks * SEG_PRIV_CAP))))
@@ -822,11 +866,19 @@
                 }
             }
 #endif
-            HIP_TRY(launch_seg_pairs(a, pair_seg, key32, percentage, part, n_parts, blocks, s));
+            if (pair_blocks) HIP_TRY(launch_seg_pairs(a, pair_seg, key32, percentage, part, n_parts, pair_blocks, s));
+            if (cross_blocks) {
+                SegArgs cross_seg = pair_seg;
+                cross_seg.priv_edges += (size_t)pair_blocks * SEG_PRIV_CAP;
+                cross_seg.priv_cnt += pair_blocks;
+                cross_seg.priv_stat += pair_blocks;
+                HIP_TRY(launch_seg_cross(a, cross_seg, percentage, cross_blocks, s));
+                ctx->seg_cross_launches++;
+            }
             if (prof) HIP_TRY(hipEventRecord(ctx->ev[8], s));
             seg_timed = true;
             priv_blocks_for_collapse = slots_to_collapse ? (uint32_t)slots : 0u;
-            if (!priv_blocks_for_collapse) HIP_TRY(launch_seg_edge_append(a, seg, blocks, s));
+            if (!priv_blocks_for_collapse) HIP_TRY(launch_seg_edge_append(a, seg, pair_blocks, s));
             st.n_pair_launches += 1;
         }
         if ((rc = enqueue_legacy_tiles(a))) return rc;
@@ -941,7 +993,8 @@
         const bool have_pairs = need_pairs && n_tasks;
         uint64_t cap = std::max<uint64_t>(ctx->edge_capacity, 1024);
         const int ahead = std::min(std::max(ctx->dag_rounds_ahead, DAG_ROUNDS), MAX_ROUNDS_PER_SYNC);
-        for (int attempt = 0;; attempt++) {
+        for (int attempt = 0;;) {
+            launches_before_attempt = st.n_pair_launches;
             if (have_pairs) {
                 uint64_t ovf_cap = 0;
                 if ((rc = reserve_lists(cap, ovf_cap))) return rc;
@@ -965,8 +1018,15 @@
             }
             if ((rc = read_control())) return rc;
             if ((rc = note_pair_counters())) return rc;
-            if (n_edges <= cap || !have_pairs) break;
-            if ((rc = grow_edge_list(cap, attempt))) return rc;
+            const bool abandoned = have_pairs && pl.seg_cross && ctx->h_counters[CNT_SEG_CROSS_ABANDONED] != 0;
+            const bool over = have_pairs && !abandoned && n_edges > cap;
+            if (!abandoned && !over) break;
+            if (over) {
+                if ((rc = grow_edge_list(cap, attempt++))) return rc;
+            } else {
+                HIP_TRY(hipMemsetAsync(&d_cnt[CNT_EDGES], 0, 2 * sizeof(unsigned long long), s));
+            }
+            if (abandoned && (rc = drop_cross())) return rc;
             HIP_TRY(hipMemsetAsync(&d_cnt[CNT_KEPT], 0, sizeof(unsigned long long), s));
             HIP_TRY(hipMemsetAsync(&d_cnt[CNT_UF_DIRECT], 0, 2 * sizeof(unsigned long long), s));
             if (!cluster) HIP_TRY(hipMemsetAsync(ctx->d_changed(), 0, CTRL_BYTES - CTRL_FLAGS_OFF, s));
@@ -979,6 +1039,23 @@
         else if ((rc = directional_rounds_end(have_pairs, ahead)))
             return rc;
         return finish_stats();
+    }
+
+    int drop_cross()
+    {
+        int rc;
+        ctx->seg_cross_failed = true;
+        if ((rc = upload_stripped_plan())) return rc;
+        seg.prep_keys = nullptr;
+        HIP_TRY(hipMemsetAsync(seg.bin_cnt, 0, seg_zero_bytes(), s));
+        static_assert(CNT_SEG_PAIRS == CNT_SEG_TASKS + 1, "one fill");
+        HIP_TRY(hipMemsetAsync(&d_cnt[CNT_SEG_TASKS], 0, 2 * sizeof(unsigned long long), s));
+        HIP_TRY(hipMemsetAsync(&d_cnt[CNT_SEG_CROSS_ABANDONED], 0, sizeof(unsigned long long), s));
+        HIP_TRY(launch_seg_build(seg, ctx->fkey.p, d_freq, key32, d_cnt, s));
+        super_pairs_counted = false;
+        st.n_pair_launches = launches_before_attempt;
+        ctx->seg_cross_abandoned_calls++;
+        return UMI_OK;
     }
 
     int enqueue_directional_collapse(int ahead)
diff --git a/umi_collapse_rs_amd/csrc/umihip_plan.hpp b/umi_collapse_rs_amd/csrc/umihip_plan.hpp
--- a/umi_collapse_rs_amd/csrc/umihip_plan.hpp
+++ b/umi_collapse_rs_amd/csrc/umihip_plan.hpp
@@ -32,6 +32,8 @@
     std::vector<SegBlock> seg_blocks;
     std::vector<SegSuper> seg_supers;
     uint64_t seg_plain = 0;
+    uint64_t seg_cross = 0;
+    uint64_t seg_cross_words = 0;
     uint32_t seg_max_bins = 0;
     int seg_max_rest = 0;
     int seg_parts = 0;
@@ -153,6 +155,8 @@
     bool on = false;
     int bases = 0;
     uint32_t cap = SEG_SUPER_CAP, min = SEG_SUPER_MIN;
+    bool cross = false;
+    uint32_t cross_map_mb = SEG_CROSS_MAP_MB;
 };
 inline int choose_super_bases(uint64_t n, int umi_len, int nb0, const SegSuperOpt &o)
 {
@@ -165,6 +169,13 @@
         return g;
     }
     return 0;
+}
+
+inline bool choose_cross(int umi_len, int sup_g, const SegSuperOpt &o, uint64_t used_bytes = 0)
+{
+    if (!o.on || !o.cross || sup_g <= 0 || umi_len > 16) return false;
+    const uint64_t bytes = (1ull << (2 * umi_len)) / 8;
+    return bytes <= ((uint64_t)o.cross_map_mb << 20) && used_bytes + bytes <= SEG_CROSS_CALL_BYTES;
 }
 
 inline void plan_segment(Plan &pl, uint64_t s, uint64_t e, int umi_len, int k, bool key32,
@@ -186,6 +197,7 @@
         sd.mask[j] = 0;
     }
     sd.sup_g = 0;
+    sd.cross = 0;
     for (uint8_t &b : sd.sup_pad) b = 0;
     for (int j = 0; j < P; j++) {
         const int b0 = j * umi_len / P, b1 = (j + 1) * umi_len / P;
@@ -205,9 +217,15 @@
     }
     if (k == 1 && key32) sd.sup_g = (uint8_t)choose_super_bases(n, umi_len, sd.nb[0], sup);
     if (sd.sup_g) {
-        const uint32_t g = sd.sup_g, nb0 = sd.nb[0];
+        const uint32_t g = sd.sup_g, nb0 = sd.nb[0], rest = (uint32_t)umi_len - nb0 + g;
+        sd.cross = rest >= 3 && choose_cross(umi_len, sd.sup_g, sup, pl.seg_cross_words * 4) ? 1 : 0;
         for (uint32_t sb = 0; sb < (1u << (2 * (nb0 - g))); sb++)
-            pl.seg_supers.push_back({sd.bin_off[0] + (sb << (2 * g)), (uint8_t)g, (uint8_t)nb0, (uint8_t)(umi_len - nb0 + g), 0});
+            pl.seg_supers.push_back({sd.bin_off[0] + (sb << (2 * g)), (uint8_t)g, (uint8_t)nb0, (uint8_t)rest, sd.cross, seg,
+                                     sd.cross ? (uint32_t)pl.seg_cross_words + sb * seg_cross_words(rest) : 0u});
+        if (sd.cross) {
+            pl.seg_cross++;
+            pl.seg_cross_words += (uint64_t)seg_cross_words(rest) << (2 * (nb0 - g));
+        }
     } else {
         pl.seg_plain++;
     }
@@ -326,6 +344,7 @@
     pl.seg_blocks.clear();
     pl.seg_supers.clear();
     pl.seg_plain = 0;
+    pl.seg_cross = pl.seg_cross_words = 0;
     pl.seg_max_bins = 0;
     pl.seg_max_rest = 0;
     pl.seg_parts = 0;
diff --git a/umi_collapse_rs_amd/csrc/umihip_seg.hip b/umi_collapse_rs_amd/csrc/umihip_seg.hip
--- a/umi_collapse_rs_amd/csrc/umihip_seg.hip
+++ b/umi_collapse_rs_amd/csrc/umihip_seg.hip
@@ -57,6 +57,7 @@
         for (int q = 0; q < SCAN_PER_THREAD; q++)
             if (local_bin(g, ch.part, c[q])) no_tasks |= 1u << q;
     }
+    if (g.segs[ch.seg].cross) no_tasks = (1u << SCAN_PER_THREAD) - 1u;
 #pragma unroll
     for (int q = 0; q < SCAN_PER_THREAD; q++) mine.y += (no_tasks >> q) & 1u ? 0u : seg_tasks_of_bin(c[q]);
     uint2 incl = mine;
@@ -314,8 +315,9 @@
     const SegDesc *__restrict__ sd = g.segs + blk.seg;
     const uint32_t cg = coarse_bases(g, blk.seg);
     Rec *__restrict__ sub = (Rec *)g.sub_rec;
-    for (int j0 = 0; j0 < g.n_parts; j0 += (int)g.parts_per_pass) {
-        const SegPass ps = seg_pass_of(sd, j0, g.n_parts, (int)g.parts_per_pass, cg);
+    const int n_parts = sd->cross ? 1 : g.n_parts;
+    for (int j0 = 0; j0 < n_parts; j0 += (int)g.parts_per_pass) {
+        const SegPass ps = seg_pass_of(sd, j0, n_parts, (int)g.parts_per_pass, cg);
         seg_block_histogram(blk, fkey, ps, hist);
         for (uint32_t c = threadIdx.x; c < ps.total; c += SEG_BLOCK_THREADS) {
             const uint32_t cnt = hist[c];
@@ -1206,6 +1208,30 @@
         const uint32_t start = __builtin_amdgcn_readfirstlane(g.bin_start[su.bin0]);
         const uint32_t c = __builtin_amdgcn_readfirstlane(g.bin_start[su.bin0 + (1u << (2 * su.g))]) - start;
         const uint32_t lo_bits = 2u * su.g, hi_shift = 2u * su.nb, rest = su.rest;
+        uint32_t *__restrict__ x_map = nullptr;
+        uint16_t *__restrict__ x_pre = nullptr;
+        uint2 *__restrict__ x_rec = nullptr;
+        if (su.cross) {
+            const SegDesc *__restrict__ sd = g.segs + su.seg;
+            x_map = g.cross_map + su.map0;
+            x_pre = g.cross_pre + su.map0;
+            x_rec = (uint2 *)((SegRec32 *)g.sub_rec + g.bin_start[sd->bin_off[1]]) + (start - g.bin_start[sd->bin_off[0]]);
+        }
+        if (su.cross && c < 2u) {
+            uint32_t code = 0xFFFFFFFFu;
+            if (c == 1u) {
+                const SegRec32 rec = sub[start];
+                const uint32_t hb = 2u * rest - lo_bits;
+                code = ((rec.key >> hi_shift) & ((1u << hb) - 1u)) | ((rec.key & ((1u << lo_bits) - 1u)) << hb);
+                if (tid == 0) {
+                    x_pre[code >> 5] = 0;
+                    x_rec[0] = make_uint2(rec.idx, (uint32_t)rec.freq);
+                }
+            }
+            for (uint32_t w = tid; w < seg_cross_words(rest); w += NT) x_map[w] = w == (code >> 5) ? 1u << (code & 31u) : 0u;
+            continue;
+        }
+        if (su.cross && c > cap && tid == 0) a.counters[CNT_SEG_CROSS_ABANDONED] = 1ull;
         if (!super_taken(g, c)) {
             if (g.super_count_pairs && c >= 2u) {
                 for (uint32_t w = tid; w < SUPER_FINE; w += NT) fine[w] = 0u;
@@ -1245,6 +1271,7 @@
             }
         const bool dup = __syncthreads_or(twice ? 1 : 0) != 0;
         stamp(1);
+        if (dup && su.cross && tid == 0) a.counters[CNT_SEG_CROSS_ABANDONED] = 1ull;
         if (dup && g.super_count_pairs) {
 #pragma unroll
             for (int r = 0; r < SUPER_RPT; r++)
@@ -1291,6 +1318,13 @@
                 }
             __syncthreads();
             stamp(2);
+            if (su.cross) {
+                for (uint32_t w = tid; w < seg_cross_words(rest); w += NT) {
+                    x_map[w] = bm[w];
+                    x_pre[w] = (uint16_t)pre[w];
+                }
+                for (uint32_t p = tid; p < c; p += NT) x_rec[p] = make_uint2(ix[p], fr[p]);
+            }
 #pragma unroll
             for (int r = 0; r < SUPER_RPT; r++) {
                 if ((uint32_t)r * NT >= c) break;
@@ -1381,6 +1415,142 @@
         __syncthreads();
         if (tid == 0 && fine_pairs) atomicAdd(&a.counters[CNT_SEG_PAIRS], fine_pairs);
     }
+}
+
+constexpr uint32_t CROSS_DRAIN_AT = 64;
+constexpr uint32_t CROSS_HITQ = CROSS_DRAIN_AT + 64;
+constexpr int CROSS_MAX_PARTNERS = 3 * SEG_CROSS_MAX_SHARED;
+static_assert(SEG_SUPER_WORDS <= (1u << 11) && CROSS_MAX_PARTNERS <= 32, "word index, bit and partner number in one queue word");
+
+template <bool CLUSTER>
+__global__ __launch_bounds__(64) void seg_cross_kernel(PairArgs a, SegArgs g, float percentage)
+{
+    __shared__ uint32_t hitq[CROSS_HITQ];
+    const int lane = threadIdx.x;
+    unsigned int n_cand = 0, n_direct = 0;
+    uint32_t n_out = 0;
+    uint2 *__restrict__ slot = g.priv_edges + (size_t)blockIdx.x * SEG_PRIV_CAP;
+    auto emit = [&](bool has, uint32_t u, uint32_t v) {
+        const unsigned long long bal = __ballot(has);
+        if (!bal) return;
+        const uint32_t cnt = (uint32_t)__builtin_popcountll(bal);
+        const uint32_t pos = n_out + (uint32_t)__builtin_popcountll(bal & ((1ull << lane) - 1ull));
+        unsigned long long base = 0;
+        if (n_out + cnt > SEG_PRIV_CAP) {
+            const uint32_t first_over = max(n_out, SEG_PRIV_CAP);
+            const int leader = __builtin_ctzll(bal);
+            if (lane == leader) base = atomicAdd(&a.counters[CNT_EDGES], (unsigned long long)(n_out + cnt - first_over));
+            base = __shfl(base, leader);
+            base -= first_over;
+        }
+        if (has) {
+            if (pos < SEG_PRIV_CAP) slot[pos] = make_uint2(u, v);
+            else if (base + pos < a.edge_cap) a.edges[base + pos] = make_uint2(u, v);
+        }
+        n_out += cnt;
+    };
+    uint32_t have_u = 0xFFFFFFFFu, sb = 0, seg_map0 = 0, W = 0, my_map0 = 0, my_rec0 = 0, seg_entries = 1, seg_pos0 = 0, seg_bin0 = 0;
+    uint32_t n_shared = 0, g2 = 0;
+    const uint2 *__restrict__ seg_rec = nullptr;
+    uint32_t nq = 0;
+    auto drain = [&]() {
+        const uint32_t n = min(nq, 64u);
+        nq -= n;
+        __builtin_amdgcn_fence(__ATOMIC_ACQ_REL, "wavefront");
+        __builtin_amdgcn_wave_barrier();
+        const bool has = (uint32_t)lane < n;
+        const uint32_t h = has ? hitq[nq + (uint32_t)lane] : 0u;
+        const uint32_t w = h & 0x7FFu, bit = (h >> 11) & 31u, pn = h >> 16;
+        const uint32_t b = pn / 3u, d = pn - 3u * b + 1u;
+        const uint32_t sbp = has ? sb ^ (d << (2u * b)) : sb;
+        const uint32_t wa_at = my_map0 + w, wb_at = seg_map0 + sbp * W + w;
+        const uint32_t wa = g.cross_map[wa_at], wb = g.cross_map[wb_at];
+        const uint32_t pa = g.cross_pre[wa_at], pb = g.cross_pre[wb_at];
+        const uint32_t start_b = g.bin_start[seg_bin0 + (sbp << g2)];
+        const uint32_t below = (1u << bit) - 1u;
+        const uint32_t ra = min(my_rec0 + pa + (uint32_t)__builtin_popcount(wa & below), seg_entries - 1u);
+        const uint32_t rb = min(start_b - seg_pos0 + pb + (uint32_t)__builtin_popcount(wb & below), seg_entries - 1u);
+        const uint2 ea = seg_rec[ra], eb = seg_rec[rb];
+        const uint32_t ia = ea.x, ib = eb.x;
+        const int32_t fa = (int32_t)ea.y, fb = (int32_t)eb.y;
+        const bool sw = ib < ia;
+        const uint32_t gi = sw ? ib : ia, gj = sw ? ia : ib;
+        const int32_t fi = sw ? fb : fa, fj = sw ? fa : fb;
+        const bool ok = has && gi != gj && gj < a.n_entries;
+        if (ok) n_cand++;
+        const bool fwd = ok && (CLUSTER || fj <= threshold_of(percentage, fi));
+        const bool bwd = ok && (CLUSTER || fi <= threshold_of(percentage, fj));
+        uint32_t uu[1] = {gi}, uv[1] = {gj};
+        bool unite[1] = {fwd && bwd};
+        if (unite[0]) n_direct++;
+        uf_union_multi<1>(g.uf_parent, uu, uv, unite);
+        emit(fwd != bwd, fwd ? gi : gj, fwd ? gj : gi);
+        __builtin_amdgcn_wave_barrier();
+    };
+
+    const bool abandoned = a.counters[CNT_SEG_CROSS_ABANDONED] != 0ull;
+    const uint32_t n_items = abandoned ? 0u : g.n_supers * SEG_CROSS_CHUNKS;
+    const uint32_t per = (n_items + gridDim.x - 1u) / gridDim.x;
+    const uint32_t it0 = min(n_items, blockIdx.x * per), it1 = min(n_items, it0 + per);
+    for (uint32_t it = it0; it < it1; it++) {
+        const uint32_t u = it / SEG_CROSS_CHUNKS, chunk = it % SEG_CROSS_CHUNKS;
+        if (u != have_u) {
+            while (nq) drain();
+            have_u = u;
+            const SegSuper su = g.supers[u];
+            W = 0u;
+            if (su.cross) {
+                const SegDesc *__restrict__ sd = g.segs + su.seg;
+                g2 = 2u * su.g;
+                n_shared = (uint32_t)su.nb - su.g;
+                seg_bin0 = sd->bin_off[0];
+                sb = (su.bin0 - seg_bin0) >> g2;
+                W = seg_cross_words(su.rest);
+                my_map0 = su.map0;
+                seg_map0 = su.map0 - sb * W;
+                seg_pos0 = g.bin_start[seg_bin0];
+                my_rec0 = g.bin_start[su.bin0] - seg_pos0;
+                seg_entries = max(1u, sd->end - sd->start);
+                seg_rec = (const uint2 *)((const SegRec32 *)g.sub_rec + g.bin_start[sd->bin_off[1]]);
+            }
+        }
+        const uint32_t w = chunk * 64u + (uint32_t)lane;
+        if (chunk * 64u >= W) continue;
+        const bool live = w < W;
+        const uint32_t mine = live ? g.cross_map[my_map0 + w] : 0u;
+        uint32_t m[CROSS_MAX_PARTNERS];
+#pragma unroll
+        for (int b = 0; b < SEG_CROSS_MAX_SHARED; b++) {
+#pragma unroll
+            for (int d = 1; d <= 3; d++) {
+                const uint32_t sbp = sb ^ ((uint32_t)d << (2 * b));
+                const bool there = (uint32_t)b < n_shared && sbp > sb;
+                m[3 * b + d - 1] = there && live ? g.cross_map[seg_map0 + sbp * W + w] : 0u;
+            }
+        }
+        for (uint32_t pn = 0; pn < 3u * n_shared; pn++) {
+            uint32_t mp = 0;
+#pragma unroll
+            for (int q = 0; q < CROSS_MAX_PARTNERS; q++) mp = pn == (uint32_t)q ? m[q] : mp;
+            uint32_t x = mine & mp;
+            while (__any(x != 0u)) {
+                const bool has = x != 0u;
+                const unsigned long long bal = __ballot(has);
+                if (has) {
+                    const uint32_t bit = (uint32_t)__builtin_ctz(x);
+                    x &= x - 1u;
+                    hitq[nq + (uint32_t)__builtin_popcountll(bal & ((1ull << lane) - 1ull))] = w | (bit << 11) | (pn << 16);
+                }
+                nq += (uint32_t)__builtin_popcountll(bal);
+                if (nq >= CROSS_DRAIN_AT) drain();
+            }
+        }
+    }
+    while (nq) drain();
+    if (lane == 0) g.priv_cnt[blockIdx.x] = min(n_out, SEG_PRIV_CAP);
+    for (int off = 32; off > 0; off >>= 1) n_cand += __shfl_down(n_cand, off);
+    for (int off = 32; off > 0; off >>= 1) n_direct += __shfl_down(n_direct, off);
+    if (lane == 0) g.priv_stat[blockIdx.x] = make_uint2(n_cand, n_direct);
 }
 
 __global__ __launch_bounds__(1024) void seg_edge_scan_kernel(uint32_t *priv_cnt, uint32_t n_blocks,
@@ -1561,6 +1731,17 @@
                  : launch_seg_super_as<false, 1024>(a, g, percentage, n_blocks, lds, s);
 }
 
+hipError_t launch_seg_cross(const PairArgs &a, const SegArgs &g, float percentage, uint32_t n_blocks, hipStream_t s)
+{
+    if (g.n_supers == 0 || n_blocks == 0) return hipSuccess;
+    if (!g.supers || !g.cross_map || !g.cross_pre || !g.uf_parent || !g.priv_stat || a.nmask || a.k != 1 || g.n_parts != 2 ||
+        g.n_supers > 0xFFFFFFFFu / SEG_CROSS_CHUNKS || (a.mode != MODE_DIRECTIONAL && a.mode != MODE_CLUSTER))
+        return hipErrorInvalidValue;
+    if (a.mode == MODE_CLUSTER) seg_cross_kernel<true><<<n_blocks, 64, 0, s>>>(a, g, percentage);
+    else seg_cross_kernel<false><<<n_blocks, 64, 0, s>>>(a, g, percentage);
+    return hipGetLastError();
+}
+
 hipError_t launch_seg_edge_append(const PairArgs &a, const SegArgs &g, uint32_t n_blocks, hipStream_t s)
 {
     if (g.n_chunks == 0 || n_blocks == 0) return hipSuccess;
```

Result: faster. 2220000 billion UMI-pair comparisons/s, median of 6 (+11.4%).
